# lmb-freiburg/flownet2

Hardware: AMD Instinct MI355X
Metric: image-pairs/sec FlowNetC forward at 448x320 (higher is better)
Workload: dtype f32

## Files before the change

flownet2_amd/_lib.py:

```python
from __future__ import annotations

import ctypes as C
import os
import re

_HERE = os.path.dirname(os.path.abspath(__file__))
SO_PATH = os.path.join(_HERE, "libflownet2_hip.so")
INCLUDE_DIR = os.path.join(_HERE, "..", "include")

_SCALARS = {"int": C.c_int, "float": C.c_float, "size_t": C.c_size_t, "long long": C.c_longlong, "unsigned long long": C.c_ulonglong,
            "char": C.c_char}
_POINTERS = {"float": C.c_void_p, "void": C.c_void_p, "unsigned char": C.c_void_p, "char": C.c_char_p, "int": C.POINTER(C.c_int),
             "unsigned": C.POINTER(C.c_uint), "size_t": C.POINTER(C.c_size_t)}
_STRUCT_NAMES = {"fn2_l1loss_params": "L1LossParams", "fn2_l1loss_scale": "L1LossScale"}
_DECLARATOR = re.compile(r"^([\w\s*]*?)(\w+)\s*(?:\[(\d+)\])?$")
_FUNCTION = re.compile(r"^([\w\s*]+?)\b(fn2_\w+)\s*\(([^()]*)\)$")


class Fn2Error(RuntimeError):

    def __init__(self, status: int, message: str):
        super().__init__(f"[fn2 status {status}] {message}")
        self.status = status


def _ctype(spec, structs, where):
    words = [w for w in spec.replace("*", " ").split() if w != "const"]
    base, stars = " ".join(words), spec.count("*")
    if stars == 0 and base in _SCALARS:
        return _SCALARS[base]
    if stars == 1 and base in structs:
        return C.POINTER(structs[base])
    if stars == 1 and base in _POINTERS:
        return _POINTERS[base]
    if stars == 2 and base in ("float", "void"):
        return C.POINTER(C.c_void_p)
    raise ValueError(f"C header: unknown type `{spec.strip()}` in `{where}`")


def _declarator(text, structs, where):
    m = _DECLARATOR.match(text.strip())
    if not m or not m.group(1).strip():
        raise ValueError(f"C header: cannot read `{text.strip()}` in `{where}`")
    t = _ctype(m.group(1), structs, where)
    return m.group(2), (t * int(m.group(3)) if m.group(3) else t), m.group(1)


def parse_header(text, structs=None):
    structs = dict(structs or {})
    functions, constants = {}, {}
    text = re.sub(r"/\*.*?\*/", " ", text, flags=re.S)
    for name, value in re.findall(r"^[ \t]*#[ \t]*define[ \t]+(FN2_\w+)[ \t]+(-?(?:0[xX][0-9a-fA-F]+|\d+))[ \t]*$", text, flags=re.M):
        constants[name] = int(value, 0)
    text = re.sub(r"^[ \t]*#.*$", " ", text, flags=re.M)

    def enum(m):
        value = -1
        for item in filter(None, (s.strip() for s in m.group(1).split(","))):
            name, _, v = (s.strip() for s in item.partition("="))
            value = int(v, 0) if v else value + 1
            constants[name] = value
        return " "
    text = re.sub(r"(?:typedef\s+)?enum\s*\w*\s*\{([^{}]*)\}\s*\w*\s*;", enum, text)

    def struct(m):
        cname, fields = m.group(1), []
        for decl in filter(None, (s.strip() for s in m.group(2).split(";"))):
            first, *more = decl.split(",")
            name, t, spec = _declarator(first, structs, "struct " + cname)
            fields.append((name, t))
            fields += [_declarator(spec + " " + other, structs, "struct " + cname)[:2] for other in more]
        pyname = _STRUCT_NAMES.get(cname) or "".join(w.capitalize() for w in cname.split("_")[1:])
        structs[cname] = type(pyname, (C.Structure,), {"_fields_": fields, "__doc__": cname, "__module__": __name__})
        return " "
    text = re.sub(r"typedef\s+struct\s+(fn2_\w+)\s*\{([^{}]*)\}\s*\w+\s*;", struct, text)

    text = re.sub(r'extern\s*"C"\s*\{|\}', " ", text)
    for stmt in filter(None, (" ".join(s.split()) for s in text.split(";"))):
        m = _FUNCTION.match(stmt)
        if not m:
            raise ValueError(f"C header: cannot read the declaration `{stmt}`")
        params = m.group(3).strip()
        args = [] if params == "void" else [_declarator(p, structs, stmt)[1] for p in params.split(",")]
        functions[m.group(2)] = (_ctype(m.group(1), structs, stmt), args)
    return functions, structs, constants


def _parse_headers():
    per_header, structs, constants = [], {}, {}
    for h in ("flownet2_hip.h", "flownet2_hip_solver.h", "flownet2_hip_corr_route.h", "flownet2_hip_conv_general.h"):
        with open(os.path.join(INCLUDE_DIR, h)) as f:
            functions, structs, c = parse_header(f.read(), structs)
        per_header.append(functions)
        constants.update(c)
    return per_header, structs, constants


_PER_HEADER, _STRUCTS, CONSTANTS = _parse_headers()
EXPORTS, SOLVER_EXPORTS, CORR_ROUTE_EXPORTS, CONV_GENERAL_EXPORTS = (list(f) for f in _PER_HEADER)
PROTOTYPES = {name: proto for f in _PER_HEADER for name, proto in f.items()}
globals().update({cls.__name__: cls for cls in _STRUCTS.values()})
_HOOKS = parse_header("""
    int fn2_debug_set_correlation_impl(int impl);
    int fn2_debug_correlation_units_plan(int N, int H, int W, int policy, unsigned* out_words, int max_words);
    int fn2_debug_set_resample_generic(int on);
    int fn2_debug_set_correlation_trace(void* device_buffer);""")[0]

_lib = None


def lib():
    global _lib
    if _lib is not None:
        return _lib
    if not os.path.exists(SO_PATH):
        raise RuntimeError(
            f"{SO_PATH} not found: the HIP extension is not built. Run `python -m flownet2_amd.build` "
            "(or __graft_entry__.build()). flownet2_amd has no CPU / PyTorch fallback.")
    L = C.CDLL(SO_PATH)
    for table, required in ((PROTOTYPES, True), (_HOOKS, False)):
        for name, (restype, argtypes) in table.items():
            if not hasattr(L, name):
                if required:
                    raise RuntimeError(f"{SO_PATH} does not export {name}")
                continue
            fn = getattr(L, name)
            fn.restype, fn.argtypes = restype, argtypes
    _lib = L
    return L


def check(status: int):
    if status != 0:
        raise Fn2Error(status, lib().fn2_last_error_string().decode())


def version() -> str:
    return lib().fn2_version().decode()
```

flownet2_amd/csrc/conv_mfma.hip:

```cpp
#include "mfma_tile.hpp"

namespace fn2 {
namespace cv {

using namespace mfma;

struct Args {
  const float* in; const float* wp; const float* bias; float* out;
  int N, Cin, Hin, Win, in_ctot, in_c0;
  int Cout, Hout, Wout, out_ctot, out_c0;
  int pad;
  int nchunks;
  int ksteps;
  int tx, ty;
  int ng;
  unsigned total;
  unsigned nbig;
  float slope; int relu;
};

template <int KS_, int S_, int MW_, int NP_, int WM_, int WNX_, int WNY_, int CQ_, int P16_ = 0, int PIN_ = 0>
struct Cfg : Window<((P16_ ? 1 : 4) * WNY_ - 1) * S_ + KS_,
                    ((P16_ ? 16 : 4) * NP_ * WNX_ - 1) * S_ + KS_ + 4,
                    CQ_, WM_ * WNX_ * WNY_> {
// ... 170 lines not shown
}

template <int KS> struct PackTile {
  static constexpr int T = KS * KS;
  static constexpr int QT = KS == 1 ? 8 : KS == 3 ? 3 : KS == 4 ? 2 : 1;
  static constexpr int CIL = 4 * QT, ROW = CIL * T + 1;
  static constexpr int LDS_FLOATS = 64 * ROW;
};

template <int KS, int ORDER>
__global__ void __launch_bounds__(256) pack_weights_view(const float* __restrict__ w, float* __restrict__ wp, int ksteps, int kalloc,
                                                         int src_co, int src_ci, long long s_co, long long s_ci, int flip) {
  using P = PackTile<KS>;
  constexpr int T = P::T, QT = P::QT, CIL = P::CIL, ROW = P::ROW;
  __shared__ float tile[P::LDS_FLOATS];
  const int grp = blockIdx.x, cq0 = blockIdx.y * QT;
  const int co0 = 64 * grp, ci0 = 4 * cq0;
  const int nquads = ksteps / T;
  constexpr int TOTAL = 64 * CIL * T;
  if constexpr (ORDER == 0) {
    const float* src = w + (size_t)co0 * s_co + (size_t)ci0 * T;
#pragma unroll
    for (int i = threadIdx.x; i < TOTAL; i += 256) {
      const int col = i / (CIL * T), e = i - col * (CIL * T), c = e / T;
      tile[col * ROW + e] = (co0 + col < src_co && ci0 + c < src_ci) ? src[(size_t)col * s_co + e] : 0.f;
    }
  } else if constexpr (ORDER == 1) {
    const float* src = w + (size_t)ci0 * s_ci + (size_t)co0 * T;
#pragma unroll
    for (int i = threadIdx.x; i < TOTAL; i += 256) {
      const int c = i / (64 * T), e = i - c * (64 * T), col = e / T, t = e - col * T;
      tile[col * ROW + c * T + t] = (co0 + col < src_co && ci0 + c < src_ci) ? src[(size_t)c * s_ci + e] : 0.f;
    }
  } else {
#pragma unroll
    for (int i = threadIdx.x; i < TOTAL; i += 256) {
      const int col = i / (CIL * T), e = i - col * (CIL * T), c = e / T, t = e - c * T;
      tile[col * ROW + e] = (co0 + col < src_co && ci0 + c < src_ci) ? w[(size_t)(co0 + col) * s_co + (size_t)(ci0 + c) * s_ci + t] : 0.f;
    }
  }
  __syncthreads();
  const int nq = min(QT, nquads - cq0);
  float* dst = wp + ((size_t)grp * kalloc + (size_t)cq0 * T) * 256;
  const int j = threadIdx.x & 3, lane = threadIdx.x >> 2;
  const float* trow = tile + (16 * j + (lane & 15)) * ROW + (lane >> 4) * T;
#pragma unroll
  for (int ks = 0; ks < QT * T; ++ks) {
    const int cq = ks / T, tap = ks - cq * T;
    if (cq < nq) dst[ks * 256 + threadIdx.x] = trow[4 * cq * T + (flip ? T - 1 - tap : tap)];
  }
  if (cq0 + QT >= nquads)
    for (int i = threadIdx.x; i < (kalloc - ksteps) * 256; i += 256) wp[((size_t)grp * kalloc + ksteps) * 256 + i] = 0.f;
}

template <int KS>
static void launch_pack_view(const float* w, float* wp, int Cout, int ksteps, int kalloc, int src_co, int src_ci, long long s_co, long long s_ci, int flip,
                             hipStream_t st) {
  using P = PackTile<KS>;
  const dim3 grid((unsigned)((Cout + 63) / 64), (unsigned)cdiv(ksteps / P::T, P::QT));
  if (s_ci == (long long)P::T) hipLaunchKernelGGL((pack_weights_view<KS, 0>), grid, dim3(256), 0, st, w, wp, ksteps, kalloc, src_co, src_ci, s_co, s_ci, flip);
  else if (s_co == (long long)P::T) hipLaunchKernelGGL((pack_weights_view<KS, 1>), grid, dim3(256), 0, st, w, wp, ksteps, kalloc, src_co, src_ci, s_co, s_ci, flip);
  else hipLaunchKernelGGL((pack_weights_view<KS, 2>), grid, dim3(256), 0, st, w, wp, ksteps, kalloc, src_co, src_ci, s_co, s_ci, flip);
}

constexpr int kSpare = 8;
constexpr int kChunkQuads = 2;

inline int chunk_quads(int KS) { return KS == 1 ? 8 : kChunkQuads; }
inline int ksteps_for(int Cin, int KS) { return cdiv(cdiv(Cin, 4), chunk_quads(KS)) * chunk_quads(KS) * KS * KS; }

template <class K>
static void set_geometry(Args& a) {
  if constexpr (K::P16) {
    a.Win *= a.Hin; a.Hin = 1; a.Wout *= a.Hout; a.Hout = 1;
  }
  a.tx = cdiv(a.Wout, K::TW); a.ty = cdiv(a.Hout, K::TH);
  a.ng = a.Cout / (16 * K::MW * K::WM);
  a.nchunks = cdiv(cdiv(a.Cin, 4), K::CQ);
}

inline long long tiles_of(const Args& a) { return (long long)a.N * a.tx * a.ty * a.ng; }

template <class K>
static int launch(const Args& base, hipStream_t st) {
  Args a = base;
  set_geometry<K>(a);
  a.nbig = (unsigned)tiles_of(a);
  return launch_tiles<&conv_mfma<K>>(a, tiles_of(a), K::THREADS, (int)(sizeof(float) * 2 * K::BUF), "conv_mfma", "conv_mfma_forward", st);
}

inline unsigned whole_rounds(long long tiles) { return (unsigned)(tiles / 256 * 256); }

template <class K>
static int launch_tail(const Args& base, hipStream_t st) {
  if constexpr (K::MW < 2) {
    return fail(FN2_ERR_UNSUPPORTED, "conv_mfma: variant has no split tail");
  } else {
    Args a = base;
    set_geometry<K>(a);
    if (tiles_of(a) > 0x1fffff00ll) return fail(FN2_ERR_UNSUPPORTED, "conv_mfma: grid too large");
    a.total = (unsigned)tiles_of(a); a.nbig = whole_rounds(a.total);
    const unsigned nsm = 2 * (a.total - a.nbig);
    const unsigned grid = a.nbig + 8 * ((nsm + 7) / 8);
    constexpr size_t lds = sizeof(float) * 2 * K::BUF;
    set_dynamic_lds_once<&conv_mfma_tail<K>>((int)lds);
    hipLaunchKernelGGL((conv_mfma_tail<K>), dim3(grid), dim3(K::THREADS), lds, st, a);
    return check_launch("conv_mfma_forward");
  }
}

struct Variant {
  int ks, s, mw, np, wm, wnx, wny, p16;
  int (*fn)(const Args&, hipStream_t);
  int (*fn_tail)(const Args&, hipStream_t);
};

#define FN2_CV_LIST(X) \
   \
  X(1, 1, 2, 7, 2, 2, 1, 8, 1) X(1, 1, 2, 7, 2, 1, 2, 8, 1) X(1, 1, 4, 7, 1, 2, 2, 8, 0) X(1, 1, 4, 7, 1, 1, 4, 8, 0) X(1, 1, 2, 6, 2, 2, 1, 8, 1) \
  X(1, 1, 2, 4, 2, 2, 1, 8, 1) X(1, 1, 2, 7, 1, 2, 2, 8, 0) X(1, 1, 2, 7, 1, 4, 1, 8, 0) X(1, 1, 2, 4, 1, 2, 2, 8, 0) X(1, 1, 4, 4, 1, 2, 2, 8, 0) \
   \
  X(3, 1, 2, 7, 2, 2, 1, 2, 1) X(3, 1, 2, 7, 2, 1, 2, 2, 1) X(3, 1, 4, 7, 1, 2, 2, 2, 0) X(3, 1, 4, 7, 1, 1, 4, 2, 0) \
  X(3, 1, 2, 6, 2, 2, 1, 2, 1) X(3, 1, 4, 6, 1, 2, 2, 2, 0) X(3, 1, 4, 4, 1, 2, 2, 2, 0) X(3, 1, 2, 4, 2, 2, 1, 2, 1) \
   \
  X(3, 2, 2, 7, 2, 1, 2, 2, 1) X(3, 2, 4, 7, 1, 1, 4, 2, 0) X(3, 2, 2, 6, 2, 2, 1, 2, 1) X(3, 2, 4, 6, 1, 2, 2, 2, 0) X(3, 2, 2, 4, 2, 2, 1, 2, 1) \
   \
  X(4, 2, 2, 7, 2, 2, 1, 2, 1) X(4, 2, 2, 7, 2, 1, 2, 2, 1) X(4, 2, 4, 7, 1, 2, 2, 2, 0) X(4, 2, 2, 6, 2, 2, 1, 2, 1) X(4, 2, 4, 4, 1, 2, 2, 2, 0) X(4, 2, 2, 4, 2, 2, 1, 2, 1) \
   \
  X(5, 2, 2, 7, 2, 2, 1, 1, 1) X(5, 2, 2, 7, 2, 1, 2, 1, 1) X(5, 2, 4, 7, 1, 2, 2, 1, 0) X(5, 2, 4, 7, 1, 1, 4, 1, 0) \
  X(5, 2, 2, 6, 2, 2, 1, 1, 1) X(5, 2, 4, 6, 1, 2, 2, 1, 0) X(5, 2, 4, 4, 1, 2, 2, 1, 0) \
   \
  X(7, 2, 2, 6, 2, 2, 1, 1, 1) X(7, 2, 2, 7, 2, 2, 1, 1, 1) X(7, 2, 4, 4, 1, 2, 2, 1, 0) X(7, 2, 4, 6, 1, 2, 2, 1, 0) X(7, 2, 2, 4, 2, 2, 1, 1, 1)

template <class K, int TAIL> struct TailFn { static constexpr int (*fn)(const Args&, hipStream_t) = nullptr; };
template <class K> struct TailFn<K, 1> { static constexpr int (*fn)(const Args&, hipStream_t) = &launch_tail<K>; };

#define FN2_CV_ROW(KS, S, MW, NP, WM, WNX, WNY, CQ, TAIL) \
  {KS, S, MW, NP, WM, WNX, WNY, 0, &launch<Cfg<KS, S, MW, NP, WM, WNX, WNY, CQ>>, TailFn<Cfg<KS, S, MW, NP, WM, WNX, WNY, CQ>, TAIL>::fn},
#define FN2_CV_ROW16(MW, NP, WM, WNX, WNY, TAIL) \
  {1, 1, MW, NP, WM, WNX, WNY, 1, &launch<Cfg<1, 1, MW, NP, WM, WNX, WNY, 8, 1>>, TailFn<Cfg<1, 1, MW, NP, WM, WNX, WNY, 8, 1>, TAIL>::fn},
#define FN2_CV_PIN(KS, S, MW, NP, WM, WNX, WNY, CQ, P16, TAIL) \
  {KS, S, MW, NP, WM, WNX, WNY, P16, &launch<Cfg<KS, S, MW, NP, WM, WNX, WNY, CQ, P16, 1>>, TailFn<Cfg<KS, S, MW, NP, WM, WNX, WNY, CQ, P16, 1>, TAIL>::fn},
static const Variant kVariants[] = {FN2_CV_LIST(FN2_CV_ROW)
  FN2_CV_ROW16(2, 7, 2, 2, 1, 1) FN2_CV_ROW16(2, 7, 4, 1, 1, 1) FN2_CV_ROW16(4, 7, 1, 4, 1, 0) FN2_CV_ROW16(4, 7, 2, 2, 1, 0) FN2_CV_ROW16(2, 5, 2, 2, 1, 1)
  FN2_CV_ROW16(2, 4, 2, 2, 1, 1) FN2_CV_ROW16(2, 7, 1, 4, 1, 0) FN2_CV_ROW16(2, 5, 1, 4, 1, 0) FN2_CV_ROW16(4, 5, 1, 4, 1, 0) FN2_CV_ROW16(2, 4, 1, 4, 1, 0)
  FN2_CV_ROW16(4, 5, 2, 2, 1, 0) FN2_CV_ROW16(4, 4, 2, 2, 1, 0)
  FN2_CV_ROW16(2, 9, 4, 1, 1, 1) FN2_CV_ROW16(2, 9, 2, 2, 1, 1) FN2_CV_ROW16(2, 3, 2, 2, 1, 1) FN2_CV_ROW16(4, 3, 1, 4, 1, 0)
  FN2_CV_ROW16(4, 9, 4, 1, 1, 0) FN2_CV_ROW16(4, 9, 2, 2, 1, 0) FN2_CV_ROW16(4, 7, 4, 1, 1, 0)
  FN2_CV_PIN(5, 2, 2, 7, 2, 2, 1, 1, 0, 1) FN2_CV_PIN(5, 2, 2, 7, 2, 1, 2, 1, 0, 1)
  FN2_CV_PIN(1, 1, 4, 9, 4, 1, 1, 8, 1, 0) FN2_CV_PIN(1, 1, 2, 9, 4, 1, 1, 8, 1, 1) FN2_CV_PIN(1, 1, 2, 5, 2, 2, 1, 8, 1, 1) FN2_CV_PIN(1, 1, 4, 7, 4, 1, 1, 8, 1, 0)
  FN2_CV_PIN(1, 1, 2, 7, 2, 2, 1, 8, 1, 1) FN2_CV_PIN(1, 1, 2, 3, 2, 2, 1, 8, 1, 1)
  FN2_CV_PIN(3, 1, 2, 7, 2, 2, 1, 2, 0, 1) FN2_CV_PIN(3, 1, 2, 6, 2, 2, 1, 2, 0, 1) FN2_CV_PIN(3, 2, 2, 7, 2, 1, 2, 2, 0, 1) FN2_CV_PIN(3, 2, 2, 6, 2, 2, 1, 2, 0, 1)
  FN2_CV_PIN(4, 2, 2, 7, 2, 2, 1, 2, 0, 1) FN2_CV_PIN(4, 2, 2, 6, 2, 2, 1, 2, 0, 1) FN2_CV_PIN(5, 2, 2, 6, 2, 2, 1, 1, 0, 1)
  FN2_CV_PIN(7, 2, 2, 6, 2, 2, 1, 1, 0, 1) FN2_CV_PIN(7, 2, 4, 6, 1, 2, 2, 1, 0, 0)};
constexpr int kNumVariants = sizeof(kVariants) / sizeof(kVariants[0]);

int g_forced_variant = -1;

static double variant_cost(const Variant& v, const Args& a, bool tail) {
  const int tw = (v.p16 ? 16 : 4) * v.np * v.wnx, th = (v.p16 ? 1 : 4) * v.wny;
  const long long wgs = v.p16 ? (long long)a.N * cdiv(a.Wout * a.Hout, tw) * (a.Cout / (16 * v.mw * v.wm))
                              : (long long)a.N * cdiv(a.Wout, tw) * cdiv(a.Hout, th) * (a.Cout / (16 * v.mw * v.wm));
  double rounds = (double)((wgs + 255) / 256);
  if (tail) {
    const long long r = wgs % 256;
    if (wgs < 256 || r == 0 || r > 128) return 1e30;
    rounds = (double)(wgs / 256) + 0.5 * 1.12;
  }
  const double eff = 1.0 / (1.0 + 0.08 * (4.0 / v.mw - 1.0) + 0.02 * (7.0 / v.np - 1.0));
  return rounds * v.mw * v.np / eff;
}

static bool variant_applies(const Variant& v, const Args& a, int KS, int S) {
  if (!v.p16 && a.Win % 4 != 0) return false;
  return v.ks == KS && v.s == S && a.Cout % (16 * v.mw * v.wm) == 0;
}

}
}

using namespace fn2;

FN2_API size_t fn2_conv_mfma_packed_floats(int Cout, int Cin, int kernel) {
  if (Cout <= 0 || Cout % 32 != 0 || Cin <= 0 || kernel <= 0) return 0;
  return (size_t)((Cout + 63) / 64) * (cv::ksteps_for(Cin, kernel) + cv::kSpare) * 256;
}

FN2_API int fn2_conv_mfma_pack_weights_view(const float* weight, float* packed, int Cout, int Cin, int kernel, int src_cout, int src_cin,
                                            long long stride_cout, long long stride_cin, int flip, void* stream);

FN2_API int fn2_conv_mfma_pack_weights(const float* weight, float* packed, int Cout, int Cin, int kernel, void* stream) {
  if (!weight || !packed) return fail(FN2_ERR_INVALID_ARG, "conv_mfma_pack_weights: null blob");
  if (Cout <= 0 || Cout % 32 != 0 || Cin <= 0 || (kernel != 1 && kernel != 3 && kernel != 4 && kernel != 5 && kernel != 7))
    return fail(FN2_ERR_UNSUPPORTED, "conv_mfma_pack_weights: needs Cout %% 32 == 0 and kernel_size 1, 3, 4, 5 or 7 (got Cout %d, kernel %d)", Cout, kernel);
  return fn2_conv_mfma_pack_weights_view(weight, packed, Cout, Cin, kernel, Cout, Cin, (long long)Cin * kernel * kernel, (long long)kernel * kernel, 0, stream);
}

FN2_API int fn2_conv_mfma_pack_weights_view(const float* weight, float* packed, int Cout, int Cin, int kernel, int src_cout, int src_cin,
                                            long long stride_cout, long long stride_cin, int flip, void* stream) {
  if (!weight || !packed) return fail(FN2_ERR_INVALID_ARG, "conv_mfma_pack_weights_view: null blob");
  if (Cout <= 0 || Cout % 32 != 0 || Cin <= 0 || (kernel != 1 && kernel != 3 && kernel != 4 && kernel != 5 && kernel != 7))
    return fail(FN2_ERR_UNSUPPORTED, "conv_mfma_pack_weights_view: needs Cout %% 32 == 0 and kernel_size 1, 3, 4, 5 or 7 (got Cout %d, kernel %d)", Cout, kernel);
  if (src_cout < 1 || src_cout > Cout || src_cin < 1 || src_cin > Cin || stride_cout < 1 || stride_cin < 1)
    return fail(FN2_ERR_INVALID_ARG, "conv_mfma_pack_weights_view: bad source view (%d of %d, %d of %d channels, strides %lld / %lld)", src_cout, Cout,
                src_cin, Cin, stride_cout, stride_cin);
  const int ksteps = cv::ksteps_for(Cin, kernel), kalloc = ksteps + cv::kSpare;
  hipStream_t st = as_stream(stream);
  switch (kernel) {
    case 1: cv::launch_pack_view<1>(weight, packed, Cout, ksteps, kalloc, src_cout, src_cin, stride_cout, stride_cin, flip ? 1 : 0, st); break;
    case 3: cv::launch_pack_view<3>(weight, packed, Cout, ksteps, kalloc, src_cout, src_cin, stride_cout, stride_cin, flip ? 1 : 0, st); break;
    case 4: cv::launch_pack_view<4>(weight, packed, Cout, ksteps, kalloc, src_cout, src_cin, stride_cout, stride_cin, flip ? 1 : 0, st); break;
    case 5: cv::launch_pack_view<5>(weight, packed, Cout, ksteps, kalloc, src_cout, src_cin, stride_cout, stride_cin, flip ? 1 : 0, st); break;
    default: cv::launch_pack_view<7>(weight, packed, Cout, ksteps, kalloc, src_cout, src_cin, stride_cout, stride_cin, flip ? 1 : 0, st); break;
  }
  return check_launch("conv_mfma_pack_weights_view");
}

FN2_API int fn2_conv_mfma_supported(int Cin, int Hin, int Win, int Cout, int kernel, int stride, int pad) {
  if (Cin <= 0 || Hin <= 0 || Win <= 0 || Cout <= 0 || Cout % 32 != 0) return 0;
  if (kernel == 1 ? ((long long)Hin * Win) % 4 != 0 : Win % 4 != 0) return 0;
  if (!((kernel == 1 && stride == 1) || (kernel == 3 && (stride == 1 || stride == 2)) || (kernel == 4 && stride == 2) || (kernel == 5 && stride == 2) || (kernel == 7 && stride == 2))) return 0;
  if (pad < 0 || pad > 4 || pad > kernel - 1) return 0;
  if ((long long)Cin * Hin * Win >= (1ll << 28)) return 0;
  const int Hout = (Hin + 2 * pad - kernel) / stride + 1, Wout = (Win + 2 * pad - kernel) / stride + 1;
  if (Hout < 1 || Wout < 1) return 0;
  cv::Args a{};
  a.Win = Win; a.Cout = Cout;
  for (int i = 0; i < cv::kNumVariants; ++i)
    if (cv::variant_applies(cv::kVariants[i], a, kernel, stride)) return 1;
  return 0;
}

FN2_API int fn2_debug_set_conv_variant(int v) { cv::g_forced_variant = v; return FN2_OK; }
FN2_API int fn2_conv_mfma_num_variants(void) { return cv::kNumVariants; }

FN2_API int fn2_conv_mfma_forward(const float* bottom, const float* packed_weight, const float* bias, float* top,
                                  int N, int Cin, int Hin, int Win, int bottom_channels, int bottom_c0,
                                  int Cout, int top_channels, int top_c0, int kernel, int stride, int pad,
                                  int relu, float negative_slope, void* stream) {
  if (N < 0) return fail(FN2_ERR_INVALID_ARG, "conv_mfma: bad batch");
  if (N == 0) return FN2_OK;
  if (const int rc = mfma::check_conv_args("conv_mfma", bottom, packed_weight, top, Cin, bottom_channels, bottom_c0, Cout, top_channels, top_c0, [&] {
        return fn2_conv_mfma_supported(Cin, Hin, Win, Cout, kernel, stride, pad) ? FN2_OK
            : fail(FN2_ERR_UNSUPPORTED, "conv_mfma: unsupported geometry (Cin %d, %dx%d, Cout %d, k %d s %d p %d)", Cin, Hin, Win, Cout, kernel, stride, pad);
      }))
    return rc;
  cv::Args a{};
  a.in = bottom; a.wp = packed_weight; a.bias = bias; a.out = top;
  a.N = N; a.Cin = Cin; a.Hin = Hin; a.Win = Win; a.in_ctot = bottom_channels; a.in_c0 = bottom_c0;
  a.Cout = Cout; a.Hout = (Hin + 2 * pad - kernel) / stride + 1; a.Wout = (Win + 2 * pad - kernel) / stride + 1;
  a.out_ctot = top_channels; a.out_c0 = top_c0; a.pad = pad;
  a.ksteps = cv::ksteps_for(Cin, kernel) + cv::kSpare;
  a.slope = negative_slope; a.relu = relu;
  hipStream_t st = as_stream(stream);
  static TuneCache cache("conv_mfma", cv::kNumVariants);
  const TuneKey key{N, Cin, Hin, Win, Cout, kernel, stride, pad, bottom_channels == Cin, top_channels == Cout};
  mfma::Pick p;
  if (const int rc = mfma::pick_variant(p, "conv_mfma", cv::g_forced_variant, cv::kNumVariants, true, cache, key, st,
                                        [&](int i) { return cv::variant_applies(cv::kVariants[i], a, kernel, stride); },
                                        [&](int i, bool tail) { return cv::variant_cost(cv::kVariants[i], a, tail); },
                                        [&](int i, bool tail) { return tail ? cv::kVariants[i].fn_tail(a, st) : cv::kVariants[i].fn(a, st); },
                                        [&](int i) { return cv::kVariants[i].fn_tail != nullptr; }))
    return rc;
  return p.tail ? cv::kVariants[p.variant].fn_tail(a, st) : cv::kVariants[p.variant].fn(a, st);
}
```

flownet2_amd/csrc/conv_plane.hip:

```cpp
#include "mfma_tile.hpp"

namespace fn2 {
namespace cp {

using namespace mfma;

constexpr int kNPR = 12;
constexpr int kLdsBytes = 160 * 1024;
constexpr int kSpare = 8;

struct Args {
  const float* in; const float* wp; const float* bias; float* out; float* part;
  int N, Cin, Hin, Win, in_ctot, in_c0;
  int Cout, Hout, Wout, out_ctot, out_c0;
  int pad;
  int P;
  int Wp;
  int img;
  int npb;
  int nig;
  int ng;
  int ksplit;
  int units;
  int ksteps;
  size_t class_stride;
  int rs, cs, wr;
  int band;
  int cap;
  int slots_c, npr;
  int buf;
  unsigned mP, mW, mrs;
  unsigned total;
  float slope; int relu;
};

template <int MODE_, int S_, int MW_, int NP_, int WM_, int WN_, int CQ_, int VEC_, int KS_ = 3>
struct Cfg {
  static constexpr int MODE = MODE_, S = S_, MW = MW_, NP = NP_, WM = WM_, WN = WN_, CQ = CQ_, VEC = VEC_, KS = KS_;
  static constexpr int NCLS = MODE == 1 ? 4 : 1;
  static constexpr int NW = NCLS * WM * WN, THREADS = 64 * NW;
  static constexpr int TAP = MODE == 1 ? 2 : KS;
  static constexpr int PADL = VEC == 4 ? 4 : (KS_ == 5 ? 2 : 1);
  static constexpr int KSC = CQ * TAP * TAP;
  static constexpr int NBUFA = KS_ == 5 ? 5 : (KSC % 9 == 0 && KSC > 9) ? 9 : (KSC % 8 == 0) ? 8 : (KSC % 4 == 0) ? 4 : 3;
  static constexpr int CAP = 16 * NP * WN;
  static_assert(KSC % NBUFA == 0, "ring phase must repeat per chunk");
  static_assert(NBUFA - 1 <= kSpare, "prefetch distance");
  static_assert(MODE == 0 || S == 1, "the deconvolution reads its input at stride 1");
  static_assert(KS == 3 || ((KS == 4 || KS == 5) && MODE == 0 && S == 2), "tap classes: 3x3 / 1, 3x3 / 2, 4x4 / 2, 5x5 / 2");
};

__device__ __forceinline__ int fastdiv(int q, int d, unsigned m) { return d == 1 ? q : (int)__umulhi((unsigned)q, m); }
inline unsigned magic_for(int d) { return d <= 1 ? 0u : (unsigned)(((1ull << 32) + (unsigned)d - 1) / (unsigned)d); }

template <class K>
__device__ __forceinline__ void stage_chunk(__amdgpu_buffer_rsrc_t rs, const unsigned (&voff)[kNPR], const Args& a, unsigned dst, int wave,
                                            unsigned chunk_off, unsigned plane_bytes, unsigned img_bytes, int nimg) {
  const int planes = nimg * 4 * K::CQ;
  const int last = a.slots_c - 64;
  for (int pl = wave; pl < planes; pl += K::NW) {
    const int il = pl / (4 * K::CQ), ch = pl % (4 * K::CQ);
    const unsigned soff = __builtin_amdgcn_readfirstlane(chunk_off + (unsigned)il * img_bytes + (unsigned)ch * plane_bytes);
    const unsigned d0 = __builtin_amdgcn_readfirstlane(dst + 4u * (unsigned)(pl * a.cs));
#pragma unroll
    for (int j = 0; j < kNPR; ++j) {
      if (j < a.npr) {
        const int s0 = 64 * j < last ? 64 * j : last;
        __builtin_amdgcn_raw_ptr_buffer_load_lds(rs, (lds_ptr_t)(uintptr_t)(d0 + 4u * K::VEC * (unsigned)s0), 4 * K::VEC, voff[j], soff, 0, 0);
      }
    }
  }
}

template <class K>
__global__ void __launch_bounds__(K::THREADS)
conv_plane(Args a) {
  extern __shared__ __attribute__((aligned(16))) float smem[];
  constexpr int S = K::S, MW = K::MW, NP = K::NP, TAP = K::TAP;
  unsigned t;
  if (!xcd_task(blockIdx.x, a.total, t)) return;
  const int g = __builtin_amdgcn_readfirstlane((int)(t % a.ng)); t /= a.ng;
  const int pb = __builtin_amdgcn_readfirstlane((int)(t % a.npb)); t /= a.npb;
  const int ig = __builtin_amdgcn_readfirstlane((int)(t % a.nig));
  const int kp = __builtin_amdgcn_readfirstlane((int)(t / a.nig));

  const int tid = threadIdx.x, lane = tid & 63;
  const int wave = __builtin_amdgcn_readfirstlane(tid >> 6);
  const int cls = wave % K::NCLS, w2 = wave / K::NCLS;
  const int py = cls >> 1, px = cls & 1;
  const int wm = w2 % K::WM, wn = w2 / K::WM;
  const int n0 = ig * a.img;
  const int nimg = a.N - n0 < a.img ? a.N - n0 : a.img;

  const int u0 = __builtin_amdgcn_readfirstlane((int)((long long)kp * a.units / a.ksplit));
  const int u1 = __builtin_amdgcn_readfirstlane((int)((long long)(kp + 1) * a.units / a.ksplit));
  const int chunk0 = u0 * (2 / K::CQ), nchunks = (u1 - u0) * (2 / K::CQ);

  const int yblk = a.band ? fastdiv(pb * a.cap, a.Wp, a.mW) : 0;
  const int yorg = (K::MODE == 0 ? S * yblk : yblk) - a.pad;

  const size_t plane = (size_t)a.Hin * a.Win;
  const unsigned plane_bytes = 4u * (unsigned)plane, img_bytes = plane_bytes * (unsigned)a.in_ctot;
  const __amdgpu_buffer_rsrc_t rs = __builtin_amdgcn_make_buffer_rsrc(
      const_cast<float*>(a.in + ((size_t)n0 * a.in_ctot + a.in_c0) * plane), 0,
      (unsigned)(img_bytes * (unsigned)(nimg - 1) + plane_bytes * (unsigned)a.Cin), kRsrcWord3);
  unsigned voff[kNPR];
#pragma unroll
  for (int j = 0; j < kNPR; ++j) {
    voff[j] = kOOB;
    if (j < a.npr) {
      const int last = a.slots_c - 64;
      const int d = K::VEC * ((64 * j < last ? 64 * j : last) + lane);
      const int row = fastdiv(d, a.rs, a.mrs), col = d - row * a.rs;
      const int yi = yorg + row, xi = col - K::PADL;
      if (row < a.wr && yi >= 0 && yi < a.Hin && xi >= 0 && xi < a.Win) voff[j] = 4u * (unsigned)(yi * a.Win + xi);
    }
  }
  const unsigned lds_base = (unsigned)(uintptr_t)(lds_ptr_t)smem;
  const unsigned chunk_bytes = 4u * K::CQ * plane_bytes;

  const int kq = lane >> 4;
  const int tile0 = NP * (pb * K::WN + wn);
  const int lim = nimg * a.P;
  int base[NP];
#pragma unroll
  for (int p = 0; p < NP; ++p) {
    int q = 16 * (tile0 + p) + (lane & 15);
    if (q >= lim) q = 16 * tile0 < lim ? 16 * tile0 : 0;
    const int il = fastdiv(q, a.P, a.mP), rem = q - il * a.P;
    const int y = fastdiv(rem, a.Wp, a.mW), x = rem - y * a.Wp;
    if constexpr (K::MODE == 0) base[p] = (il * 4 * K::CQ + kq) * a.cs + (S * (y - yblk)) * a.rs + S * x + K::PADL - a.pad;
    else base[p] = (il * 4 * K::CQ + kq) * a.cs + (y - yblk + py) * a.rs + x + K::PADL - 1 + px;
  }
  using WV = typename WVec<MW>::T;
  const int cg0 = (g * K::WM + wm) * MW;
  const float* wl = weight_lane(a.wp + (size_t)cls * a.class_stride, cg0, a.ksteps, lane) + (size_t)chunk0 * K::KSC * 256;

  f32x4 acc[MW][NP];
#pragma unroll
  for (int j = 0; j < MW; ++j)
#pragma unroll
    for (int p = 0; p < NP; ++p) acc[j][p] = f32x4{0.f, 0.f, 0.f, 0.f};

  WV wreg[K::NBUFA];
  stage_chunk<K>(rs, voff, a, lds_base, wave, (unsigned)chunk0 * chunk_bytes, plane_bytes, img_bytes, nimg);
#pragma unroll
  for (int i = 0; i < K::NBUFA - 1; ++i) wreg[i] = weight_load<MW>(wl, i);

  for (int c = 0; c < nchunks; ++c) {
    const int buf = c & 1;
    wait_vmcnt<K::NBUFA - 1>();
    __builtin_amdgcn_s_barrier();
    if (c + 1 < nchunks)
      stage_chunk<K>(rs, voff, a, lds_base + 4u * (unsigned)((buf ^ 1) * a.buf), wave, (unsigned)(chunk0 + c + 1) * chunk_bytes, plane_bytes, img_bytes, nimg);
    const float* win = smem + buf * a.buf;
    const int ks0 = c * K::KSC;
    constexpr int NSTEP = K::CQ * TAP;
    float bb[2][TAP][NP];
    auto lds_step = [&](int st, float (&b)[TAP][NP]) {
      const float* wk = win + ((st / TAP) * 4 * a.cs + (st % TAP) * a.rs);
#pragma unroll
      for (int kx = 0; kx < TAP; ++kx)
#pragma unroll
        for (int p = 0; p < NP; ++p) b[kx][p] = wk[base[p] + kx];
    };
    lds_step(0, bb[0]);
    __builtin_amdgcn_sched_barrier(0);
#pragma unroll
    for (int st = 0; st < NSTEP; ++st) {
      const float* wkn = win + (((st + 1) / TAP) * 4 * a.cs + ((st + 1) % TAP) * a.rs);
#pragma unroll
      for (int kx = 0; kx < TAP; ++kx) {
        const int ks = st * TAP + kx;
        wreg[(ks + K::NBUFA - 1) % K::NBUFA] = weight_load<MW>(wl, ks0 + ks + K::NBUFA - 1);
        const WV w = wreg[ks % K::NBUFA];
#pragma unroll
        for (int p = 0; p < NP; ++p) {
#pragma unroll
          for (int j = 0; j < MW; ++j)
            acc[j][p] = __builtin_amdgcn_mfma_f32_16x16x4f32(bb[st & 1][kx][p], wget<MW>(w, j), acc[j][p], 0, 0, 0);
          if (st + 1 < NSTEP) bb[(st + 1) & 1][kx][p] = wkn[base[p] + kx];
          __builtin_amdgcn_sched_barrier(0);
        }
      }
    }
  }

  const bool final_pass = a.ksplit == 1;
  const int Po = a.Hout * a.Wout;
  float* dst = final_pass ? a.out : a.part + (size_t)kp * a.N * a.Cout * Po;
  const int ctot = final_pass ? a.out_ctot : a.Cout, c0 = final_pass ? a.out_c0 : 0;
#pragma unroll
  for (int p = 0; p < NP; ++p) {
    const int q0 = 16 * (tile0 + p) + 4 * (lane >> 4);
    if (q0 >= lim) continue;
    const int il = fastdiv(q0, a.P, a.mP), pix = q0 - il * a.P;
#pragma unroll
    for (int j = 0; j < MW; ++j) {
      const int co = 16 * (cg0 + j) + (lane & 15);
      const float bv = (final_pass && a.bias) ? a.bias[co] : 0.f;
      f32x4 v = acc[j][p];
      if (final_pass) v = bias_relu4(v, bv, a.relu, a.slope);
      if constexpr (K::MODE == 0) {
        float* o = dst + ((size_t)(n0 + il) * ctot + c0 + co) * a.P + pix;
        if (pix + 3 < a.P && (a.P & 3) == 0) *reinterpret_cast<f32x4*>(o) = v;
        else {
          int il2 = il, pix2 = pix;
#pragma unroll
          for (int r = 0; r < 4; ++r) {
            if (q0 + r < lim) dst[((size_t)(n0 + il2) * ctot + c0 + co) * a.P + pix2] = v[r];
            if (++pix2 == a.P) { pix2 = 0; ++il2; }
          }
        }
      } else {
        int il2 = il, m = fastdiv(pix, a.Wp, a.mW), l = pix - m * a.Wp;
#pragma unroll
        for (int r = 0; r < 4; ++r) {
          if (q0 + r < lim) dst[(((size_t)(n0 + il2) * ctot + c0 + co) * a.Hout + 2 * m + py) * a.Wout + 2 * l + px] = v[r];
          if (++l == a.Wp) { l = 0; if (++m == a.Hin) { m = 0; ++il2; } }
        }
      }
    }
  }
}

template <int KS>
__global__ void __launch_bounds__(256) plane_reduce(const float* __restrict__ part, const float* __restrict__ bias, float* __restrict__ out,
                                                    int N, int Cout, int P, int out_ctot, int out_c0, int ksplit, int relu, float slope) {
  const unsigned total = (unsigned)N * (unsigned)Cout * (unsigned)P;
  for (unsigned i = blockIdx.x * blockDim.x + threadIdx.x; i < total; i += gridDim.x * blockDim.x) {
    float s;
    if constexpr (KS > 0) {
      float v[KS];
#pragma unroll
      for (int k = 0; k < KS; ++k) v[k] = part[(size_t)k * total + i];
      s = v[0];
#pragma unroll
      for (int k = 1; k < KS; ++k) s += v[k];
    } else {
      s = part[i];
      int k = 1;
      for (; k + 3 < ksplit; k += 4) {
        float v[4];
#pragma unroll
        for (int j = 0; j < 4; ++j) v[j] = part[(size_t)(k + j) * total + i];
#pragma unroll
        for (int j = 0; j < 4; ++j) s += v[j];
      }
      for (; k < ksplit; ++k) s += part[(size_t)k * total + i];
    }
    const unsigned r = i / (unsigned)P, pix = i - r * (unsigned)P;
    const unsigned n = r / (unsigned)Cout, co = r - n * (unsigned)Cout;
    s += bias ? bias[co] : 0.f;
    if (relu) s = s > 0.f ? s : s * slope;
    out[((size_t)n * out_ctot + out_c0 + co) * P + pix] = s;
  }
}

template <int SK>
__global__ void __launch_bounds__(256) pack_deconv_weights(const float* __restrict__ w, float* __restrict__ wp, int Cin, int Cout, int ksteps, int kalloc) {
  constexpr int T = SK * SK, ROW = 8 * T + 1;
  __shared__ float tile[64 * ROW];
  const int grp = blockIdx.x, u = blockIdx.y;
  const int co0 = 64 * grp, ci0 = 8 * u, ngrp = Cout / 64;
#pragma unroll
  for (int i = threadIdx.x; i < 8 * 64 * T; i += 256) {
    const int c = i / (64 * T), e = i - c * (64 * T), col = e / T, t = e - col * T;
    tile[col * ROW + c * T + t] = (ci0 + c < Cin) ? w[((size_t)(ci0 + c) * Cout + co0) * T + e] : 0.f;
  }
  __syncthreads();
  const int j = threadIdx.x & 3, lane = threadIdx.x >> 2;
  const float* trow = tile + (16 * j + (lane & 15)) * ROW + (lane >> 4) * T;
#pragma unroll
  for (int cls = 0; cls < 4; ++cls) {
    const int py = cls >> 1, px = cls & 1;
    float* dst = wp + (((size_t)cls * ngrp + grp) * kalloc + (size_t)8 * u) * 256 + threadIdx.x;
#pragma unroll
    for (int k = 0; k < 8; ++k) {
      const int q = k >> 2, ta = (k >> 1) & 1, tb = k & 1;
      const int ky = py == 0 ? (ta == 0 ? 3 : 1) : (ta == 0 ? 2 : 0), kx = px == 0 ? (tb == 0 ? 3 : 1) : (tb == 0 ? 2 : 0);
      dst[k * 256] = (ky < SK && kx < SK) ? trow[4 * q * T + ky * SK + kx] : 0.f;
    }
    if (8 * (u + 1) >= ksteps)
      for (int i = threadIdx.x; i < (kalloc - ksteps) * 256; i += 256) wp[(((size_t)cls * ngrp + grp) * kalloc + ksteps) * 256 + i] = 0.f;
  }
}

struct Variant {
  int mode, s, mw, np, wm, wn, cq, vec, ks;
  int (*fn)(const Args&, hipStream_t);
};

static bool plan(const Variant& v, Args& a) {
  if (a.Cout % (16 * v.mw * v.wm) != 0) return false;
  if (v.vec == 4 && a.Win % 4 != 0) return false;
  const int padl = v.vec == 4 ? 4 : (v.ks == 5 ? 2 : 1);
  const int cap = 16 * v.np * v.wn;
  a.cap = cap;
  int prow = v.mode == 0 ? a.Hout : a.Hin;
  a.band = 0;
  if (a.P > cap) {
    const int span = (cap + a.Wp - 2) / a.Wp + 1;
    if (span < prow) { prow = span; a.band = 1; }
  }
  if (v.mode == 0) {
    const int wr_need = (prow - 1) * v.s + v.ks;
    a.wr = (!a.band && a.Hin + 2 * a.pad < wr_need) ? a.Hin + 2 * a.pad : wr_need;
  } else {
    a.wr = prow + 2;
  }
  const int wc = padl + a.Win + (v.ks == 5 ? 2 : 1);
  a.rs = v.vec == 4 ? cdiv(wc, 4) * 4 : wc;
  const int plane_dw = a.wr * a.rs < 64 * v.vec ? 64 * v.vec : a.wr * a.rs;
  a.cs = up_mod(plane_dw, 16, 32);
  a.slots_c = a.cs / v.vec;
  a.npr = cdiv(a.slots_c, 64);
  if (a.npr > kNPR) return false;
  int img = 1;
  if (a.P < cap && a.Cin % 8 == 0) {
    img = cap / a.P;
    if (img > a.N) img = a.N;
    while (img > 1 && 2ll * img * 4 * v.cq * a.cs * 4 > kLdsBytes) --img;
  }
  if (2ll * img * 4 * v.cq * a.cs * 4 > kLdsBytes) return false;
  a.img = img;
  a.nig = cdiv(a.N, img);
  a.npb = img == 1 ? cdiv(a.P, cap) : 1;
  a.ng = a.Cout / (16 * v.mw * v.wm);
  a.buf = img * 4 * v.cq * a.cs;
  if ((long long)a.N * a.P >= 65536 || a.cs >= 65536) return false;
  a.mP = magic_for(a.P); a.mW = magic_for(a.Wp); a.mrs = magic_for(a.rs);
  const long long total = (long long)a.ng * a.npb * a.nig * a.ksplit;
  if (total > 0x3fffff00ll) return false;
  a.total = (unsigned)total;
  return true;
}

template <class K>
static int launch(const Args& a, hipStream_t st) {
  const size_t lds = sizeof(float) * 2 * (size_t)a.buf;
  set_dynamic_lds_once<&conv_plane<K>>(kLdsBytes);
  hipLaunchKernelGGL((conv_plane<K>), dim3(8 * ((a.total + 7) / 8)), dim3(K::THREADS), lds, st, a);
  return check_launch("conv_plane_forward");
}

#define FN2_CP_TILES(X, S, VEC) \
  X(0, S, 2, 9, 2, 2, 2, VEC) X(0, S, 2, 5, 2, 2, 2, VEC) X(0, S, 2, 7, 2, 2, 2, VEC) X(0, S, 4, 5, 1, 4, 2, VEC) X(0, S, 2, 9, 1, 4, 1, VEC) \
  X(0, S, 4, 9, 1, 4, 1, VEC) X(0, S, 2, 9, 1, 4, 2, VEC) X(0, S, 4, 4, 2, 2, 2, VEC) \
   \
  X(0, S, 2, 9, 2, 4, 2, VEC) X(0, S, 2, 5, 2, 4, 2, VEC) X(0, S, 2, 5, 4, 2, 2, VEC)
#define FN2_DP_TILES(X, VEC) \
  X(1, 1, 2, 9, 1, 1, 2, VEC) X(1, 1, 2, 9, 1, 1, 1, VEC) X(1, 1, 4, 9, 1, 1, 1, VEC) X(1, 1, 4, 9, 1, 1, 2, VEC) X(1, 1, 2, 5, 1, 1, 2, VEC) \
  X(1, 1, 4, 5, 1, 1, 2, VEC) X(1, 1, 2, 7, 1, 1, 2, VEC) X(1, 1, 4, 7, 1, 1, 1, VEC)
#define FN2_CP_LIST(X) FN2_CP_TILES(X, 1, 1) FN2_CP_TILES(X, 1, 4) FN2_CP_TILES(X, 2, 1) FN2_CP_TILES(X, 2, 4) FN2_DP_TILES(X, 1) FN2_DP_TILES(X, 4)
#define FN2_CP_ROW(MODE, S, MW, NP, WM, WN, CQ, VEC) {MODE, S, MW, NP, WM, WN, CQ, VEC, MODE == 1 ? 4 : 3, &launch<Cfg<MODE, S, MW, NP, WM, WN, CQ, VEC>>},
#define FN2_CP4_TILES(X, VEC) X(2, 9, 2, 2, 2, VEC) X(2, 5, 2, 2, 2, VEC) X(4, 5, 1, 4, 2, VEC) X(2, 5, 2, 4, 2, VEC)
#define FN2_CP4_ROW(MW, NP, WM, WN, CQ, VEC) {0, 2, MW, NP, WM, WN, CQ, VEC, 4, &launch<Cfg<0, 2, MW, NP, WM, WN, CQ, VEC, 4>>},
#define FN2_CP5_TILES(X, VEC) X(2, 9, 2, 2, 1, VEC) X(2, 5, 2, 2, 1, VEC) X(4, 5, 1, 4, 1, VEC) X(2, 9, 1, 4, 1, VEC) X(2, 7, 2, 2, 1, VEC) X(4, 4, 2, 2, 1, VEC)
#define FN2_CP5_ROW(MW, NP, WM, WN, CQ, VEC) {0, 2, MW, NP, WM, WN, CQ, VEC, 5, &launch<Cfg<0, 2, MW, NP, WM, WN, CQ, VEC, 5>>},
static const Variant kVariants[] = {FN2_CP_LIST(FN2_CP_ROW) FN2_CP4_TILES(FN2_CP4_ROW, 1) FN2_CP4_TILES(FN2_CP4_ROW, 4)
                                    FN2_CP5_TILES(FN2_CP5_ROW, 1) FN2_CP5_TILES(FN2_CP5_ROW, 4)};
constexpr int kNumVariants = sizeof(kVariants) / sizeof(kVariants[0]);

int g_forced_variant = -1;
int g_forced_ksplit = 0;

static int ksplit_for(long long mfma_tiles, int units) {
  int k = 1;
  if (g_forced_ksplit > 0) k = g_forced_ksplit;
  else {
    const double want = 14336.0 / (double)mfma_tiles;
    while (k < 16 && (double)k < want) k *= 2;
    if ((double)k > 1.5 * want && k > 1) k /= 2;
  }
  while (k > 1 && k > units) k /= 2;
  return k;
}

static double variant_cost(const Variant& v, const Args& a) {
  const double rounds = (double)((a.total + 255) / 256);
  const double eff = 1.0 / (1.0 + 0.08 * (4.0 / v.mw - 1.0) + 0.02 * (9.0 / v.np - 1.0));
  return rounds * v.mw * v.np / eff;
}

static int forward(Args a, int mode, int stride, int ks, void* workspace, size_t workspace_bytes, const char* what, hipStream_t st) {
  const int Po = a.Hout * a.Wout;
  if (a.ksplit > 1) {
    const size_t need = sizeof(float) * (size_t)a.ksplit * a.N * a.Cout * Po;
    if (!workspace || workspace_bytes < need) return fail(FN2_ERR_WORKSPACE, "%s: workspace of %zu bytes needed", what, need);
    if ((reinterpret_cast<uintptr_t>(workspace) & 15) != 0) return fail(FN2_ERR_UNSUPPORTED, "%s: workspace must be 16-byte aligned", what);
    a.part = static_cast<float*>(workspace);
  }
  auto run = [&](int i) -> int {
    const Variant& v = kVariants[i];
    Args t = a;
    if (v.mode != mode || v.s != stride || v.ks != ks || !plan(v, t)) return FN2_ERR_UNSUPPORTED;
    return v.fn(t, st);
  };
  auto applies = [&](int i) -> bool {
    Args t = a;
    return kVariants[i].mode == mode && kVariants[i].s == stride && kVariants[i].ks == ks && plan(kVariants[i], t);
  };
  auto cost = [&](int i, bool) -> double {
    Args t = a;
    plan(kVariants[i], t);
    return variant_cost(kVariants[i], t);
  };
  static TuneCache cache_conv("conv_plane", kNumVariants), cache_deconv("deconv_plane", kNumVariants);
  const TuneKey key{a.N, a.Cin, a.Hin, a.Win, a.Cout, stride + 16 * ks, a.pad, a.ksplit, a.in_ctot == a.Cin, a.out_ctot == a.Cout};
  Pick p;
  if (const int rc = pick_variant(p, what, g_forced_variant, kNumVariants, false, mode == 0 ? cache_conv : cache_deconv, key, st, applies, cost,
                                  [&](int i, bool) { return run(i); }, [](int) { return false; }))
    return rc;
  if (const int rc = run(p.variant)) return rc;
  if (a.ksplit > 1) {
    const long long total = (long long)a.N * a.Cout * Po;
    if (total >= (1ll << 31)) return fail(FN2_ERR_UNSUPPORTED, "%s: blob too large for the part reduction", what);
    const dim3 rg(blocks_for(total, 256, 4096));
#define FN2_PR(KS_) hipLaunchKernelGGL(plane_reduce<KS_>, rg, dim3(256), 0, st, a.part, a.bias, a.out, a.N, a.Cout, Po, a.out_ctot, a.out_c0, a.ksplit, a.relu, a.slope)
    switch (a.ksplit) {
      case 2: FN2_PR(2); break;
      case 3: FN2_PR(3); break;
      case 4: FN2_PR(4); break;
      case 6: FN2_PR(6); break;
      case 8: FN2_PR(8); break;
      case 12: FN2_PR(12); break;
      case 16: FN2_PR(16); break;
      default: FN2_PR(0); break;
    }
#undef FN2_PR
    return check_launch(what);
  }
  return FN2_OK;
}

static bool supported(const Args& a, int mode, int stride, int ks) {
  for (int i = 0; i < kNumVariants; ++i) {
    Args t = a;
    if (kVariants[i].mode == mode && kVariants[i].s == stride && kVariants[i].ks == ks && plan(kVariants[i], t)) return true;
  }
  return false;
}

}
}

using namespace fn2;

static bool plane_geometry_ok(int N, int Cin, int Hin, int Win, int Cout, int kernel, int stride, int pad) {
  if (N <= 0 || Cin <= 0 || Cin % 8 != 0 || Hin <= 0 || Win <= 0 || Cout <= 0 || Cout % 64 != 0) return false;
  if ((stride != 1 && stride != 2) || pad < 0 || pad > 2) return false;
  if (!((kernel == 3 && pad <= 1) || (kernel == 4 && stride == 2 && pad == 1) || (kernel == 5 && stride == 2 && pad == 2))) return false;
  if (Hin + 2 * pad < kernel || Win + 2 * pad < kernel) return false;
  if ((long long)N * Cin * Hin * Win >= (1ll << 28)) return false;
  return true;
}

static void fill_args(cp::Args& a, int N, int Cin, int Hin, int Win, int Cout, int kernel, int stride, int pad) {
  a.N = N; a.Cin = Cin; a.Hin = Hin; a.Win = Win; a.Cout = Cout; a.pad = pad;
  a.Hout = (Hin + 2 * pad - kernel) / stride + 1; a.Wout = (Win + 2 * pad - kernel) / stride + 1;
  a.P = a.Hout * a.Wout; a.Wp = a.Wout;
  a.units = ((Cin + 3) / 4 + 1) / 2;
  a.ksplit = cp::ksplit_for((long long)cp::cdiv(order_batch(N) * a.P, 16) * (Cout / 16), a.units);
  a.ksteps = a.units * 2 * kernel * kernel + cp::kSpare;
  a.class_stride = 0;
}

FN2_API int fn2_conv_plane_k_supported(int N, int Cin, int Hin, int Win, int Cout, int kernel, int stride, int pad) {
  if (!plane_geometry_ok(N, Cin, Hin, Win, Cout, kernel, stride, pad)) return 0;
  cp::Args a{};
  fill_args(a, N, Cin, Hin, Win, Cout, kernel, stride, pad);
  return cp::supported(a, 0, stride, kernel) ? 1 : 0;
}

FN2_API int fn2_conv_plane_k_ksplit(int N, int Cin, int Hin, int Win, int Cout, int kernel, int stride, int pad) {
  if (!plane_geometry_ok(N, Cin, Hin, Win, Cout, kernel, stride, pad)) return 0;
  cp::Args a{};
  fill_args(a, N, Cin, Hin, Win, Cout, kernel, stride, pad);
  return a.ksplit;
}

FN2_API size_t fn2_conv_plane_k_workspace_bytes(int N, int Cin, int Hin, int Win, int Cout, int kernel, int stride, int pad) {
  if (!plane_geometry_ok(N, Cin, Hin, Win, Cout, kernel, stride, pad)) return 0;
  cp::Args a{};
  fill_args(a, N, Cin, Hin, Win, Cout, kernel, stride, pad);
  return a.ksplit > 1 ? sizeof(float) * (size_t)a.ksplit * N * Cout * a.P : 0;
}

FN2_API int fn2_conv_plane_supported(int N, int Cin, int Hin, int Win, int Cout, int stride, int pad) {
  return fn2_conv_plane_k_supported(N, Cin, Hin, Win, Cout, 3, stride, pad);
}
FN2_API int fn2_conv_plane_ksplit(int N, int Cin, int Hin, int Win, int Cout, int stride, int pad) {
  return fn2_conv_plane_k_ksplit(N, Cin, Hin, Win, Cout, 3, stride, pad);
}
FN2_API size_t fn2_conv_plane_workspace_bytes(int N, int Cin, int Hin, int Win, int Cout, int stride, int pad) {
  return fn2_conv_plane_k_workspace_bytes(N, Cin, Hin, Win, Cout, 3, stride, pad);
}

FN2_API int fn2_debug_set_plane_variant(int v) { cp::g_forced_variant = v; return FN2_OK; }
FN2_API int fn2_debug_set_plane_ksplit(int k) { cp::g_forced_ksplit = k; return FN2_OK; }
FN2_API int fn2_conv_plane_num_variants(void) { return cp::kNumVariants; }

FN2_API int fn2_conv_plane_k_forward(const float* bottom, const float* packed_weight, const float* bias, float* top,
                                     int N, int Cin, int Hin, int Win, int bottom_channels, int bottom_c0,
                                     int Cout, int top_channels, int top_c0, int kernel, int stride, int pad,
                                     int relu, float negative_slope, void* workspace, size_t workspace_bytes, void* stream) {
  if (N < 0) return fail(FN2_ERR_INVALID_ARG, "conv_plane: bad batch");
  if (N == 0) return FN2_OK;
  if (!bottom || !packed_weight || !top) return fail(FN2_ERR_INVALID_ARG, "conv_plane: null blob");
  if (!plane_geometry_ok(N, Cin, Hin, Win, Cout, kernel, stride, pad))
    return fail(FN2_ERR_UNSUPPORTED, "conv_plane: unsupported geometry (N %d, Cin %d, %dx%d, Cout %d, k %d s %d p %d)", N, Cin, Hin, Win, Cout, kernel, stride, pad);
  if (bottom_c0 < 0 || bottom_c0 + Cin > bottom_channels || top_c0 < 0 || top_c0 + Cout > top_channels)
    return fail(FN2_ERR_INVALID_ARG, "conv_plane: channel slice outside the blob");
  if (((reinterpret_cast<uintptr_t>(bottom) | reinterpret_cast<uintptr_t>(top) | reinterpret_cast<uintptr_t>(packed_weight)) & 15) != 0)
    return fail(FN2_ERR_UNSUPPORTED, "conv_plane: blobs must be 16-byte aligned");
  if ((long long)bottom_channels * Hin * Win * 4 * N >= 0x7ffffff0ll) return fail(FN2_ERR_UNSUPPORTED, "conv_plane: bottom blob too large");
  cp::Args a{};
  fill_args(a, N, Cin, Hin, Win, Cout, kernel, stride, pad);
  a.in = bottom; a.wp = packed_weight; a.bias = bias; a.out = top;
  a.in_ctot = bottom_channels; a.in_c0 = bottom_c0; a.out_ctot = top_channels; a.out_c0 = top_c0;
  a.slope = negative_slope; a.relu = relu;
  return cp::forward(a, 0, stride, kernel, workspace, workspace_bytes, "conv_plane", as_stream(stream));
}

FN2_API int fn2_conv_plane_forward(const float* bottom, const float* packed_weight, const float* bias, float* top,
                                   int N, int Cin, int Hin, int Win, int bottom_channels, int bottom_c0,
                                   int Cout, int top_channels, int top_c0, int stride, int pad,
                                   int relu, float negative_slope, void* workspace, size_t workspace_bytes, void* stream) {
  return fn2_conv_plane_k_forward(bottom, packed_weight, bias, top, N, Cin, Hin, Win, bottom_channels, bottom_c0, Cout, top_channels, top_c0,
                                  3, stride, pad, relu, negative_slope, workspace, workspace_bytes, stream);
}

static bool deconv_geometry_ok(int N, int Cin, int Hin, int Win, int Cout) {
  if (N <= 0 || Cin <= 0 || Hin <= 0 || Win <= 0 || Cout <= 0 || Cout % 64 != 0) return false;
  if ((long long)N * Cin * Hin * Win >= (1ll << 28) || (long long)N * Cout * Hin * Win >= (1ll << 27)) return false;
  return true;
}

static void fill_deconv_args(cp::Args& a, int N, int Cin, int Hin, int Win, int Cout) {
  a.N = N; a.Cin = Cin; a.Hin = Hin; a.Win = Win; a.Cout = Cout; a.pad = 1;
  a.Hout = 2 * Hin; a.Wout = 2 * Win;
  a.P = Hin * Win; a.Wp = Win;
  a.units = ((Cin + 3) / 4 + 1) / 2;
  a.ksplit = cp::ksplit_for(4ll * cp::cdiv(order_batch(N) * a.P, 16) * (Cout / 16), a.units);
  a.ksteps = a.units * 2 * 4 + cp::kSpare;
  a.class_stride = (size_t)(Cout / 64) * a.ksteps * 256;
}

FN2_API int fn2_deconv_plane_supported(int N, int Cin, int Hin, int Win, int Cout) {
  if (!deconv_geometry_ok(N, Cin, Hin, Win, Cout)) return 0;
  cp::Args a{};
  fill_deconv_args(a, N, Cin, Hin, Win, Cout);
  return cp::supported(a, 1, 1, 4) ? 1 : 0;
}

FN2_API int fn2_deconv_plane_ksplit(int N, int Cin, int Hin, int Win, int Cout) {
  if (!deconv_geometry_ok(N, Cin, Hin, Win, Cout)) return 0;
  cp::Args a{};
  fill_deconv_args(a, N, Cin, Hin, Win, Cout);
  return a.ksplit;
}

FN2_API size_t fn2_deconv_plane_workspace_bytes(int N, int Cin, int Hin, int Win, int Cout) {
  if (!deconv_geometry_ok(N, Cin, Hin, Win, Cout)) return 0;
  cp::Args a{};
  fill_deconv_args(a, N, Cin, Hin, Win, Cout);
  return a.ksplit > 1 ? sizeof(float) * (size_t)a.ksplit * N * Cout * a.Hout * a.Wout : 0;
}

FN2_API size_t fn2_deconv_plane_packed_floats(int Cin, int Cout) {
  if (Cin <= 0 || Cout <= 0 || Cout % 64 != 0) return 0;
  return 4 * (size_t)(Cout / 64) * ((((Cin + 3) / 4 + 1) / 2) * 2 * 4 + cp::kSpare) * 256;
}

FN2_API int fn2_deconv_plane_pack_weights_k(const float* weight, float* packed, int Cin, int Cout, int src_kernel, void* stream) {
  if (!weight || !packed) return fail(FN2_ERR_INVALID_ARG, "deconv_plane_pack_weights: null blob");
  if (Cin <= 0 || Cout <= 0 || Cout % 64 != 0) return fail(FN2_ERR_UNSUPPORTED, "deconv_plane_pack_weights: needs Cout %% 64 == 0 (got %d)", Cout);
  if (src_kernel != 3 && src_kernel != 4) return fail(FN2_ERR_UNSUPPORTED, "deconv_plane_pack_weights: the blob has 4x4 taps, or 3x3 (zero-padded to 4x4)");
  const int units = ((Cin + 3) / 4 + 1) / 2, ksteps = units * 2 * 4, kalloc = ksteps + cp::kSpare;
  const dim3 grid((unsigned)(Cout / 64), (unsigned)units);
  if (src_kernel == 4) hipLaunchKernelGGL((cp::pack_deconv_weights<4>), grid, dim3(256), 0, as_stream(stream), weight, packed, Cin, Cout, ksteps, kalloc);
  else hipLaunchKernelGGL((cp::pack_deconv_weights<3>), grid, dim3(256), 0, as_stream(stream), weight, packed, Cin, Cout, ksteps, kalloc);
  return check_launch("deconv_plane_pack_weights");
}

FN2_API int fn2_deconv_plane_pack_weights(const float* weight, float* packed, int Cin, int Cout, void* stream) {
  return fn2_deconv_plane_pack_weights_k(weight, packed, Cin, Cout, 4, stream);
}

FN2_API int fn2_deconv_plane_forward(const float* bottom, const float* packed_weight, const float* bias, float* top,
                                     int N, int Cin, int Hin, int Win, int bottom_channels, int bottom_c0,
                                     int Cout, int top_channels, int top_c0, int relu, float negative_slope,
                                     void* workspace, size_t workspace_bytes, void* stream) {
  if (N < 0) return fail(FN2_ERR_INVALID_ARG, "deconv_plane: bad batch");
  if (N == 0) return FN2_OK;
  if (!bottom || !packed_weight || !top) return fail(FN2_ERR_INVALID_ARG, "deconv_plane: null blob");
  if (!deconv_geometry_ok(N, Cin, Hin, Win, Cout))
    return fail(FN2_ERR_UNSUPPORTED, "deconv_plane: unsupported geometry (N %d, Cin %d, %dx%d, Cout %d)", N, Cin, Hin, Win, Cout);
  if (bottom_c0 < 0 || bottom_c0 + Cin > bottom_channels || top_c0 < 0 || top_c0 + Cout > top_channels)
    return fail(FN2_ERR_INVALID_ARG, "deconv_plane: channel slice outside the blob");
  if (((reinterpret_cast<uintptr_t>(bottom) | reinterpret_cast<uintptr_t>(top) | reinterpret_cast<uintptr_t>(packed_weight)) & 15) != 0)
    return fail(FN2_ERR_UNSUPPORTED, "deconv_plane: blobs must be 16-byte aligned");
  if ((long long)bottom_channels * Hin * Win * 4 * N >= 0x7ffffff0ll) return fail(FN2_ERR_UNSUPPORTED, "deconv_plane: bottom blob too large");
  cp::Args a{};
  fill_deconv_args(a, N, Cin, Hin, Win, Cout);
  a.in = bottom; a.wp = packed_weight; a.bias = bias; a.out = top;
  a.in_ctot = bottom_channels; a.in_c0 = bottom_c0; a.out_ctot = top_channels; a.out_c0 = top_c0;
  a.slope = negative_slope; a.relu = relu;
  return cp::forward(a, 1, 1, 4, workspace, workspace_bytes, "deconv_plane", as_stream(stream));
}
```

flownet2_amd/csrc/conv_route.cpp:

```cpp
#include "conv_internal.hpp"
#include "fn2_common.hpp"

namespace {

struct Out { int H, W; };
inline Out conv_out(const fn2_conv_desc* d) {
  return {(d->Hin + 2 * d->pad - d->kernel) / d->stride + 1, (d->Win + 2 * d->pad - d->kernel) / d->stride + 1};
}

bool valid(const fn2_conv_desc* d) {
  return d && d->N >= 1 && d->Cin >= 1 && d->Cout >= 1 && d->Hin >= 1 && d->Win >= 1 && d->kernel >= 1 && d->stride >= 1 && d->pad >= 0 &&
         d->Hin + 2 * d->pad >= d->kernel && d->Win + 2 * d->pad >= d->kernel;
}

bool conv_route_applies(const fn2_conv_desc* d, int route) {
  const int k = d->kernel, s = d->stride, p = d->pad;
  switch (route) {
    case FN2_CONV_ROUTE_WINOGRAD: return k == 3 && s == 1 && fn2_conv_wino_supported(d->Cin, d->Hin, d->Win, d->Cout, p) != 0;
    case FN2_CONV_ROUTE_PLANE:
      return k == 3 ? fn2_conv_plane_supported(d->N, d->Cin, d->Hin, d->Win, d->Cout, s, p) != 0
                    : (k == 5 && s == 2 && p == 2 && fn2_conv_plane_k_supported(d->N, d->Cin, d->Hin, d->Win, d->Cout, 5, 2, 2) != 0);
    case FN2_CONV_ROUTE_DIRECT: return fn2_conv_mfma_supported(d->Cin, d->Hin, d->Win, d->Cout, k, s, p) != 0;
    case FN2_CONV_ROUTE_STEM: return k == 7 && s == 2 && p == 3 && fn2_conv_k7s2_relu_supported(d->Cin, d->Hin, d->Win, d->Cout) != 0;
    case FN2_CONV_ROUTE_HEAD: return k == 3 && s == 1 && p == 1 && d->Cout == 2;
    default: return false;
  }
}

bool split_route(const fn2_conv_desc* d, int route) {
  return route == (FN2_CONV_ROUTE_DIRECT | FN2_CONV_ARITH_BF16X3) && fn2_conv_bf16x3_supported(d) != 0;
}

bool wino_split_route(const fn2_conv_desc* d, int route) {
  return route == (FN2_CONV_ROUTE_WINOGRAD | FN2_CONV_ARITH_BF16X3) && fn2_conv_wino_bf16x3_supported(d) != 0;
}

bool deconv_gemm_ok(const fn2_conv_desc* d) {
  return (d->Cout * 16) % 32 == 0 && (d->Hin * d->Win) % 4 == 0 && fn2_conv_mfma_supported(d->Cin, d->Hin, d->Win, d->Cout * 16, 1, 1, 0) != 0;
}

bool deconv_split_route(const fn2_conv_desc* d, int route) {
  return route == (FN2_DECONV_ROUTE_GEMM | FN2_CONV_ARITH_BF16X3) && d->kernel == 4 && d->stride == 2 && d->pad == 1 && deconv_gemm_ok(d) &&
         fn2_deconv_bf16x3_supported(d) != 0;
}

bool deconv_route_applies(const fn2_conv_desc* d, int route) {
  if (d->kernel != 4 || d->stride != 2 || d->pad != 1) return false;
  if (deconv_split_route(d, route)) return true;
  switch (route) {
    case FN2_DECONV_ROUTE_GEMM: return deconv_gemm_ok(d);
    case FN2_DECONV_ROUTE_PLANE: return fn2_deconv_plane_supported(d->N, d->Cin, d->Hin, d->Win, d->Cout) != 0;
    case FN2_DECONV_ROUTE_HEAD: return d->Cin == 2 && d->Cout == 2;
    default: return false;
  }
}

}

FN2_API int fn2_conv_route(const fn2_conv_desc* d, int flags) {
  if (!valid(d)) return FN2_CONV_ROUTE_NONE;
  const bool force = (flags & FN2_ROUTE_FORCE) != 0;
  const int k = d->kernel, s = d->stride, p = d->pad, Cin = d->Cin, Cout = d->Cout, H = d->Hin, W = d->Win;
  const bool inv = fn2_get_batch_invariant() != 0;
  const int N = inv ? 1 : d->N;
  const bool wino_first = force || inv;
  const Out o = conv_out(d);
  if (k == 7 && s == 2 && p == 3 && !(Cin % 4 == 0 && fn2_conv_mfma_supported(Cin, H, W, Cout, k, s, p)) && fn2_conv_k7s2_relu_supported(Cin, H, W, Cout))
    return FN2_CONV_ROUTE_STEM;
  if (k == 3 && s == 1 && p == 1 && Cout == 2) return FN2_CONV_ROUTE_HEAD;
  const bool wino_ok = k == 3 && s == 1 && fn2_conv_wino_supported(Cin, H, W, Cout, p) != 0;
  const int wino = ((flags & FN2_ROUTE_WINO_BF16X3) && fn2_conv_wino_bf16x3_supported(d)) ? (FN2_CONV_ROUTE_WINOGRAD | FN2_CONV_ARITH_BF16X3) : FN2_CONV_ROUTE_WINOGRAD;
  if (wino_ok && (wino_first || (long long)N * ((o.H + 7) / 8) * ((o.W + 7) / 8) * (Cout / 16) >= 1000)) return wino;
  const int maxpix = 8000;
  if (k == 3 && (force || o.H * o.W <= maxpix) && fn2_conv_plane_supported(N, Cin, H, W, Cout, s, p) &&
      (N == d->N || fn2_conv_plane_supported(d->N, Cin, H, W, Cout, s, p)))
    return FN2_CONV_ROUTE_PLANE;
  if (k == 5 && s == 2 && p == 2 && (long long)N * ((o.H + 3) / 4) * ((o.W + 3) / 4) * (Cout / 16) < 64 * 256 && o.H * o.W <= maxpix &&
      fn2_conv_plane_k_supported(d->N, Cin, H, W, Cout, 5, 2, 2) && (N == d->N || fn2_conv_plane_k_supported(N, Cin, H, W, Cout, 5, 2, 2)))
    return FN2_CONV_ROUTE_PLANE;
  if (wino_ok) return wino;
  if (fn2_conv_mfma_supported(Cin, H, W, Cout, k, s, p))
    return ((flags & FN2_ROUTE_BF16X3) && fn2_conv_bf16x3_supported(d)) ? (FN2_CONV_ROUTE_DIRECT | FN2_CONV_ARITH_BF16X3) : FN2_CONV_ROUTE_DIRECT;
  return FN2_CONV_ROUTE_NONE;
}

FN2_API size_t fn2_conv_packed_weight_floats(const fn2_conv_desc* d, int route) {
  if (!valid(d)) return 0;
  if (split_route(d, route)) return fn2::conv_bf16x3_packed_floats(d->Cout, d->Cin, d->kernel);
  if (wino_split_route(d, route)) return fn2::conv_wino_bf16x3_packed_floats(d->Cout, d->Cin);
  if (route == FN2_CONV_ROUTE_WINOGRAD) return fn2_conv_wino_packed_floats(d->Cout, d->Cin);
  if (route == FN2_CONV_ROUTE_DIRECT || route == FN2_CONV_ROUTE_PLANE) return fn2_conv_mfma_packed_floats(d->Cout, d->Cin, d->kernel);
  if (route == FN2_CONV_ROUTE_STEM || route == FN2_CONV_ROUTE_HEAD) return (size_t)d->Cout * d->Cin * d->kernel * d->kernel;
  return 0;
}

FN2_API int fn2_conv_pack_weights(const fn2_conv_desc* d, int route, const float* weight, float* packed, void* stream) {
  if (!valid(d) || !weight || !packed) return fn2::fail(FN2_ERR_INVALID_ARG, "conv_pack_weights: bad descriptor or NULL blob");
  if (split_route(d, route)) return fn2::conv_bf16x3_pack_weights(weight, packed, d->Cout, d->Cin, d->kernel, stream);
  if (wino_split_route(d, route)) return fn2::conv_wino_bf16x3_pack_weights(weight, packed, d->Cout, d->Cin, stream);
  if (route == FN2_CONV_ROUTE_WINOGRAD) return fn2_conv_wino_pack_weights(weight, packed, d->Cout, d->Cin, stream);
  if (route == FN2_CONV_ROUTE_DIRECT || route == FN2_CONV_ROUTE_PLANE) return fn2_conv_mfma_pack_weights(weight, packed, d->Cout, d->Cin, d->kernel, stream);
  if (route == FN2_CONV_ROUTE_STEM || route == FN2_CONV_ROUTE_HEAD) {
    if (weight != packed &&
        hipMemcpyAsync(packed, weight, sizeof(float) * (size_t)d->Cout * d->Cin * d->kernel * d->kernel, hipMemcpyDeviceToDevice, fn2::as_stream(stream)) != hipSuccess)
      return fn2::fail(FN2_ERR_LAUNCH, "conv_pack_weights: device copy of the weight blob failed");
    return FN2_OK;
  }
  return fn2::fail(FN2_ERR_UNSUPPORTED, "conv_pack_weights: no own kernel for this layer (route %d)", route);
}

FN2_API size_t fn2_conv_workspace_bytes(const fn2_conv_desc* d, int route) {
  if (valid(d) && route == FN2_CONV_ROUTE_HEAD) return fn2_predict_flow_conv_workspace_bytes(d->N, d->Cin, d->Hin, d->Win);
  if (!valid(d) || route != FN2_CONV_ROUTE_PLANE) return 0;
  return d->kernel == 3 ? fn2_conv_plane_workspace_bytes(d->N, d->Cin, d->Hin, d->Win, d->Cout, d->stride, d->pad)
                        : fn2_conv_plane_k_workspace_bytes(d->N, d->Cin, d->Hin, d->Win, d->Cout, d->kernel, d->stride, d->pad);
}

FN2_API int fn2_conv_forward(const fn2_conv_desc* d, int route, const float* bottom, int bottom_channels, int bottom_c0,
                             const float* packed_weight, const float* bias, float* top, int top_channels, int top_c0,
                             int relu, float negative_slope, void* workspace, size_t workspace_bytes, void* stream) {
  if (!valid(d)) return fn2::fail(FN2_ERR_INVALID_ARG, "conv_forward: bad descriptor");
  if (split_route(d, route))
    return fn2::conv_bf16x3_forward(bottom, packed_weight, bias, top, d->N, d->Cin, d->Hin, d->Win, bottom_channels, bottom_c0, d->Cout, top_channels,
                                    top_c0, d->kernel, d->stride, d->pad, relu, negative_slope, stream);
  if (wino_split_route(d, route))
    return fn2::conv_wino_bf16x3_forward(bottom, packed_weight, bias, top, d->N, d->Cin, d->Hin, d->Win, bottom_channels, bottom_c0, d->Cout, top_channels,
                                         top_c0, d->kernel, d->stride, d->pad, relu, negative_slope, stream);
  if (!conv_route_applies(d, route))
    return fn2::fail(FN2_ERR_UNSUPPORTED, "conv_forward: no own kernel for Convolution{kernel %d, stride %d, pad %d} %d -> %d on %d x %d (route %d)",
                     d->kernel, d->stride, d->pad, d->Cin, d->Cout, d->Hin, d->Win, route);
  if (!bottom || !packed_weight || !top) return fn2::fail(FN2_ERR_INVALID_ARG, "conv_forward: NULL blob");
  if (bottom_c0 < 0 || bottom_c0 + d->Cin > bottom_channels || top_c0 < 0 || top_c0 + d->Cout > top_channels)
    return fn2::fail(FN2_ERR_INVALID_ARG, "conv_forward: channel slice outside its blob");
  switch (route) {
    case FN2_CONV_ROUTE_WINOGRAD:
      return fn2_conv_wino_forward(bottom, packed_weight, bias, top, d->N, d->Cin, d->Hin, d->Win, bottom_channels, bottom_c0, d->Cout, top_channels,
                                   top_c0, d->pad, relu, negative_slope, stream);
    case FN2_CONV_ROUTE_PLANE:
      if (d->kernel == 3)
        return fn2_conv_plane_forward(bottom, packed_weight, bias, top, d->N, d->Cin, d->Hin, d->Win, bottom_channels, bottom_c0, d->Cout,
                                      top_channels, top_c0, d->stride, d->pad, relu, negative_slope, workspace, workspace_bytes, stream);
      return fn2_conv_plane_k_forward(bottom, packed_weight, bias, top, d->N, d->Cin, d->Hin, d->Win, bottom_channels, bottom_c0, d->Cout,
                                      top_channels, top_c0, d->kernel, d->stride, d->pad, relu, negative_slope, workspace, workspace_bytes, stream);
    case FN2_CONV_ROUTE_DIRECT:
      return fn2_conv_mfma_forward(bottom, packed_weight, bias, top, d->N, d->Cin, d->Hin, d->Win, bottom_channels, bottom_c0, d->Cout, top_channels,
                                   top_c0, d->kernel, d->stride, d->pad, relu, negative_slope, stream);
    case FN2_CONV_ROUTE_STEM:
      if (bottom_channels != d->Cin || bottom_c0 != 0 || top_channels != d->Cout || top_c0 != 0)
        return fn2::fail(FN2_ERR_UNSUPPORTED, "conv_forward: the stem kernel reads and writes whole blobs, not channel slices");
      return fn2_conv_k7s2_relu_forward(bottom, packed_weight, bias, top, d->N, d->Cin, d->Hin, d->Win, d->Cout, relu ? negative_slope : 1.0f, stream);
    case FN2_CONV_ROUTE_HEAD: {
      if (bottom_channels != d->Cin || bottom_c0 != 0 || top_channels != d->Cout || top_c0 != 0)
        return fn2::fail(FN2_ERR_UNSUPPORTED, "conv_forward: the flow-head kernel reads and writes whole blobs, not channel slices");
      const int rc = fn2_predict_flow_conv_forward(bottom, packed_weight, bias, top, d->N, d->Cin, d->Hin, d->Win, workspace, workspace_bytes, stream);
      if (rc != FN2_OK || !relu) return rc;
      return fn2_bias_leaky_relu_forward(top, nullptr, d->N, d->Cout, d->Hin, d->Win, negative_slope, stream);
    }
    default:
      return fn2::fail(FN2_ERR_UNSUPPORTED, "conv_forward: no own kernel for Convolution{kernel %d, stride %d, pad %d} %d -> %d on %d x %d",
                       d->kernel, d->stride, d->pad, d->Cin, d->Cout, d->Hin, d->Win);
  }
}

FN2_API int fn2_deconv_route(const fn2_conv_desc* d, int flags) {
  if (!valid(d) || d->kernel != 4 || d->stride != 2 || d->pad != 1) return FN2_DECONV_ROUTE_NONE;
  if (d->Cin == 2 && d->Cout == 2) return FN2_DECONV_ROUTE_HEAD;
  if (deconv_gemm_ok(d))
    return ((flags & FN2_ROUTE_BF16X3) && fn2_deconv_bf16x3_supported(d)) ? (FN2_DECONV_ROUTE_GEMM | FN2_CONV_ARITH_BF16X3) : FN2_DECONV_ROUTE_GEMM;
  if (fn2_deconv_plane_supported(d->N, d->Cin, d->Hin, d->Win, d->Cout)) return FN2_DECONV_ROUTE_PLANE;
  return FN2_DECONV_ROUTE_NONE;
}

FN2_API size_t fn2_deconv_packed_weight_floats(const fn2_conv_desc* d, int route) {
  if (!valid(d)) return 0;
  if (deconv_split_route(d, route)) return fn2::deconv_bf16x3_packed_floats(d->Cin, d->Cout);
  if (route == FN2_DECONV_ROUTE_GEMM) return fn2_conv_mfma_packed_floats(d->Cout * 16, d->Cin, 1);
  if (route == FN2_DECONV_ROUTE_PLANE) return fn2_deconv_plane_packed_floats(d->Cin, d->Cout);
  if (route == FN2_DECONV_ROUTE_HEAD) return (size_t)d->Cin * d->Cout * 16;
  return 0;
}

FN2_API int fn2_deconv_pack_weights(const fn2_conv_desc* d, int route, const float* weight, float* packed, void* stream) {
  if (!valid(d) || !weight || !packed) return fn2::fail(FN2_ERR_INVALID_ARG, "deconv_pack_weights: bad descriptor or NULL blob");
  if (deconv_split_route(d, route)) return fn2::deconv_bf16x3_pack_weights(weight, packed, d->Cin, d->Cout, stream);
  const int M = d->Cout * 16;
  if (route == FN2_DECONV_ROUTE_GEMM) return fn2_conv_mfma_pack_weights_view(weight, packed, M, d->Cin, 1, M, d->Cin, 1, M, 0, stream);
  if (route == FN2_DECONV_ROUTE_PLANE) return fn2_deconv_plane_pack_weights(weight, packed, d->Cin, d->Cout, stream);
  if (route == FN2_DECONV_ROUTE_HEAD) {
    if (weight != packed && hipMemcpyAsync(packed, weight, sizeof(float) * (size_t)d->Cin * d->Cout * 16, hipMemcpyDeviceToDevice, fn2::as_stream(stream)) != hipSuccess)
      return fn2::fail(FN2_ERR_LAUNCH, "deconv_pack_weights: device copy of the weight blob failed");
    return FN2_OK;
  }
  return fn2::fail(FN2_ERR_UNSUPPORTED, "deconv_pack_weights: no own kernel for this layer (route %d)", route);
}

FN2_API size_t fn2_deconv_workspace_bytes(const fn2_conv_desc* d, int route) {
  if (!valid(d)) return 0;
  if (route == FN2_DECONV_ROUTE_GEMM || deconv_split_route(d, route)) return sizeof(float) * (size_t)d->N * d->Cout * 16 * d->Hin * d->Win;
  if (route == FN2_DECONV_ROUTE_PLANE) return fn2_deconv_plane_workspace_bytes(d->N, d->Cin, d->Hin, d->Win, d->Cout);
  return 0;
}

FN2_API int fn2_deconv_forward(const fn2_conv_desc* d, int route, const float* bottom, int bottom_channels, int bottom_c0,
                               const float* packed_weight, const float* bias, float* top, int top_channels, int top_c0,
                               int relu, float negative_slope, void* workspace, size_t workspace_bytes, void* stream) {
  if (!valid(d)) return fn2::fail(FN2_ERR_INVALID_ARG, "deconv_forward: bad descriptor");
  if (!deconv_route_applies(d, route))
    return fn2::fail(FN2_ERR_UNSUPPORTED, "deconv_forward: no own kernel for Deconvolution{kernel %d, stride %d, pad %d} %d -> %d on %d x %d (route %d)",
                     d->kernel, d->stride, d->pad, d->Cin, d->Cout, d->Hin, d->Win, route);
  if (!bottom || !packed_weight || !top) return fn2::fail(FN2_ERR_INVALID_ARG, "deconv_forward: NULL blob");
  if (bottom_c0 < 0 || bottom_c0 + d->Cin > bottom_channels || top_c0 < 0 || top_c0 + d->Cout > top_channels)
    return fn2::fail(FN2_ERR_INVALID_ARG, "deconv_forward: channel slice outside its blob");
  if (route == FN2_DECONV_ROUTE_GEMM || route == (FN2_DECONV_ROUTE_GEMM | FN2_CONV_ARITH_BF16X3)) {
    if (!workspace || workspace_bytes < fn2_deconv_workspace_bytes(d, route))
      return fn2::fail(FN2_ERR_INVALID_ARG, "deconv_forward: workspace of %zu bytes needed for the column matrix", fn2_deconv_workspace_bytes(d, route));
    float* col = static_cast<float*>(workspace);
    int rc = route != FN2_DECONV_ROUTE_GEMM
                 ? fn2::deconv_bf16x3_gemm(bottom, packed_weight, col, d->N, d->Cin, d->Hin, d->Win, bottom_channels, bottom_c0, d->Cout, stream)
                 : fn2_conv_mfma_forward(bottom, packed_weight, nullptr, col, d->N, d->Cin, d->Hin, d->Win, bottom_channels, bottom_c0, d->Cout * 16,
                                         d->Cout * 16, 0, 1, 1, 0, 0, 0.f, stream);
    if (rc) return rc;
    return fn2_col2im_bias_relu_forward_into(col, bias, top, d->N, d->Cout, 2 * d->Hin, 2 * d->Win, 4, 1, 2, relu, negative_slope, top_channels, top_c0, stream);
  }
  if (route == FN2_DECONV_ROUTE_PLANE)
    return fn2_deconv_plane_forward(bottom, packed_weight, bias, top, d->N, d->Cin, d->Hin, d->Win, bottom_channels, bottom_c0, d->Cout, top_channels,
                                    top_c0, relu, negative_slope, workspace, workspace_bytes, stream);
  if (route == FN2_DECONV_ROUTE_HEAD) {
    if (bottom_channels != 2 || bottom_c0 != 0) return fn2::fail(FN2_ERR_UNSUPPORTED, "deconv_forward: the flow-head kernel reads a whole 2-channel blob");
    if (relu) return fn2::fail(FN2_ERR_UNSUPPORTED, "deconv_forward: the 2-channel flow-head kernel has no fused ReLU (the FlowNet graphs have none there)");
    return fn2_upsample_flow_deconv_forward_into(bottom, packed_weight, bias, top, d->N, d->Hin, d->Win, top_channels, top_c0, stream);
  }
  return fn2::fail(FN2_ERR_UNSUPPORTED, "deconv_forward: no own kernel for Deconvolution{kernel %d, stride %d, pad %d} %d -> %d on %d x %d",
                   d->kernel, d->stride, d->pad, d->Cin, d->Cout, d->Hin, d->Win);
}

namespace {

inline int round_up(int v, int m) { return (v + m - 1) / m * m; }
inline size_t align256(size_t v) { return (v + 255) & ~(size_t)255; }

struct Bwd { int route, Ct, Ht, Wt, Cb, Hb, Wb, Cp; };

Bwd bwd_geom(const fn2_conv_desc* d, int transposed) {
  Bwd g{FN2_BWD_ROUTE_NONE, 0, 0, 0, 0, 0, 0, 0};
  if (!valid(d)) return g;
  const int k = d->kernel, s = d->stride, p = d->pad, N = d->N;
  g.Cb = d->Cin; g.Hb = d->Hin; g.Wb = d->Win; g.Ct = d->Cout; g.Cp = d->Cin;
  if (transposed) {
    if (k != 4 || s != 2 || p != 1 || d->Cout % 4 != 0) return g;
    g.Ht = 2 * d->Hin; g.Wt = 2 * d->Win; g.Cp = round_up(d->Cin, 64);
    if (fn2_conv_mfma_supported(g.Ct, g.Ht, g.Wt, g.Cp, 4, 2, 1)) g.route = FN2_BWD_ROUTE_DIRECT;
    else if (d->Cout % 8 == 0 && fn2_conv_plane_k_supported(N, g.Ct, g.Ht, g.Wt, g.Cp, 4, 2, 1)) g.route = FN2_BWD_ROUTE_PLANE;
    return g;
  }
  const Out o = conv_out(d);
  g.Ht = o.H; g.Wt = o.W;
  if (s == 2 && ((k == 5 && p == 2) || (k == 3 && p == 1)) && d->Cin % 64 == 0) {
    if (fn2_tconv_supported(g.Ct, g.Ht, g.Wt, g.Cb, g.Hb, g.Wb, k, p)) { g.route = FN2_BWD_ROUTE_TCONV; return g; }
    if (k == 3 && g.Hb == 2 * g.Ht && g.Wb == 2 * g.Wt && fn2_deconv_plane_supported(N, g.Ct, g.Ht, g.Wt, g.Cb)) { g.route = FN2_BWD_ROUTE_DECONV_PLANE; return g; }
  }
  if (k == 1 && s == 1 && p == 0) {
    g.Cp = round_up(d->Cin, 32);
    if (fn2_conv_mfma_supported(g.Ct, g.Ht, g.Wt, g.Cp, 1, 1, 0)) g.route = FN2_BWD_ROUTE_DIRECT;
    return g;
  }
  if (k == 3 && s == 1 && p == 1) {
    g.Cp = round_up(d->Cin, 16);
    if (fn2_conv_wino_supported(g.Ct, g.Ht, g.Wt, g.Cp, 1)) { g.route = FN2_BWD_ROUTE_WINOGRAD; return g; }
    g.Cp = round_up(d->Cin, 64);
    if (d->Cout % 8 == 0 && fn2_conv_plane_supported(N, g.Ct, g.Ht, g.Wt, g.Cp, 1, 1)) g.route = FN2_BWD_ROUTE_PLANE;
  }
  return g;
}

size_t bwd_kernel_workspace(const fn2_conv_desc* d, int transposed, const Bwd& g) {
  if (g.route == FN2_BWD_ROUTE_PLANE)
    return transposed ? fn2_conv_plane_k_workspace_bytes(d->N, g.Ct, g.Ht, g.Wt, g.Cp, 4, 2, 1) : fn2_conv_plane_workspace_bytes(d->N, g.Ct, g.Ht, g.Wt, g.Cp, 1, 1);
  if (g.route == FN2_BWD_ROUTE_DECONV_PLANE) return fn2_deconv_plane_workspace_bytes(d->N, g.Ct, g.Ht, g.Wt, g.Cb);
  return 0;
}

__global__ void __launch_bounds__(256) rot180_swap(const float* __restrict__ w, float* __restrict__ out, int Cout, int Cin, int Cp) {
  const long long i = (long long)blockIdx.x * 256 + threadIdx.x, total = (long long)Cp * Cout * 9;
  if (i >= total) return;
  const int t = (int)(i % 9);
  const long long r = i / 9;
  const int co = (int)(r % Cout), ci = (int)(r / Cout);
  out[i] = ci < Cin ? w[((size_t)co * Cin + ci) * 9 + (8 - t)] : 0.f;
}

struct BwdRoute { int base; bool split; };
BwdRoute bwd_route_of(const fn2_conv_desc* d, int transposed, int route, const Bwd& g) {
  if (route == (FN2_BWD_ROUTE_TCONV | FN2_CONV_ARITH_BF16X3))
    return (g.route == FN2_BWD_ROUTE_TCONV && fn2_tconv_bf16x3_supported(d, transposed)) ? BwdRoute{FN2_BWD_ROUTE_TCONV, true} : BwdRoute{FN2_BWD_ROUTE_NONE, false};
  if (route & FN2_CONV_ARITH_BF16X3) return BwdRoute{FN2_BWD_ROUTE_NONE, false};
  return BwdRoute{route, false};
}

}

FN2_API int fn2_conv_backward_data_route(const fn2_conv_desc* d, int transposed) { return bwd_geom(d, transposed).route; }

FN2_API int fn2_conv_backward_data_route_flags(const fn2_conv_desc* d, int transposed, int flags) {
  const int route = bwd_geom(d, transposed).route;
  if ((flags & FN2_ROUTE_BF16X3) && route == FN2_BWD_ROUTE_TCONV && fn2_tconv_bf16x3_supported(d, transposed)) return route | FN2_CONV_ARITH_BF16X3;
  return route;
}

FN2_API size_t fn2_conv_backward_data_packed_weight_floats(const fn2_conv_desc* d, int transposed, int route_arith) {
  const Bwd g = bwd_geom(d, transposed);
  const BwdRoute br = bwd_route_of(d, transposed, route_arith, g);
  const int route = br.base;
  if (route == FN2_BWD_ROUTE_NONE || route != g.route) return 0;
  if (br.split) return fn2::tconv_bf16x3_packed_floats(g.Cb, g.Ct, d->kernel, d->pad);
  switch (route) {
    case FN2_BWD_ROUTE_WINOGRAD: return fn2_conv_wino_packed_floats(g.Cp, g.Ct);
    case FN2_BWD_ROUTE_TCONV: return fn2_conv_mfma_packed_floats(g.Cb, g.Ct, d->kernel);
    case FN2_BWD_ROUTE_DECONV_PLANE: return fn2_deconv_plane_packed_floats(g.Ct, g.Cb);
    default: return fn2_conv_mfma_packed_floats(g.Cp, g.Ct, d->kernel);
  }
}

FN2_API size_t fn2_conv_backward_data_pack_workspace_bytes(const fn2_conv_desc* d, int transposed, int route) {
  const Bwd g = bwd_geom(d, transposed);
  return (route == FN2_BWD_ROUTE_WINOGRAD && route == g.route) ? sizeof(float) * (size_t)g.Cp * g.Ct * 9 : 0;
}

FN2_API int fn2_conv_backward_data_pack_weights(const fn2_conv_desc* d, int transposed, int route, const float* weight, float* packed,
                                                void* workspace, size_t workspace_bytes, void* stream) {
  const Bwd g = bwd_geom(d, transposed);
  if (!weight || !packed) return fn2::fail(FN2_ERR_INVALID_ARG, "conv_backward_data_pack_weights: NULL blob");
  const BwdRoute br = bwd_route_of(d, transposed, route, g);
  if (br.base == FN2_BWD_ROUTE_NONE || br.base != g.route)
    return fn2::fail(FN2_ERR_UNSUPPORTED, "conv_backward_data_pack_weights: route %d is not this layer's (%d)", route, g.route);
  if (br.split) return fn2::tconv_bf16x3_pack_weights(weight, packed, g.Cb, g.Ct, d->kernel, d->pad, stream);
  const int k = d->kernel, Cin = d->Cin, Cout = d->Cout;
  switch (route) {
    case FN2_BWD_ROUTE_WINOGRAD: {
      const size_t need = fn2_conv_backward_data_pack_workspace_bytes(d, transposed, route);
      if (!workspace || workspace_bytes < need) return fn2::fail(FN2_ERR_WORKSPACE, "conv_backward_data_pack_weights: %zu bytes of scratch needed for the rotated blob", need);
      const long long total = (long long)g.Cp * Cout * 9;
      hipLaunchKernelGGL(rot180_swap, dim3((unsigned)((total + 255) / 256)), dim3(256), 0, reinterpret_cast<hipStream_t>(stream), weight,
                         static_cast<float*>(workspace), Cout, Cin, g.Cp);
      const int rc = fn2::check_launch("conv_backward_data_pack_weights (rotate)");
      if (rc) return rc;
      return fn2_conv_wino_pack_weights(static_cast<const float*>(workspace), packed, g.Cp, Cout, stream);
    }
    case FN2_BWD_ROUTE_TCONV:
      return fn2_conv_mfma_pack_weights_view(weight, packed, Cin, Cout, k, Cin, Cout, (long long)k * k, (long long)Cin * k * k, 0, stream);
    case FN2_BWD_ROUTE_DECONV_PLANE:
      return fn2_deconv_plane_pack_weights_k(weight, packed, Cout, Cin, 3, stream);
    case FN2_BWD_ROUTE_PLANE:
      if (transposed) return fn2_conv_mfma_pack_weights_view(weight, packed, g.Cp, Cout, 4, Cin, Cout, (long long)Cout * 16, 16, 0, stream);
      return fn2_conv_mfma_pack_weights_view(weight, packed, g.Cp, Cout, 3, Cin, Cout, 9, (long long)Cin * 9, 1, stream);
    default:
      if (transposed) return fn2_conv_mfma_pack_weights_view(weight, packed, g.Cp, Cout, 4, Cin, Cout, (long long)Cout * 16, 16, 0, stream);
      return fn2_conv_mfma_pack_weights_view(weight, packed, g.Cp, Cout, 1, Cin, Cout, 1, Cin, 0, stream);
  }
}

FN2_API size_t fn2_conv_backward_data_workspace_bytes(const fn2_conv_desc* d, int transposed, int route_arith) {
  const Bwd g = bwd_geom(d, transposed);
  const int route = bwd_route_of(d, transposed, route_arith, g).base;
  if (route == FN2_BWD_ROUTE_NONE || route != g.route) return 0;
  size_t b = align256(bwd_kernel_workspace(d, transposed, g));
  if (g.Cp != g.Cb) b += sizeof(float) * (size_t)d->N * g.Cp * g.Hb * g.Wb;
  return b;
}

FN2_API size_t fn2_conv_backward_data_workspace_bytes_with_room(const fn2_conv_desc* d, int transposed, int route_arith, int bottom_room) {
  const Bwd g = bwd_geom(d, transposed);
  const int route = bwd_route_of(d, transposed, route_arith, g).base;
  if (route == FN2_BWD_ROUTE_NONE || route != g.route) return 0;
  if (bottom_room >= g.Cp) return bwd_kernel_workspace(d, transposed, g);
  return fn2_conv_backward_data_workspace_bytes(d, transposed, route);
}

FN2_API int fn2_conv_backward_data_computed_channels(const fn2_conv_desc* d, int transposed, int route_arith) {
  const Bwd g = bwd_geom(d, transposed);
  const int route = bwd_route_of(d, transposed, route_arith, g).base;
  return (route == FN2_BWD_ROUTE_NONE || route != g.route) ? 0 : g.Cp;
}

FN2_API int fn2_conv_backward_data_masked_supported(const fn2_conv_desc* d, int transposed, int route_arith) {
  const Bwd g = bwd_geom(d, transposed);
  const int route = bwd_route_of(d, transposed, route_arith, g).base;
  return route == FN2_BWD_ROUTE_TCONV && route == g.route && g.Cp == g.Cb;
}
// ... 155 lines not shown
```

flownet2_amd/csrc/flow_head.hip:

```cpp
#include "fn2_common.hpp"

namespace fn2 {

constexpr int kHeadPix = 64;

template <int G>
__global__ void __launch_bounds__(kHeadPix* G) conv3x3_c2_taps(const float* __restrict__ in, const float* __restrict__ w,
                                                                float* __restrict__ P, int N, int C, int H, int W, int nsplit) {
  __shared__ float red[G][18][kHeadPix];
  const int lane_pix = threadIdx.x % kHeadPix;
  const int grp = __builtin_amdgcn_readfirstlane(threadIdx.x / kHeadPix);
  const size_t plane = (size_t)H * W;
  const long long total = (long long)N * H * W;
  const long long p = (long long)blockIdx.x * kHeadPix + lane_pix;
  const bool live = p < total;
  const int n = live ? (int)(p / (long long)plane) : 0;
  const unsigned pix = live ? (unsigned)(p - (long long)n * plane) : 0u;
  const float* src = in + (size_t)n * C * plane + pix;
  float a[18];
#pragma unroll
  for (int k = 0; k < 18; ++k) a[k] = 0.f;
  const int ngroups = G * nsplit;
  const int c_per = (C + ngroups - 1) / ngroups;
  const int c_lo = min(C, ((int)blockIdx.y * G + grp) * c_per), c_hi = min(C, c_lo + c_per);
  for (int c = c_lo; c < c_hi; c += 8) {
    float v[8];
#pragma unroll
    for (int cc = 0; cc < 8; ++cc) v[cc] = (c + cc < c_hi) ? src[(size_t)(c + cc) * plane] : 0.f;
    __builtin_amdgcn_sched_barrier(0);
#pragma unroll
    for (int cc = 0; cc < 8; ++cc) {
      if (c + cc < c_hi) {
        const float* w0 = w + (size_t)(c + cc) * 9;
        const float* w1 = w + ((size_t)C + c + cc) * 9;
#pragma unroll
        for (int t = 0; t < 9; ++t) {
          a[t] = fmaf(w0[t], v[cc], a[t]);
          a[9 + t] = fmaf(w1[t], v[cc], a[9 + t]);
        }
      }
    }
  }
#pragma unroll
  for (int k = 0; k < 18; ++k) red[grp][k][lane_pix] = a[k];
  __syncthreads();
  if (live) {
    float* dst = P + ((size_t)blockIdx.y * N + n) * 18 * plane + pix;
    for (int k = grp; k < 18; k += G) {
      float sacc = 0.f;
#pragma unroll
      for (int g = 0; g < G; ++g) sacc += red[g][k][lane_pix];
      dst[(size_t)k * plane] = sacc;
    }
  }
}

template <int NSPLIT>
__global__ void __launch_bounds__(256) conv3x3_c2_gather(const float* __restrict__ P, const float* __restrict__ bias,
                                                          float* __restrict__ out, int N, int H, int W) {
  const unsigned plane = (unsigned)H * W;
  const unsigned pix = blockIdx.x * 256u + threadIdx.x;
  if (pix >= plane) return;
  const int y = pix / W, x = pix - y * W;
  const unsigned no = blockIdx.y;
  const unsigned n = no >> 1, o = no & 1;
  float v[NSPLIT][9];
#pragma unroll
  for (int sp = 0; sp < NSPLIT; ++sp) {
    const float* Pn = P + (((size_t)sp * N + n) * 18 + o * 9) * plane;
#pragma unroll
    for (int dy = 0; dy < 3; ++dy)
#pragma unroll
      for (int dx = 0; dx < 3; ++dx) {
        const int yy = y + dy - 1, xx = x + dx - 1;
        const bool ok = yy >= 0 && yy < H && xx >= 0 && xx < W;
        v[sp][dy * 3 + dx] = ok ? Pn[(size_t)(dy * 3 + dx) * plane + (unsigned)yy * W + xx] : 0.f;
      }
  }
  float sacc = bias ? bias[o] : 0.f;
#pragma unroll
  for (int sp = 0; sp < NSPLIT; ++sp)
#pragma unroll
    for (int t = 0; t < 9; ++t) sacc += v[sp][t];
  out[(size_t)no * plane + pix] = sacc;
}

__global__ void __launch_bounds__(256) deconv4x4s2_c2(const float* __restrict__ in, const float* __restrict__ w,
                                                       const float* __restrict__ bias, float* __restrict__ out,
                                                       int N, int H, int W, int out_ctot, int out_c0) {
  const int Ho = 2 * H, Wo = 2 * W;
  const long long total = (long long)N * Ho * Wo;
  for (long long idx = blockIdx.x * (long long)blockDim.x + threadIdx.x; idx < total; idx += (long long)gridDim.x * blockDim.x) {
    const int X = (int)(idx % Wo), Y = (int)((idx / Wo) % Ho), n = (int)(idx / ((long long)Wo * Ho));
    float a0 = bias ? bias[0] : 0.f, a1 = bias ? bias[1] : 0.f;
#pragma unroll
    for (int ty = 0; ty < 2; ++ty) {
      const int ky = ((Y + 1) & 1) + 2 * ty;
      const int iy = (Y + 1 - ky) / 2;
      if (Y + 1 - ky < 0 || iy >= H) continue;
#pragma unroll
      for (int tx = 0; tx < 2; ++tx) {
        const int kx = ((X + 1) & 1) + 2 * tx;
        const int ix = (X + 1 - kx) / 2;
        if (X + 1 - kx < 0 || ix >= W) continue;
#pragma unroll
        for (int c = 0; c < 2; ++c) {
          const float v = in[(((size_t)n * 2 + c) * H + iy) * W + ix];
          a0 = fmaf(w[((c * 2 + 0) * 4 + ky) * 4 + kx], v, a0);
          a1 = fmaf(w[((c * 2 + 1) * 4 + ky) * 4 + kx], v, a1);
        }
      }
    }
    out[(((size_t)n * out_ctot + out_c0 + 0) * Ho + Y) * Wo + X] = a0;
    out[(((size_t)n * out_ctot + out_c0 + 1) * Ho + Y) * Wo + X] = a1;
  }
}

}

using namespace fn2;

constexpr int kHeadG = 16;

static int head_splits(int N, int C, int H, int W) {
  const long long blocks = ((long long)order_batch(N) * H * W + kHeadPix - 1) / kHeadPix;
  int nsplit = 1;
  while (nsplit < 8 && blocks * kHeadG * nsplit < 4096 && C >= 8 * kHeadG * nsplit * 2) nsplit *= 2;
  return nsplit;
}

FN2_API size_t fn2_predict_flow_conv_workspace_bytes(int N, int C, int H, int W) {
  if (N < 1 || C < 1 || H < 1 || W < 1) return 0;
  return sizeof(float) * (size_t)head_splits(N, C, H, W) * N * 18 * H * W;
}

FN2_API int fn2_predict_flow_conv_forward(const float* in, const float* weight, const float* bias, float* out,
                                          int N, int C, int H, int W, void* workspace, size_t workspace_bytes, void* stream) {
  if (N < 0 || C < 1 || H < 1 || W < 1) return fail(FN2_ERR_INVALID_ARG, "predict_flow_conv: bad shape [%d,%d,%d,%d]", N, C, H, W);
  if (N == 0) return FN2_OK;
  if (!in || !weight || !out) return fail(FN2_ERR_INVALID_ARG, "predict_flow_conv: NULL blob pointer");
  if ((long long)H * W >= (1ll << 31) || 2ll * N > 65535) return fail(FN2_ERR_UNSUPPORTED, "predict_flow_conv: blob too large");
  const size_t need = fn2_predict_flow_conv_workspace_bytes(N, C, H, W);
  if (!workspace || workspace_bytes < need) return fail(FN2_ERR_WORKSPACE, "predict_flow_conv: workspace too small (%zu < %zu)", workspace_bytes, need);
  const long long total = (long long)N * H * W;
  const unsigned blocks = (unsigned)((total + kHeadPix - 1) / kHeadPix);
  const int nsplit = head_splits(N, C, H, W);
  hipStream_t st = as_stream(stream);
  float* P = reinterpret_cast<float*>(workspace);
  hipLaunchKernelGGL(conv3x3_c2_taps<kHeadG>, dim3(blocks, nsplit), dim3(kHeadPix * kHeadG), 0, st, in, weight, P, N, C, H, W, nsplit);
  const dim3 g2(((unsigned)H * W + 255) / 256, 2 * N);
  switch (nsplit) {
    case 1: hipLaunchKernelGGL(conv3x3_c2_gather<1>, g2, dim3(256), 0, st, P, bias, out, N, H, W); break;
    case 2: hipLaunchKernelGGL(conv3x3_c2_gather<2>, g2, dim3(256), 0, st, P, bias, out, N, H, W); break;
    case 4: hipLaunchKernelGGL(conv3x3_c2_gather<4>, g2, dim3(256), 0, st, P, bias, out, N, H, W); break;
    default: hipLaunchKernelGGL(conv3x3_c2_gather<8>, g2, dim3(256), 0, st, P, bias, out, N, H, W); break;
  }
  return check_launch("predict_flow_conv_forward");
}

FN2_API int fn2_upsample_flow_deconv_forward(const float* in, const float* weight, const float* bias, float* out,
                                             int N, int H, int W, void* stream) {
  if (N < 0 || H < 1 || W < 1) return fail(FN2_ERR_INVALID_ARG, "upsample_flow_deconv: bad shape");
  if (N == 0) return FN2_OK;
  if (!in || !weight || !out) return fail(FN2_ERR_INVALID_ARG, "upsample_flow_deconv: NULL blob pointer");
  const long long total = (long long)N * 4 * H * W;
  hipLaunchKernelGGL(deconv4x4s2_c2, dim3(blocks_for(total, 256, 4096)), dim3(256), 0, as_stream(stream), in, weight, bias, out, N, H, W, 2, 0);
  return check_launch("upsample_flow_deconv_forward");
}

FN2_API int fn2_upsample_flow_deconv_forward_into(const float* in, const float* weight, const float* bias, float* top,
                                                  int N, int H, int W, int top_channels, int top_c0, void* stream) {
  if (N < 0 || H < 1 || W < 1) return fail(FN2_ERR_INVALID_ARG, "upsample_flow_deconv: bad shape");
  if (top_c0 < 0 || top_c0 + 2 > top_channels) return fail(FN2_ERR_INVALID_ARG, "upsample_flow_deconv: channel slice outside the blob");
  if (N == 0) return FN2_OK;
  if (!in || !weight || !top) return fail(FN2_ERR_INVALID_ARG, "upsample_flow_deconv: NULL blob pointer");
  const long long total = (long long)N * 4 * H * W;
  hipLaunchKernelGGL(deconv4x4s2_c2, dim3(blocks_for(total, 256, 4096)), dim3(256), 0, as_stream(stream), in, weight, bias, top, N, H, W, top_channels, top_c0);
  return check_launch("upsample_flow_deconv_forward_into");
}
```

flownet2_amd/csrc/im2col.hip:

```cpp
#include "fn2_common.hpp"

namespace fn2 {

struct ColArgs {
  int C, H, W;
  int Hc, Wc;
  int k, pad, stride;
  float slope;
  int relu;
  int im_ctot, im_c0;
};

template <int K>
__global__ void __launch_bounds__(256) im2col_kernel(const float* __restrict__ im, float* __restrict__ col, ColArgs a) {
  const int kk = K > 0 ? K : a.k;
  const unsigned hwc = (unsigned)a.Hc * a.Wc;
  const unsigned plane = blockIdx.y;
  const float* src = im + (size_t)plane * a.H * a.W;
  float* dst = col + (size_t)plane * kk * kk * hwc;
  for (unsigned p = blockIdx.x * blockDim.x + threadIdx.x; p < hwc; p += gridDim.x * blockDim.x) {
    const int yc = p / a.Wc, xc = p % a.Wc;
    const int y0 = yc * a.stride - a.pad, x0 = xc * a.stride - a.pad;
    for (int i = 0; i < kk; ++i) {
      const int y = y0 + i;
      for (int j = 0; j < kk; ++j) {
        const int x = x0 + j;
        const bool in = y >= 0 && y < a.H && x >= 0 && x < a.W;
        dst[(size_t)(i * kk + j) * hwc + p] = in ? src[(size_t)y * a.W + x] : 0.f;
      }
    }
  }
}

__global__ void __launch_bounds__(256) col2im_bias_relu_kernel(const float* __restrict__ col, const float* __restrict__ bias,
                                                               float* __restrict__ im, ColArgs a) {
  const unsigned hw = (unsigned)a.H * a.W, hwc = (unsigned)a.Hc * a.Wc;
  const unsigned plane = blockIdx.y;
  const float* src = col + (size_t)plane * a.k * a.k * hwc;
  const float b = bias ? bias[plane % (unsigned)a.C] : 0.f;
  for (unsigned p = blockIdx.x * blockDim.x + threadIdx.x; p < hw; p += gridDim.x * blockDim.x) {
    const int y = p / a.W + a.pad, x = p % a.W + a.pad;
    const int yc_lo = y < a.k ? 0 : (y - a.k) / a.stride + 1, yc_hi = min(y / a.stride + 1, a.Hc);
    const int xc_lo = x < a.k ? 0 : (x - a.k) / a.stride + 1, xc_hi = min(x / a.stride + 1, a.Wc);
    float v = 0.f;
    for (int yc = yc_lo; yc < yc_hi; ++yc) {
      const int i = y - yc * a.stride;
      for (int xc = xc_lo; xc < xc_hi; ++xc) {
        const int j = x - xc * a.stride;
        v += src[(size_t)(i * a.k + j) * hwc + (unsigned)yc * a.Wc + xc];
      }
    }
    v += b;
    im[((size_t)(plane / (unsigned)a.C) * a.im_ctot + a.im_c0 + plane % (unsigned)a.C) * hw + p] = (a.relu && v <= 0.f) ? v * a.slope : v;
  }
}

__global__ void __launch_bounds__(256) col2im_k4s2p1_bias_relu_kernel(const float* __restrict__ col, const float* __restrict__ bias,
                                                                      float* __restrict__ im, ColArgs a) {
  const unsigned hw = (unsigned)a.H * a.W, hwc = (unsigned)a.Hc * a.Wc;
  const unsigned plane = blockIdx.y;
  const float* src = col + (size_t)plane * 16 * hwc;
  const float b = bias ? bias[plane % (unsigned)a.C] : 0.f;
  float* dst = im + ((size_t)(plane / (unsigned)a.C) * a.im_ctot + a.im_c0 + plane % (unsigned)a.C) * hw;
  for (unsigned p = blockIdx.x * blockDim.x + threadIdx.x; p < hwc; p += gridDim.x * blockDim.x) {
    const int yc0 = p / a.Wc, xc0 = p - yc0 * a.Wc;
    float t[4][4];
#pragma unroll
    for (int i = 0; i < 4; ++i) {
      const int yc = yc0 + (i == 3 ? -1 : i == 0 ? 1 : 0);
#pragma unroll
      for (int j = 0; j < 4; ++j) {
        const int xc = xc0 + (j == 3 ? -1 : j == 0 ? 1 : 0);
        const bool ok = yc >= 0 && yc < a.Hc && xc >= 0 && xc < a.Wc;
        t[i][j] = ok ? src[(size_t)(i * 4 + j) * hwc + (unsigned)yc * a.Wc + xc] : 0.f;
      }
    }
#pragma unroll
    for (int py = 0; py < 2; ++py) {
      const int i0 = py ? 2 : 3, i1 = py ? 0 : 1;
      float o[2];
#pragma unroll
      for (int px = 0; px < 2; ++px) {
        const int j0 = px ? 2 : 3, j1 = px ? 0 : 1;
        float v = 0.f;
        v += t[i0][j0]; v += t[i0][j1]; v += t[i1][j0]; v += t[i1][j1];
        v += b;
        o[px] = (a.relu && v <= 0.f) ? v * a.slope : v;
      }
      *reinterpret_cast<float2*>(dst + (size_t)(2 * yc0 + py) * a.W + 2 * xc0) = make_float2(o[0], o[1]);
    }
  }
}

static int col_geometry(const char* who, int N, int C, int H, int W, int k, int pad, int stride, ColArgs* a) {
  if (N < 0 || C <= 0 || H <= 0 || W <= 0 || k <= 0 || pad < 0 || stride <= 0)
    return fail(FN2_ERR_INVALID_ARG, "%s: bad arguments (N %d C %d H %d W %d kernel %d pad %d stride %d)", who, N, C, H, W, k, pad, stride);
  if (H + 2 * pad < k || W + 2 * pad < k) return fail(FN2_ERR_INVALID_ARG, "%s: kernel %d larger than the padded image", who, k);
  a->C = C; a->H = H; a->W = W; a->k = k; a->pad = pad; a->stride = stride;
  a->Hc = (H + 2 * pad - k) / stride + 1;
  a->Wc = (W + 2 * pad - k) / stride + 1;
  a->slope = 0.f; a->relu = 0; a->im_ctot = C; a->im_c0 = 0;
  if ((long long)N * C > 0x7fffffffll / 256 || (long long)H * W >= (1ll << 31) || (long long)k * k * a->Hc * a->Wc >= (1ll << 31))
    return fail(FN2_ERR_UNSUPPORTED, "%s: blob too large", who);
  return FN2_OK;
}

}

using namespace fn2;

FN2_API int fn2_im2col_forward(const float* im, float* col, int N, int C, int H, int W, int kernel, int pad, int stride, void* stream) {
  ColArgs a;
  int rc = col_geometry("im2col", N, C, H, W, kernel, pad, stride, &a);
  if (rc) return rc;
  if (N == 0) return FN2_OK;
  if (!im || !col) return fail(FN2_ERR_INVALID_ARG, "im2col: null blob");
  hipStream_t st = reinterpret_cast<hipStream_t>(stream);
  const unsigned hwc = (unsigned)a.Hc * a.Wc;
  unsigned bx = (hwc + 255) / 256; if (bx > 64) bx = 64;
  const long long planes = (long long)N * C;
  for (long long p0 = 0; p0 < planes; p0 += 65535) {
    const unsigned py = (unsigned)((planes - p0) < 65535 ? (planes - p0) : 65535);
    const float* s = im + (size_t)p0 * H * W;
    float* d = col + (size_t)p0 * kernel * kernel * hwc;
    if (kernel == 3) hipLaunchKernelGGL(im2col_kernel<3>, dim3(bx, py), dim3(256), 0, st, s, d, a);
    else             hipLaunchKernelGGL(im2col_kernel<0>, dim3(bx, py), dim3(256), 0, st, s, d, a);
  }
  return check_launch("im2col_forward");
}

static int col2im_launch(const float* col, const float* bias, float* im, int N, int C, int H, int W, int kernel, int pad, int stride,
                         int apply_relu, float negative_slope, int im_ctot, int im_c0, void* stream) {
  ColArgs a;
  int rc = col_geometry("col2im_bias_relu", N, C, H, W, kernel, pad, stride, &a);
  if (rc) return rc;
  if (im_c0 < 0 || im_c0 + C > im_ctot) return fail(FN2_ERR_INVALID_ARG, "col2im_bias_relu: channel slice outside the blob");
  if (N == 0) return FN2_OK;
  if (!im || !col) return fail(FN2_ERR_INVALID_ARG, "col2im_bias_relu: null blob");
  a.relu = apply_relu ? 1 : 0; a.slope = negative_slope; a.im_ctot = im_ctot; a.im_c0 = im_c0;
  hipStream_t st = reinterpret_cast<hipStream_t>(stream);
  const unsigned hw = (unsigned)H * W, hwc = (unsigned)a.Hc * a.Wc;
  unsigned bx = (hw + 255) / 256; if (bx > 64) bx = 64;
  const long long planes = (long long)N * C;
  const long long step = planes > 65535 ? ((65535 / C) > 0 ? (long long)(65535 / C) * C : 0) : planes;
  if (step == 0) return fail(FN2_ERR_UNSUPPORTED, "col2im_bias_relu: more than 65535 channels");
  const bool quad = kernel == 4 && stride == 2 && pad == 1 && H % 2 == 0 && W % 2 == 0 && (reinterpret_cast<uintptr_t>(im) & 7) == 0;
  unsigned bq = (hwc + 255) / 256; if (bq > 64) bq = 64;
  for (long long p0 = 0; p0 < planes; p0 += step) {
    const unsigned py = (unsigned)((planes - p0) < step ? (planes - p0) : step);
    if (quad) hipLaunchKernelGGL(col2im_k4s2p1_bias_relu_kernel, dim3(bq, py), dim3(256), 0, st, col + (size_t)p0 * kernel * kernel * hwc, bias,
                                 im + (size_t)(p0 / C) * im_ctot * hw, a);
    else hipLaunchKernelGGL(col2im_bias_relu_kernel, dim3(bx, py), dim3(256), 0, st, col + (size_t)p0 * kernel * kernel * hwc, bias,
                            im + (size_t)(p0 / C) * im_ctot * hw, a);
  }
  return check_launch("col2im_bias_relu_forward");
}

FN2_API int fn2_col2im_bias_relu_forward(const float* col, const float* bias, float* im, int N, int C, int H, int W,
                                         int kernel, int pad, int stride, int apply_relu, float negative_slope, void* stream) {
  return col2im_launch(col, bias, im, N, C, H, W, kernel, pad, stride, apply_relu, negative_slope, C, 0, stream);
}

FN2_API int fn2_col2im_bias_relu_forward_into(const float* col, const float* bias, float* top, int N, int C, int H, int W,
                                              int kernel, int pad, int stride, int apply_relu, float negative_slope,
                                              int top_channels, int top_c0, void* stream) {
  return col2im_launch(col, bias, top, N, C, H, W, kernel, pad, stride, apply_relu, negative_slope, top_channels, top_c0, stream);
}
```

flownet2_amd/functional.py:

```python
from __future__ import annotations

import collections
import os

import torch

from . import ops


_BATCH_INVARIANT = [False]


def set_batch_invariant(on: bool = True):
    _BATCH_INVARIANT[0] = bool(on)
    ops.set_batch_invariant(bool(on))


def batch_invariant() -> bool:
    return _BATCH_INVARIANT[0]


LIBRARY_FALLBACKS = [0]


# ... 724 lines not shown
                                                                                      "data " if lib_x else "", "weight" if lib_w else ""), flush=True)
    if lib_x or lib_w:
        if x.is_cuda:
            _note_fallback("%s backward{stride %d, pad %d}%s%s" % ("Deconvolution" if transposed else "Convolution", stride, pad,
                                                                   " data" if lib_x else "", " weight" if lib_w else ""), x, w)
        cd, was = torch.backends.cudnn, torch.backends.cudnn.deterministic
        cd.deterministic = True
        try:
            gxl, gwl, _ = torch.ops.aten.convolution_backward(d, x, w, None, [stride, stride], [pad, pad], [1, 1], transposed, [0, 0], 1,
                                                              [lib_x, lib_w, False])
        finally:
            cd.deterministic = was
        gx, gw = (gxl if lib_x else gx), (gwl if lib_w else gw)
    return gx, gw, db


def _layer_desc(w, stride, pad, transposed, x_shape=None, d_shape=None):
    k = int(w.shape[2])
    if w.shape[3] != k:
        return None
    Cin, Cout = (int(w.shape[0]), int(w.shape[1])) if transposed else (int(w.shape[1]), int(w.shape[0]))
    if x_shape is not None:
        N, H, W = int(x_shape[0]), int(x_shape[2]), int(x_shape[3])
    elif transposed and d_shape[2] % 2 == 0 and d_shape[3] % 2 == 0:
        N, H, W = int(d_shape[0]), int(d_shape[2]) // 2, int(d_shape[3]) // 2
    elif not transposed and stride == 1:
        N, H, W = int(d_shape[0]), int(d_shape[2]) - 1 + k - 2 * pad, int(d_shape[3]) - 1 + k - 2 * pad
    else:
        return None
    if H < 1 or W < 1:
        return None
    return ops.conv_desc(N, Cin, H, W, Cout, k, stride, pad)


def _own_bwd_weight(d, x, w, stride, pad, transposed):
    if not d.is_cuda:
        return None
    desc = _layer_desc(w, stride, pad, transposed, x_shape=x.shape)
    if desc is None or not ops.conv_backward_weights_supported(desc, transposed):
        return None
    if (not transposed and desc.kernel == 7) and not (d.is_contiguous() and x.is_contiguous()):
        d, x = d.contiguous(), x.contiguous()
    xb, x0 = _channel_slice(x)
    db, d0 = _channel_slice(d)
    return ops.conv_backward_weights(xb, db, desc, transposed, out=_grad_slot(w), bottom_c0=x0, top_c0=d0,
                                     bf16x3=not transposed and _bf16x3("wgrad"))


_PACKED_T = {}


def _cached_pack(cache, w, tag, make):
    return _cached(cache, (id(w), tag), w, make)


def _own_bwd_data(d, w, stride, pad, transposed, x_shape=None):
    if not d.is_cuda:
        return None
    desc = _layer_desc(w, stride, pad, transposed, x_shape=x_shape, d_shape=d.shape)
    if desc is None:
        return None
    route = ops.conv_backward_data_route(desc, transposed, bf16x3=_bf16x3("dgrad"))
    if route == 0:
        return None
    key = (desc.N, desc.Hin, desc.Win)
    packed = _cached_pack(_PACKED_T, w, ("dgrad", route, bool(transposed), stride, pad) + key,
                          lambda: ops.conv_backward_data_pack_weights(w.detach().contiguous(), desc, transposed, route))
    db, d0 = _channel_slice(d)
    return ops.conv_backward_data(db, packed, desc, transposed, route, top_c0=d0)


def _own_bwd_data_masked(d, w, stride, pad, x, slope):
    desc = _layer_desc(w, stride, pad, False, x_shape=x.shape)
    if desc is None or not d.is_cuda:
        return None
    route = ops.conv_backward_data_route(desc, False, bf16x3=_bf16x3("dgrad"))
    if route == 0 or not ops.conv_backward_data_masked_supported(desc, False, route):
        return None
    key = (desc.N, desc.Hin, desc.Win)
    packed = _cached_pack(_PACKED_T, w, ("dgrad", route, False, stride, pad) + key,
                          lambda: ops.conv_backward_data_pack_weights(w.detach().contiguous(), desc, False, route))
    db, d0 = _channel_slice(d)
    xb, x0 = _channel_slice(x)
    return ops.conv_backward_data_masked(db, packed, desc, False, route, xb, slope, top_c0=d0, data_c0=x0)


def _needs_grad(*ts):
    return torch.is_grad_enabled() and any(t is not None and t.requires_grad for t in ts)


def conv_forward_route(desc, act=True, whole_blobs=True) -> int:
    route = ops.conv_forward_route(desc, force=_ROUTE_FORCE[0], bf16x3=_bf16x3("conv"), wino_bf16x3=_bf16x3("wino"))
    stem = route == ops.CONV_ROUTE_STEM
    if route == ops.CONV_ROUTE_HEAD:
        return ops.CONV_ROUTE_NONE
    if stem and not (act and whole_blobs):
        return ops.CONV_ROUTE_NONE
    if desc.kernel not in (1, 3, 5, 7) or (desc.kernel == 7 and not stem and desc.Cin % 4 != 0):
        return ops.CONV_ROUTE_NONE
    return route


def deconv_forward_route(desc, act=True) -> int:
    if not act or desc.Cin < 64:
        return ops.DECONV_ROUTE_NONE
    route = ops.deconv_forward_route(desc, bf16x3=_bf16x3("deconv"))
    return ops.DECONV_ROUTE_NONE if route == ops.DECONV_ROUTE_HEAD else route


def conv_route_name(x_shape, w, stride, pad, act=True, whole_blobs=True):
    desc = _layer_desc(w, stride, pad, False, x_shape=x_shape)
    if desc is None:
        return None
    route = conv_forward_route(desc, act, whole_blobs)
    name = ops.CONV_FWD_ROUTES[route & ~ops.CONV_ARITH_BF16X3]
    return name + "+bf16x3" if name and route & ops.CONV_ARITH_BF16X3 else name


def conv_mfma_relu(x, weight, bias, stride, pad, negative_slope=0.1, act=True, out=None, out_c0=0, relu_chain=None):
    desc = _layer_desc(weight, stride, pad, False, x_shape=x.shape) if x.is_cuda else None
    route = conv_forward_route(desc, act, out is None) if desc is not None else ops.CONV_ROUTE_NONE
    if route == ops.CONV_ROUTE_NONE:
        return None
    if relu_chain is not None and int(relu_chain[0]) & 1 and route != ops.CONV_ROUTE_STEM:
        raise RuntimeError("relu_chain: only the stem layer is a chain producer")

    def run(xx, ww, bb, o=None, o0=0):
        if route == ops.CONV_ROUTE_STEM:
            blob, c0, packed = xx.contiguous(), 0, ww.detach().contiguous()
        else:
            blob, c0 = _channel_slice(xx)
            packed = _cached_pack(_PACKED_T, ww, ("fwd", route, False), lambda: ops.conv_pack_weights(ww.detach(), desc, route))
        return ops.conv_forward(blob, packed, bb, desc, route, False, act, negative_slope, out=o, out_c0=o0, in_c0=c0)

    if _needs_grad(x, weight, bias):
        return _OwnForwardConv.apply(x, weight, bias, run, stride, pad, negative_slope, act, False, None if out is None else (out, out_c0), relu_chain)
    return run(x, weight, bias, out, out_c0)


def deconv_relu(x, weight, bias, negative_slope=0.1, act=True, out=None, out_c0=0):
    desc = _layer_desc(weight, 2, 1, True, x_shape=x.shape) if x.is_cuda else None
    route = deconv_forward_route(desc, act) if desc is not None else ops.DECONV_ROUTE_NONE
    if route == ops.DECONV_ROUTE_NONE:
        return None

    def run(xx, ww, bb, o=None, o0=0):
        blob, c0 = _channel_slice(xx)
        packed = _cached_pack(_PACKED_T, ww, ("fwd", route, True), lambda: ops.conv_pack_weights(ww.detach(), desc, route, True))
        return ops.conv_forward(blob, packed, bb, desc, route, True, True, negative_slope, out=o, out_c0=o0, in_c0=c0)

    if _needs_grad(x, weight, bias):
        return _OwnForwardConv.apply(x, weight, bias, run, 2, 1, negative_slope, True, True, None if out is None else (out, out_c0))
    return run(x, weight, bias, out, out_c0)
```

flownet2_amd/graph_backend.py:

```python
from __future__ import annotations

import contextlib
import types

import torch.nn.functional as F

NEG_SLOPE = 0.1

_LISTENERS = []


@contextlib.contextmanager
def listening(fn):
    _LISTENERS.append(fn)
    try:
        yield fn
    finally:
        _LISTENERS.remove(fn)


def _declines(*args, **kwargs):
    return None


class GraphBackend:
    FORWARDED = ("correlation", "resample", "flow_warp", "channel_norm", "downsample", "l1_loss", "scale_shift", "resample_slices",
                 "flow_warp_slices", "channel_norm_slices", "l1_loss_multi", "downsample_ahead", "wait_ahead")

    def __init__(self, obj):
        get = lambda name: getattr(obj, name, None)
        self.obj = obj
        for name in self.FORWARDED:
            if get(name) is not None:
                setattr(self, name, get(name))
        self.own_conv, self.own_deconv = get("conv_mfma_relu") or _declines, get("deconv_relu") or _declines
        self.own_correlation_relu_into = get("correlation_relu_into") or _declines
        self._predict, self._upsample = get("predict_flow_conv"), get("upsample_flow_deconv")
        self._bias_act = get("conv_bias_leaky_relu")
        self._conv2d = get("lib_conv2d") or (lambda x, w, b, s, p: F.conv2d(x, w, b, stride=s, padding=p))
        self._deconv2d = get("lib_conv_transpose2d") or (lambda x, w, b, s, p: F.conv_transpose2d(x, w, b, stride=s, padding=p))
        self._act = get("leaky_relu") or (lambda y, slope, name: F.leaky_relu(y, slope))
        self.conv_route_name, self.relu_chain_supported = get("conv_route_name"), get("relu_chain_supported")
        self.writes_slices = self.own_conv is not _declines
        self.fuses_correlation = self.own_correlation_relu_into is not _declines
        self.has_slices = get("resample_slices") is not None
        self.has_scale_shift = get("scale_shift") is not None
        self.trains_in_place = get("conv_backward") is not None
        self.has_stem_chain = self.trains_in_place and self.conv_route_name is not None and self.relu_chain_supported is not None
        self.has_multi_loss = get("l1_loss_multi") is not None
        self.targets_ahead = get("downsample_ahead") is not None

    def __getattr__(self, name):
        if name in self.FORWARDED:
            return getattr(self.obj, name)
        raise AttributeError(name)

    def _ran(self, name, y, **info):
        for fn in list(_LISTENERS):
            fn(name, y, dict(info, backend=self))

    def wrote(self, kind, name, y, out, out_c0, channels, x, w=None, stride=1, pad=0):
        if _LISTENERS:
            self._ran(name, y if y.requires_grad else out[:, out_c0:out_c0 + channels], kind=kind, act=True, x=x, w=w, stride=stride, pad=pad,
                      own=True, into=True)

    def conv_wb(self, x, w, b, stride, pad, act=True, slope=NEG_SLOPE, name=None, relu_chain=None):
        y = self.own_conv(x, w, b, stride, pad, slope, act, relu_chain=relu_chain)
        own = y is not None
        if not own:
            if relu_chain is not None:
                raise RuntimeError("relu_chain: no own kernel takes this layer (its consumer was told the stem kernel would)")
            if act and self._bias_act is not None:
                y = self._bias_act(self._conv2d(x, w, None, stride, pad), b, slope)
            else:
                y = self._conv2d(x, w, b, stride, pad)
                if act:
                    y = self._act(y, slope, name)
        if _LISTENERS:
            self._ran(name, y, kind="conv", act=act, x=x, w=w, stride=stride, pad=pad, own=own, into=False)
        return y

    def conv(self, x, P, name, stride, pad, act=True, relu_chain=None):
        return self.conv_wb(x, P[name + ".w"], P[name + ".b"], stride, pad, act, NEG_SLOPE, name, relu_chain)

    def deconv_wb(self, x, w, b, act=True, slope=NEG_SLOPE, name=None):
        y = self.own_deconv(x, w, b, slope, act)
        own = y is not None
        if not own:
            if act and self._bias_act is not None:
                y = self._bias_act(self._deconv2d(x, w, None, 2, 1), b, slope)
            else:
                y = self._deconv2d(x, w, b, 2, 1)
                if act:
                    y = self._act(y, slope, name)
        if _LISTENERS:
            self._ran(name, y, kind="deconv", act=act, x=x, w=w, stride=2, pad=1, own=own, into=False)
        return y

    def deconv(self, x, P, name, act=True):
        return self.deconv_wb(x, P[name + ".w"], P[name + ".b"], act, NEG_SLOPE, name)

    def predict_flow(self, x, P, name):
        if self._predict is not None:
            return self._predict(x, P[name + ".w"], P[name + ".b"])
        return self.conv(x, P, name, 1, 1, act=False)

    def upsample_flow(self, x, P, name, out=None, out_c0=0):
        if self._upsample is None:
            return None if out is not None else self.deconv(x, P, name, act=False)
        if out is not None:
            return self._upsample(x, P[name + ".w"], P[name + ".b"], out=out, out_c0=out_c0)
        return self._upsample(x, P[name + ".w"], P[name + ".b"])

    def leaky_relu(self, x, name, slope=NEG_SLOPE):
        y = self._act(x, slope, name)
        if _LISTENERS:
            self._ran(name, y, kind="relu", act=True, x=x, own=False, into=False)
        return y


_MODULE_ADAPTERS = {}


def backend_of(obj) -> GraphBackend:
    if isinstance(obj, GraphBackend):
        return obj
    if obj is None or isinstance(obj, types.ModuleType):
        be = _MODULE_ADAPTERS.get(obj)
        if be is None:
            be = _MODULE_ADAPTERS[obj] = GraphBackend(obj)
        return be
    return GraphBackend(obj)
```

flownet2_amd/nets.py:

```python
from __future__ import annotations

import math
import os
from typing import Dict, Optional

import torch

from .graph_backend import NEG_SLOPE, GraphBackend, backend_of, listening

FLOW_SCALE = 20.0
SD_FLOW_SCALE = 0.05
LOSS_WEIGHTS = {6: 0.32, 5: 0.08, 4: 0.02, 3: 0.01, 2: 0.005}

_ENC_TAIL = [("conv4", 256, 512, 3, 2, 1), ("conv4_1", 512, 512, 3, 1, 1), ("conv5", 512, 512, 3, 2, 1),
             ("conv5_1", 512, 512, 3, 1, 1), ("conv6", 512, 1024, 3, 2, 1), ("conv6_1", 1024, 1024, 3, 1, 1)]
_DEC = [("Convolution1", "conv", 1024, 2), ("deconv5", "deconv", 1024, 512), ("upsample_flow6to5", "deconv", 2, 2),
        ("Convolution2", "conv", 1026, 2), ("deconv4", "deconv", 1026, 256), ("upsample_flow5to4", "deconv", 2, 2),
        ("Convolution3", "conv", 770, 2), ("deconv3", "deconv", 770, 128), ("upsample_flow4to3", "deconv", 2, 2),
        ("Convolution4", "conv", 386, 2), ("deconv2", "deconv", 386, 64), ("upsample_flow3to2", "deconv", 2, 2),
        ("Convolution5", "conv", 194, 2)]


def layer_table(kind: str = "C", in_channels: int = 6):
    t = []
    if kind == "C":
        t += [("conv1", "conv", 3, 64, 7, 2, 3), ("conv2", "conv", 64, 128, 5, 2, 2), ("conv3", "conv", 128, 256, 5, 2, 2),
              ("conv_redir", "conv", 256, 32, 1, 1, 0), ("conv3_1", "conv", 473, 256, 3, 1, 1)]
    else:
        t += [("conv1", "conv", in_channels, 64, 7, 2, 3), ("conv2", "conv", 64, 128, 5, 2, 2), ("conv3", "conv", 128, 256, 5, 2, 2),
              ("conv3_1", "conv", 256, 256, 3, 1, 1)]
    t += [(n, "conv", ci, co, k, s, p) for (n, ci, co, k, s, p) in _ENC_TAIL]
    for (n, k, ci, co) in _DEC:
        t.append((n, k, ci, co, 3, 1, 1) if k == "conv" else (n, k, ci, co, 4, 2, 1))
    return t


def init_params(kind: str = "C", seed: int = 0, device="cpu", in_channels: int = 6) -> Dict[str, torch.Tensor]:
    g = torch.Generator().manual_seed(seed)
    params = {}
    for (name, k, ci, co, ks, s, p) in layer_table(kind, in_channels):
        shape = (co, ci, ks, ks) if k == "conv" else (ci, co, ks, ks)
        fan_in = ci * ks * ks if k == "conv" else ci * ks * ks / (s * s)
        std = math.sqrt(2.0 / ((1 + NEG_SLOPE ** 2) * fan_in))
        if name.startswith("Convolution"):
            std *= 0.5
        if name.startswith("upsample_flow"):
            std = 0.25
        params[name + ".w"] = (torch.randn(shape, generator=g) * std).to(device)
        params[name + ".b"] = torch.zeros(co).to(device)
    return params


def num_params(params) -> int:
    return sum(int(v.numel()) for v in params.values())


def conv_forward(x, w, b, stride, pad, act, backend, slope=None, relu_chain=None):
    return backend_of(backend).conv_wb(x, w, b, stride, pad, act, NEG_SLOPE if slope is None else slope, relu_chain=relu_chain)


_LAST_ROUTE = [""]


def _note_route(name, y, info):
    if info["kind"] != "conv":
        return
    be, x, w = info["backend"], info["x"], info["w"]
    if not info["own"]:
        _LAST_ROUTE[0] = "library conv2d"
    elif be.conv_route_name is None:
        _LAST_ROUTE[0] = "own kernel"
    else:
        _LAST_ROUTE[0] = "fn2 %s" % be.conv_route_name(x.shape, w, info["stride"], info["pad"], info["act"], not info["into"])


def _trace_route(name, y, info):
    if info["kind"] == "conv":
        _note_route(name, y, info)
        print("conv route %-16s in %-22s k%d s%d act=%d -> %s%s" % (name, tuple(info["x"].shape), info["w"].shape[2], info["stride"], info["act"],
                                                                  _LAST_ROUTE[0], " (into its Concat blob)" if info["into"] else ""))


if os.environ.get("FN2_TRACE_CONV") == "1":
    listening(_trace_route).__enter__()


_CONSTS: Dict[tuple, torch.Tensor] = {}


def _const(device, values):
    key = (str(device), tuple(float(v) for v in values))
    if key not in _CONSTS:
        _CONSTS[key] = torch.tensor(key[1], device=device, dtype=torch.float32)
    return _CONSTS[key]


def deconv_forward(x, w, b, act=True, backend=None, slope=None):
    return backend_of(backend).deconv_wb(x, w, b, act, NEG_SLOPE if slope is None else slope)


def _conv_into_concat(x, P, name, stride, pad, extra_channels, be, relu_chain=None):
    w = P[name + ".w"]
    training = torch.is_grad_enabled() and (x.requires_grad or _any_requires_grad(P))
    if be.writes_slices and w.shape[2] in (3, 5) and (be.trains_in_place or not training):
        k = w.shape[2]
        ho, wo = (x.shape[2] + 2 * pad - k) // stride + 1, (x.shape[3] + 2 * pad - k) // stride + 1
        blob = torch.empty((x.shape[0], w.shape[0] + extra_channels, ho, wo), device=x.device, dtype=x.dtype)
        y = be.own_conv(x, w, P[name + ".b"], stride, pad, NEG_SLOPE, True, out=blob, out_c0=0, relu_chain=relu_chain)
        if y is not None:
            be.wrote("conv", name, y, blob, 0, w.shape[0], x, w, stride, pad)
            return blob, (y if (training and y.requires_grad) else blob[:, :w.shape[0]])
    if relu_chain is not None:
        raise RuntimeError("relu_chain: conv '%s' left the own-kernel route after its producer was told it would fold the ReLU derivative" % name)
    return None, be.conv(x, P, name, stride, pad)


def _any_requires_grad(P) -> bool:
    vals = P.P.values() if isinstance(P, _Prefixed) else P.values()
    return any(v.requires_grad for v in vals)


def _refine_stage(P, skip, x, dname, flow, uname, be):
    blob, s = skip if isinstance(skip, tuple) else (None, skip)
    if blob is None:
        return torch.cat([s, be.deconv(x, P, dname), be.upsample_flow(flow, P, uname)], 1)
    wd, bd = P[dname + ".w"], P[dname + ".b"]
    cs, cd = s.shape[1], wd.shape[1]
    assert blob.shape[1] == cs + cd + 2
    d = be.own_deconv(x, wd, bd, NEG_SLOPE, True, out=blob, out_c0=cs)
    if d is not None:
        be.wrote("deconv", dname, d, blob, cs, cd, x, wd, 2, 1)
    stage_params = [wd, bd, P[uname + ".w"], P[uname + ".b"]]
    if torch.is_grad_enabled() and (s.requires_grad or x.requires_grad or flow.requires_grad or any(p.requires_grad for p in stage_params)):
        u = be.upsample_flow(flow, P, uname, out=blob, out_c0=cs + cd) if d is not None else None
        if d is None or u is None:
            return torch.cat([s, be.deconv(x, P, dname), be.upsample_flow(flow, P, uname)], 1)
        part = lambda t, c0, c: t if t.requires_grad else blob[:, c0:c0 + c]
        return _ConcatInPlace.apply(blob, s, part(d, cs, cd), part(u, cs + cd, 2))
    if d is None:
        blob[:, cs:cs + cd].copy_(be.deconv(x, P, dname))
    if be.upsample_flow(flow, P, uname, out=blob, out_c0=cs + cd) is None:
        blob[:, cs + cd:].copy_(be.upsample_flow(flow, P, uname))
    return blob


def _decoder(P, conv6_1, conv5_1, conv4_1, conv3_1, conv2, be):
    flow6 = be.predict_flow(conv6_1, P, "Convolution1")
    c5 = _refine_stage(P, conv5_1, conv6_1, "deconv5", flow6, "upsample_flow6to5", be)
    flow5 = be.predict_flow(c5, P, "Convolution2")
    c4 = _refine_stage(P, conv4_1, c5, "deconv4", flow5, "upsample_flow5to4", be)
    flow4 = be.predict_flow(c4, P, "Convolution3")
    c3 = _refine_stage(P, conv3_1, c4, "deconv3", flow4, "upsample_flow4to3", be)
    flow3 = be.predict_flow(c3, P, "Convolution4")
    c2 = _refine_stage(P, conv2, c3, "deconv2", flow3, "upsample_flow3to2", be)
    flow2 = be.predict_flow(c2, P, "Convolution5")
    return {2: flow2, 3: flow3, 4: flow4, 5: flow5, 6: flow6}


def _skip_conv(x, P, name, stride, pad, dname, be, relu_chain=None):
    return _conv_into_concat(x, P, name, stride, pad, P[dname + ".w"].shape[1] + 2, be, relu_chain=relu_chain)


RELU_CHAIN = [True]


def _stem_chain(P, x, be):
    if not (RELU_CHAIN[0] and be.has_stem_chain and torch.is_grad_enabled() and x.is_cuda):
        return None, None
    w1, w2 = P["conv1.w"], P["conv2.w"]
    if not (w1.requires_grad and w2.requires_grad and P["conv1.b"].requires_grad) or x.requires_grad:
        return None, None
    if be.conv_route_name(x.shape, w1, 2, 3) != "stem":
        return None, None
    c1_shape = (x.shape[0], w1.shape[0], (x.shape[2] - 1) // 2 + 1, (x.shape[3] - 1) // 2 + 1)
    if not be.relu_chain_supported(c1_shape, w2, 2, 2):
        return None, None
    cell = {"masked": False, "slope": NEG_SLOPE}
    return (1, cell), (2, cell)


class _ConcatInPlace(torch.autograd.Function):

    @staticmethod
    def forward(ctx, blob, *parts):
        ctx.cuts = [p.shape[1] for p in parts]
        assert sum(ctx.cuts) == blob.shape[1] and all(p.data_ptr() >= blob.data_ptr() for p in parts)
        return blob.view_as(blob)

    @staticmethod
    def backward(ctx, g):
        out, c0 = [None], 0
        for c in ctx.cuts:
            out.append(g[:, c0:c0 + c])
            c0 += c
        return tuple(out)


class _SplitTowers(torch.autograd.Function):

    @staticmethod
    def forward(ctx, x):
        n = x.shape[0] // 2
        return x[:n], x[n:]

    @staticmethod
    def backward(ctx, ga, gb):
        return torch.cat([ga, gb], 0)


class _StackedAndFirstTower(torch.autograd.Function):

    @staticmethod
    def forward(ctx, x):
        return x.view_as(x), x[:x.shape[0] // 2]

    @staticmethod
    def backward(ctx, g_all, g_first):
        if g_all._base is not None or not g_all.is_contiguous():
            g_all = g_all.clone(memory_format=torch.contiguous_format)
        g_all[:g_first.shape[0]].add_(g_first)
        return g_all


_CORR = dict(pad=20, kernel_size=1, max_displacement=20, stride_1=1, stride_2=2)


def flownet_c_core(P, img0, img1, backend, towers=None):
    be = backend_of(backend)
    x = towers if towers is not None else torch.cat([img0, img1], 0)
    n = x.shape[0] // 2
    chain1, chain2 = _stem_chain(P, x, be)
    c1 = be.conv(x, P, "conv1", 2, 3, relu_chain=chain1)
    blob2, c2 = _skip_conv(c1, P, "conv2", 2, 2, "deconv2", be, relu_chain=chain2)
    training = torch.is_grad_enabled() and c2.requires_grad
    c2_first = None
    if training:
        c2, c2_first = _StackedAndFirstTower.apply(c2)
    c3 = be.conv(c2, P, "conv3", 2, 2)
    c3a, c3b = _SplitTowers.apply(c3) if (training and c3.requires_grad) else (c3[:n], c3[n:])
    wr, br = P["conv_redir.w"], P["conv_redir.b"]
    cr = wr.shape[0]
    cat = None
    if be.fuses_correlation:
        cat = torch.empty((n, cr + 441, c3a.shape[2], c3a.shape[3]), device=c3a.device, dtype=c3a.dtype)
        if be.trains_in_place and torch.is_grad_enabled() and (c3a.requires_grad or c3b.requires_grad):
            redir = be.own_conv(c3a, wr, br, 1, 0, NEG_SLOPE, True, out=cat, out_c0=0)
            if redir is not None:
                be.wrote("conv", "conv_redir", redir, cat, 0, cr, c3a, wr, 1, 0)
            corr = be.own_correlation_relu_into(c3a, c3b, cat, cr, NEG_SLOPE, training=True, **_CORR)
            be.wrote("relu", "relu", corr, cat, cr, 441, c3a)
            if redir is not None and redir.requires_grad:
                cat = _ConcatInPlace.apply(cat, redir, corr)
            else:
                cat = torch.cat([be.conv(c3a, P, "conv_redir", 1, 0), corr], 1)
        else:
            corr = be.own_correlation_relu_into(c3a, c3b, cat, cr, NEG_SLOPE, **_CORR)
            if corr is None:
                cat = None
            else:
                be.wrote("relu", "relu", corr, cat, cr, 441, c3a)
                redir = None
                if not (torch.is_grad_enabled() and _any_requires_grad(P)):
                    redir = be.own_conv(c3a, wr, br, 1, 0, NEG_SLOPE, True, out=cat, out_c0=0)
                if redir is None:
                    cat[:, :cr].copy_(be.conv(c3a, P, "conv_redir", 1, 0))
                else:
                    be.wrote("conv", "conv_redir", redir, cat, 0, cr, c3a, wr, 1, 0)
    if cat is None:
        redir = be.conv(c3a, P, "conv_redir", 1, 0)
        corr = be.correlation(c3a, c3b, **_CORR)
        cat = torch.cat([redir, be.leaky_relu(corr, "relu")], 1)
    blob3, c31 = _skip_conv(cat, P, "conv3_1", 1, 1, "deconv3", be)
    c4 = be.conv(c31, P, "conv4", 2, 1)
    blob4, c41 = _skip_conv(c4, P, "conv4_1", 1, 1, "deconv4", be)
    c5 = be.conv(c41, P, "conv5", 2, 1)
    blob5, c51 = _skip_conv(c5, P, "conv5_1", 1, 1, "deconv5", be)
    c6 = be.conv(c51, P, "conv6", 2, 1)
    c61 = be.conv(c6, P, "conv6_1", 1, 1)
    c2s = c2_first if c2_first is not None else c2[:n]
    skip2 = (blob2[:n], c2s) if blob2 is not None else c2s
    return _decoder(P, c61, (blob5, c51), (blob4, c41), (blob3, c31), skip2, be)


def flownet_s_core(P, x, backend=None):
    be = backend_of(backend)
    c1 = be.conv(x, P, "conv1", 2, 3)
    blob2, c2 = _skip_conv(c1, P, "conv2", 2, 2, "deconv2", be)
    c3 = be.conv(c2, P, "conv3", 2, 2)
    blob3, c31 = _skip_conv(c3, P, "conv3_1", 1, 1, "deconv3", be)
    c4 = be.conv(c31, P, "conv4", 2, 1)
    blob4, c41 = _skip_conv(c4, P, "conv4_1", 1, 1, "deconv4", be)
    c5 = be.conv(c41, P, "conv5", 2, 1)
    blob5, c51 = _skip_conv(c5, P, "conv5_1", 1, 1, "deconv5", be)
    c6 = be.conv(c51, P, "conv6", 2, 1)
    c61 = be.conv(c6, P, "conv6_1", 1, 1)
    return _decoder(P, c61, (blob5, c51), (blob4, c41), (blob3, c31), (blob2, c2), be)


def adapted_size(h: int, w: int, divisor: int = 64):
    return int(math.ceil(h / divisor) * divisor), int(math.ceil(w / divisor) * divisor)


def deploy_forward(kind: str, P, img0, img1, backend, mean: Optional[torch.Tensor] = None):
    backend = backend_of(backend)
    N, _, H, W = img0.shape
    ah, aw = adapted_size(H, W)
    neg_default = mean is None
    if mean is None:
        mean = _const(img0.device, (0.411, 0.433, 0.45))
# ... 350 lines not shown
```

flownet2_amd/ops.py:

```python
from __future__ import annotations

import ctypes as C

import torch

from . import _lib
from ._lib import CorrParams, L1LossParams, check


def _consts(*names):
    return tuple(_lib.CONSTANTS["FN2_" + n] for n in names)


MULTIPLY, SUBTRACT = _consts("CORR_MULTIPLY", "CORR_SUBTRACT")
FILL_ZERO, FILL_NAN = _consts("FILL_ZERO", "FILL_NAN")
NEAREST, LINEAR, CUBIC, AREA = _consts("RESAMPLE_NEAREST", "RESAMPLE_LINEAR", "RESAMPLE_CUBIC", "RESAMPLE_AREA")


def _stream():
    return C.c_void_p(torch.cuda.current_stream().cuda_stream)


def _chk(t: torch.Tensor, name: str, ndim: int = 4):
    if not isinstance(t, torch.Tensor) or not t.is_cuda:
# ... 396 lines not shown
            raise ValueError("scale_shift: top blob does not match the bottom")
    s = _chk_opt(shift, "shift", 1)
    check(_lib.lib().fn2_scale_shift_forward(_ptr(x), _ptr(out), _ptr(s), N, Cc, H, W, out.shape[1], out_c0, C.c_float(float(scale)), _stream()))
    return out


def predict_flow_conv_backward_supported(N, C, H, W) -> bool:
    return bool(_lib.lib().fn2_predict_flow_conv_backward_supported(int(N), int(C), int(H), int(W)))


def predict_flow_conv_backward(x, weight, top_diff, need_x=True, need_w=True, need_b=True):
    xb, xctot, xc0, Cc = _as_slice(x, "bottom[0]")
    w, g = _chk(weight, "weight"), _chk(top_diff, "top.diff")
    N, _, H, W = xb.shape
    if tuple(w.shape) != (2, Cc, 3, 3) or tuple(g.shape) != (N, 2, H, W):
        raise ValueError("predict_flow_conv_backward: weight must be [2,C,3,3] and top_diff [N,2,H,W]")
    dx = torch.empty((N, Cc, H, W), device=g.device, dtype=torch.float32) if need_x else None
    dw = torch.empty_like(w) if need_w else None
    db = torch.empty(2, device=g.device, dtype=torch.float32) if need_b else None
    nbytes = _lib.lib().fn2_predict_flow_conv_backward_workspace_bytes(N, Cc, H, W) if (need_w or need_b) else 0
    ws = torch.empty(max(nbytes, 4), dtype=torch.uint8, device=g.device)
    check(_lib.lib().fn2_predict_flow_conv_backward(_ptr(xb), xctot, xc0, _ptr(w), _ptr(g), _ptr(dx), _ptr(dw), _ptr(db), N, Cc, H, W, 0,
                                                    _ptr(ws), nbytes, _stream()))
    return dx, dw, db


def upsample_flow_deconv_backward(x, weight, top_diff, need_x=True, need_w=True, need_b=True):
    x, w, g = _chk(x, "bottom[0]"), _chk(weight, "weight"), _chk(top_diff, "top.diff")
    N, Cc, H, W = x.shape
    if Cc != 2 or tuple(w.shape) != (2, 2, 4, 4) or tuple(g.shape) != (N, 2, 2 * H, 2 * W):
        raise ValueError("upsample_flow_deconv_backward: bottom [N,2,H,W], weight [2,2,4,4], top_diff [N,2,2H,2W]")
    dx = torch.empty_like(x) if need_x else None
    dw = torch.empty_like(w) if need_w else None
    db = torch.empty(2, device=g.device, dtype=torch.float32) if need_b else None
    nbytes = _lib.lib().fn2_upsample_flow_deconv_backward_workspace_bytes(N, H, W) if (need_w or need_b) else 0
    ws = torch.empty(max(nbytes, 4), dtype=torch.uint8, device=g.device)
    check(_lib.lib().fn2_upsample_flow_deconv_backward(_ptr(x), _ptr(w), _ptr(g), _ptr(dx), _ptr(dw), _ptr(db), N, H, W, 0, _ptr(ws), nbytes, _stream()))
    return dx, dw, db


def conv_k7s2_relu_supported(Cin, Hin, Win, Cout) -> bool:
    return bool(_lib.lib().fn2_conv_k7s2_relu_supported(int(Cin), int(Hin), int(Win), int(Cout)))


def conv_k7s2_wgrad_supported(N, Cin, Hin, Win, Cout) -> bool:
    return bool(_lib.lib().fn2_conv_k7s2_wgrad_supported(int(N), int(Cin), int(Hin), int(Win), int(Cout)))


def conv_k7s2_wgrad_ksplit(N, Cin, Hin, Win, Cout) -> int:
    return int(_lib.lib().fn2_conv_k7s2_wgrad_ksplit(int(N), int(Cin), int(Hin), int(Win), int(Cout)))


def conv_k7s2_wgrad(top_diff, bottom):
    d, x = _chk(top_diff, "top.diff"), _chk(bottom, "bottom[0]")
    N, Cin, H, W = x.shape
    Cout = d.shape[1]
    if tuple(d.shape) != (N, Cout, (H - 1) // 2 + 1, (W - 1) // 2 + 1):
        raise ValueError(f"conv_k7s2_wgrad: top_diff {tuple(d.shape)} does not belong to a bottom of {tuple(x.shape)}")
    dw = torch.empty((Cout, Cin, 7, 7), device=x.device, dtype=torch.float32)
    ws, need = _scratch(x.device, _lib.lib().fn2_conv_k7s2_wgrad_workspace_bytes(N, Cin, H, W, Cout))
    check(_lib.lib().fn2_conv_k7s2_wgrad(_ptr(d), _ptr(x), _ptr(dw), N, Cin, H, W, Cout, 0, _ptr(ws), need, _stream()))
    return dw


def conv_k7s2_relu_forward(x, weight, bias=None, negative_slope=0.1):
    x, w = _chk(x, "bottom[0]"), _chk(weight, "weight")
    N, Cin, H, W = x.shape
    Cout = w.shape[0]
    if tuple(w.shape) != (Cout, Cin, 7, 7):
        raise ValueError(f"stem weight must be [Cout,{Cin},7,7], got {tuple(w.shape)}")
    b = _chk_opt(bias, "bias", 1)
    out = torch.empty((N, Cout, (H - 1) // 2 + 1, (W - 1) // 2 + 1), device=x.device, dtype=torch.float32)
    check(_lib.lib().fn2_conv_k7s2_relu_forward(_ptr(x), _ptr(w), _ptr(b), _ptr(out), N, Cin, H, W, Cout,
                                                C.c_float(float(negative_slope)), _stream()))
    return out


CONV_ROUTE_NONE, CONV_ROUTE_DIRECT, CONV_ROUTE_WINOGRAD, CONV_ROUTE_PLANE, CONV_ROUTE_STEM, CONV_ROUTE_HEAD = _consts(
    "CONV_ROUTE_NONE", "CONV_ROUTE_DIRECT", "CONV_ROUTE_WINOGRAD", "CONV_ROUTE_PLANE", "CONV_ROUTE_STEM", "CONV_ROUTE_HEAD")
DECONV_ROUTE_NONE, DECONV_ROUTE_GEMM, DECONV_ROUTE_PLANE, DECONV_ROUTE_HEAD = _consts("DECONV_ROUTE_NONE", "DECONV_ROUTE_GEMM", "DECONV_ROUTE_PLANE",
                                                                                      "DECONV_ROUTE_HEAD")
ROUTE_FORCE, ROUTE_BF16X3, ROUTE_WINO_BF16X3 = _consts("ROUTE_FORCE", "ROUTE_BF16X3", "ROUTE_WINO_BF16X3")
CONV_ARITH_BF16X3, = _consts("CONV_ARITH_BF16X3")
CONV_FWD_ROUTES = {0: None, 1: "direct", 2: "wino", 3: "plane", 4: "stem", 5: "head"}
DECONV_FWD_ROUTES = {0: None, 1: "gemm", 2: "plane", 3: "head"}
CONV_ROUTES = {0: None, 1: "direct", 2: "wino", 3: "plane", 4: None, 5: None}
DECONV_ROUTES = {0: None, 1: "gemm", 2: "plane", 3: None}


def conv_route(N, Cin, Hin, Win, Cout, kernel, stride, pad, force=False):
    return CONV_ROUTES[conv_forward_route(conv_desc(N, Cin, Hin, Win, Cout, kernel, stride, pad), force)]


def deconv_route(N, Cin, Hin, Win, Cout, kernel=4, stride=2, pad=1):
    return DECONV_ROUTES[deconv_forward_route(conv_desc(N, Cin, Hin, Win, Cout, kernel, stride, pad))]


BWD_ROUTES = {0: None, 1: "wino", 2: "tconv", 3: "plane", 4: "direct", 5: "deconv_plane"}


def conv_desc(N, Cin, Hin, Win, Cout, kernel, stride, pad):
    return _lib.ConvDesc(int(N), int(Cin), int(Hin), int(Win), int(Cout), int(kernel), int(stride), int(pad))


def conv_forward_route(desc, force=False, bf16x3=False, wino_bf16x3=False) -> int:
    flags = (ROUTE_FORCE if force else 0) | (ROUTE_BF16X3 if bf16x3 else 0) | (ROUTE_WINO_BF16X3 if wino_bf16x3 else 0)
    return int(_lib.lib().fn2_conv_route(C.byref(desc), flags))


def deconv_forward_route(desc, bf16x3=False) -> int:
    return int(_lib.lib().fn2_deconv_route(C.byref(desc), ROUTE_BF16X3 if bf16x3 else 0))


def conv_pack_weights(weight, desc, route, transposed=False):
    w = _chk(weight, "weight")
    L = _lib.lib()
    floats, pack = (L.fn2_deconv_packed_weight_floats, L.fn2_deconv_pack_weights) if transposed else (L.fn2_conv_packed_weight_floats, L.fn2_conv_pack_weights)
    n = int(floats(C.byref(desc), int(route)))
    k = desc.kernel
    if n == 0 or tuple(w.shape) != ((desc.Cin, desc.Cout, k, k) if transposed else (desc.Cout, desc.Cin, k, k)):
        raise ValueError("conv_pack_weights: route %d has no operand for a weight of shape %s" % (route, tuple(w.shape)))
    packed = torch.empty(n, device=w.device, dtype=torch.float32)
    check(pack(C.byref(desc), int(route), _ptr(w), _ptr(packed), _stream()))
    return packed


def conv_forward(x, packed, bias, desc, route, transposed=False, relu=True, negative_slope=0.1, out=None, out_c0=0, in_c0=0):
    x = _chk(x, "bottom[0]")
    N, Ctot, H, W = x.shape
    k, s, p = desc.kernel, desc.stride, desc.pad
    if (N, H, W) != (desc.N, desc.Hin, desc.Win) or in_c0 < 0 or in_c0 + desc.Cin > Ctot:
        raise ValueError(f"conv_forward: bottom blob {tuple(x.shape)} does not hold the layer's [{desc.N},{desc.Cin},{desc.Hin},{desc.Win}] at channel {in_c0}")
    Ho, Wo = (2 * H, 2 * W) if transposed else ((H + 2 * p - k) // s + 1, (W + 2 * p - k) // s + 1)
    if out is None:
        out = torch.empty((N, desc.Cout, Ho, Wo), device=x.device, dtype=torch.float32)
    else:
        _chk(out, "top[0]")
        if not out.is_contiguous() or out.shape[0] != N or tuple(out.shape[2:]) != (Ho, Wo) or out_c0 < 0 or out_c0 + desc.Cout > out.shape[1]:
            raise ValueError(f"conv_forward: top blob {tuple(out.shape)} does not match [{N},>={out_c0 + desc.Cout},{Ho},{Wo}]")
    b = _chk(bias, "bias", ndim=1) if bias is not None else None
    pw = _chk(packed, "packed weight", ndim=None)
    L = _lib.lib()
    if pw.numel() != int((L.fn2_deconv_packed_weight_floats if transposed else L.fn2_conv_packed_weight_floats)(C.byref(desc), int(route))):
        raise ValueError("conv_forward: the operand has %d floats, not what route %d reads for this layer" % (pw.numel(), route))
    need = int((L.fn2_deconv_workspace_bytes if transposed else L.fn2_conv_workspace_bytes)(C.byref(desc), int(route)))
    if transposed and (route & ~CONV_ARITH_BF16X3) == DECONV_ROUTE_GEMM:
        ws = torch.empty((need + 3) // 4, device=x.device, dtype=torch.float32)
    else:
        ws = _plane_workspace(x.device, need) if need else None
    check((L.fn2_deconv_forward if transposed else L.fn2_conv_forward)(
        C.byref(desc), int(route), _ptr(x), Ctot, int(in_c0), _ptr(pw), _ptr(b), _ptr(out), out.shape[1], int(out_c0),
        int(bool(relu)), C.c_float(float(negative_slope)), _ptr(ws), need, _stream()))
    return out


def conv_backward_data_route(desc, transposed=False, bf16x3=False) -> int:
    if not bf16x3:
        return int(_lib.lib().fn2_conv_backward_data_route(C.byref(desc), int(bool(transposed))))
    return int(_lib.lib().fn2_conv_backward_data_route_flags(C.byref(desc), int(bool(transposed)), ROUTE_BF16X3))


def _check_dgrad_operand(what, packed, desc, tr, route):
    n = int(_lib.lib().fn2_conv_backward_data_packed_weight_floats(C.byref(desc), tr, int(route)))
    if n == 0:
        raise ValueError("%s: route %d is not this layer's" % (what, route))
    if packed.numel() != n:
        raise ValueError("%s: the operand has %d floats, route %d of this layer needs %d (packed for another route?)" % (what, packed.numel(), route, n))


def conv_backward_data_pack_weights(weight, desc, transposed, route):
    w = _chk(weight, "weight")
    L, tr = _lib.lib(), int(bool(transposed))
    n = int(L.fn2_conv_backward_data_packed_weight_floats(C.byref(desc), tr, int(route)))
    if n == 0:
        raise ValueError("conv_backward_data_pack_weights: route %d is not this layer's" % route)
    packed = torch.empty(n, device=w.device, dtype=torch.float32)
    need = int(L.fn2_conv_backward_data_pack_workspace_bytes(C.byref(desc), tr, int(route)))
    ws = torch.empty(need // 4, device=w.device, dtype=torch.float32) if need else None
    check(L.fn2_conv_backward_data_pack_weights(C.byref(desc), tr, int(route), _ptr(w), _ptr(packed), _ptr(ws), need, _stream()))
    return packed


def conv_backward_data(top_diff, packed_weight, desc, transposed, route, top_c0=0):
    d = _chk(top_diff, "top_diff")
    L, tr = _lib.lib(), int(bool(transposed))
    Cp = int(L.fn2_conv_backward_data_computed_channels(C.byref(desc), tr, int(route)))
    if Cp == 0:
        raise ValueError("conv_backward_data: route %d is not this layer's" % route)
    _check_dgrad_operand("conv_backward_data", packed_weight, desc, tr, route)
    out = torch.empty((desc.N, Cp, desc.Hin, desc.Win), device=d.device, dtype=torch.float32)
    need = int(L.fn2_conv_backward_data_workspace_bytes_with_room(C.byref(desc), tr, int(route), Cp))
    ws = _plane_workspace(d.device, need) if need else None
    check(L.fn2_conv_backward_data(C.byref(desc), tr, int(route), _ptr(d), d.shape[1], int(top_c0), _ptr(packed_weight), _ptr(out), Cp, 0, Cp,
                                   _ptr(ws), need, _stream()))
    return out[:, :desc.Cin] if Cp != desc.Cin else out


def conv_backward_weights_supported(desc, transposed=False) -> bool:
    return bool(_lib.lib().fn2_conv_backward_weights_supported(C.byref(desc), int(bool(transposed))))


def conv_backward_weights_arith(desc, transposed=False, bf16x3=False) -> int:
    return int(_lib.lib().fn2_conv_backward_weights_arith(C.byref(desc), int(bool(transposed)), ROUTE_BF16X3 if bf16x3 else 0))


def conv_backward_weights(bottom, top_diff, desc, transposed=False, out=None, accumulate=False, bottom_c0=0, top_c0=0, bf16x3=False):
    x, d = _chk(bottom, "bottom"), _chk(top_diff, "top_diff")
    L, tr = _lib.lib(), int(bool(transposed))
    k = desc.kernel
    shape = (desc.Cin, desc.Cout, k, k) if transposed else (desc.Cout, desc.Cin, k, k)
    if out is None:
        out = torch.empty(shape, device=x.device, dtype=torch.float32)
        accumulate = False
    else:
        out = _chk(out, "weight diff")
        if tuple(out.shape) != shape:
            raise ValueError("conv_backward_weights: weight diff has the wrong shape")
    arith = conv_backward_weights_arith(desc, transposed, True) if bf16x3 else 0
    if arith:
        need = int(L.fn2_conv_backward_weights_workspace_bytes_arith(C.byref(desc), tr, arith))
        ws = _plane_workspace(x.device, need) if need else None
        check(L.fn2_conv_backward_weights_arith_run(C.byref(desc), tr, arith, _ptr(x), x.shape[1], int(bottom_c0), _ptr(d), d.shape[1], int(top_c0),
                                                    _ptr(out), int(bool(accumulate)), _ptr(ws), need, _stream()))
        return out
    need = int(L.fn2_conv_backward_weights_workspace_bytes(C.byref(desc), tr))
    ws = _plane_workspace(x.device, need) if need else None
    check(L.fn2_conv_backward_weights(C.byref(desc), tr, _ptr(x), x.shape[1], int(bottom_c0), _ptr(d), d.shape[1], int(top_c0), _ptr(out),
                                      int(bool(accumulate)), _ptr(ws), need, _stream()))
    return out


def conv_backward_data_masked_supported(desc, transposed, route) -> bool:
    return bool(_lib.lib().fn2_conv_backward_data_masked_supported(C.byref(desc), int(bool(transposed)), int(route)))


def conv_backward_data_masked(top_diff, packed, desc, transposed, route, bottom_data, negative_slope, top_c0=0, data_c0=0):
    d, y = _chk(top_diff, "top_diff"), _chk(bottom_data, "bottom data")
    _check_dgrad_operand("conv_backward_data_masked", packed, desc, int(bool(transposed)), route)
    out = torch.empty((desc.N, desc.Cin, desc.Hin, desc.Win), device=d.device, dtype=torch.float32)
    check(_lib.lib().fn2_conv_backward_data_masked(C.byref(desc), int(bool(transposed)), int(route), _ptr(d), d.shape[1], int(top_c0), _ptr(packed),
                                                   _ptr(out), desc.Cin, 0, _ptr(y), y.shape[1], int(data_c0), C.c_float(float(negative_slope)), _stream()))
    return out


def conv_backward_weights_bias_fused(desc, transposed=False) -> bool:
    return bool(_lib.lib().fn2_conv_backward_weights_bias_fused(C.byref(desc), int(bool(transposed))))


def conv_backward_weights_bias(bottom, top_diff, desc, transposed=False, out=None):
    x, d = _chk(bottom, "bottom"), _chk(top_diff, "top_diff")
    L, tr = _lib.lib(), int(bool(transposed))
    k = desc.kernel
    dw = out if out is not None else torch.empty((desc.Cout, desc.Cin, k, k), device=x.device, dtype=torch.float32)
    db = torch.empty(desc.Cout, device=x.device, dtype=torch.float32)
    need = int(L.fn2_conv_backward_weights_workspace_bytes(C.byref(desc), tr))
    ws = _plane_workspace(x.device, need) if need else None
    check(L.fn2_conv_backward_weights_bias(C.byref(desc), tr, _ptr(x), _ptr(d), _ptr(dw), _ptr(db), 0, _ptr(ws), need, _stream()))
    return dw, db


def conv_backward_bias(top_diff, C_, top_c0=0, out=None, accumulate=False):
    d = _chk(top_diff, "top_diff")
    N, Ctot, H, W = d.shape
    if out is None:
        out = torch.empty(C_, device=d.device, dtype=torch.float32)
        accumulate = False
    need = int(_lib.lib().fn2_bias_leaky_relu_backward_workspace_bytes(N, C_, H, W))
    ws = _plane_workspace(d.device, need)
    check(_lib.lib().fn2_conv_backward_bias(_ptr(d), Ctot, int(top_c0), _ptr(out), N, int(C_), H, W, int(bool(accumulate)), _ptr(ws), need, _stream()))
    return out


def conv_general_supported(desc, transposed=False) -> bool:
    return bool(_lib.lib().fn2_conv_general_supported(C.byref(desc), int(bool(transposed))))


def set_conv_general_groups(groups: int = 0):
    check(_lib.lib().fn2_debug_set_conv_general_groups(int(groups)))


def conv_general_sizes(desc, transposed=False):
    n = [C.c_size_t() for _ in range(4)]
    check(_lib.lib().fn2_conv_general_sizes(C.byref(desc), int(bool(transposed)), *(C.byref(v) for v in n)))
    return tuple(int(v.value) for v in n)


def conv_general_out_shape(desc, transposed=False):
    k, s, p = desc.kernel, desc.stride, desc.pad
    if transposed:
        return s * (desc.Hin - 1) + k - 2 * p, s * (desc.Win - 1) + k - 2 * p
    return (desc.Hin + 2 * p - k) // s + 1, (desc.Win + 2 * p - k) // s + 1


def _general_weight_shape(desc, transposed):
    k = desc.kernel
    return (desc.Cin, desc.Cout, k, k) if transposed else (desc.Cout, desc.Cin, k, k)


def conv_general_pack_weights(weight, desc, transposed=False, backward=False):
    w = _chk(weight, "weight")
    if tuple(w.shape) != _general_weight_shape(desc, transposed):
        raise ValueError("conv_general_pack_weights: weight of shape %s is not this layer's" % (tuple(w.shape),))
    packed = torch.empty(conv_general_sizes(desc, transposed)[1 if backward else 0], device=w.device, dtype=torch.float32)
    check(_lib.lib().fn2_conv_general_pack_weights(C.byref(desc), int(bool(transposed)), 1 if backward else 0, _ptr(w), _ptr(packed), _stream()))
    return packed

# ... 484 lines not shown
```

Baseline: 3597.

## Fuse flow-head gather and upsample into deconv second pass in decoder stages

Adds a decoder stage-finish path. The predict_flow tap gather plus the 4x4 flow upsample into the concat blob now run as extra workgroups inside the deconvolution's second pass: the plane K-split reduction or the col2im finish. This removes separate small kernel launches for predict_flow and upsample per refinement level. It also adds two 1x1 MFMA conv variants. The path is on by default through an environment flag, falls back when unsupported, and adds code complexity plus a risk of load imbalance inside the fused kernels.

```diff
diff --git a/flownet2_amd/_lib.py b/flownet2_amd/_lib.py
--- a/flownet2_amd/_lib.py
+++ b/flownet2_amd/_lib.py
@@ -88,7 +88,7 @@
 
 def _parse_headers():
     per_header, structs, constants = [], {}, {}
-    for h in ("flownet2_hip.h", "flownet2_hip_solver.h", "flownet2_hip_corr_route.h", "flownet2_hip_conv_general.h"):
+    for h in ("flownet2_hip.h", "flownet2_hip_solver.h", "flownet2_hip_corr_route.h", "flownet2_hip_conv_general.h", "flownet2_hip_decoder.h"):
         with open(os.path.join(INCLUDE_DIR, h)) as f:
             functions, structs, c = parse_header(f.read(), structs)
         per_header.append(functions)
@@ -97,7 +97,7 @@
 
 
 _PER_HEADER, _STRUCTS, CONSTANTS = _parse_headers()
-EXPORTS, SOLVER_EXPORTS, CORR_ROUTE_EXPORTS, CONV_GENERAL_EXPORTS = (list(f) for f in _PER_HEADER)
+EXPORTS, SOLVER_EXPORTS, CORR_ROUTE_EXPORTS, CONV_GENERAL_EXPORTS, DECODER_EXPORTS = (list(f) for f in _PER_HEADER)
 PROTOTYPES = {name: proto for f in _PER_HEADER for name, proto in f.items()}
 globals().update({cls.__name__: cls for cls in _STRUCTS.values()})
 _HOOKS = parse_header("""
diff --git a/flownet2_amd/csrc/conv_mfma.hip b/flownet2_amd/csrc/conv_mfma.hip
--- a/flownet2_amd/csrc/conv_mfma.hip
+++ b/flownet2_amd/csrc/conv_mfma.hip
@@ -346,7 +346,8 @@
   FN2_CV_PIN(1, 1, 2, 7, 2, 2, 1, 8, 1, 1) FN2_CV_PIN(1, 1, 2, 3, 2, 2, 1, 8, 1, 1)
   FN2_CV_PIN(3, 1, 2, 7, 2, 2, 1, 2, 0, 1) FN2_CV_PIN(3, 1, 2, 6, 2, 2, 1, 2, 0, 1) FN2_CV_PIN(3, 2, 2, 7, 2, 1, 2, 2, 0, 1) FN2_CV_PIN(3, 2, 2, 6, 2, 2, 1, 2, 0, 1)
   FN2_CV_PIN(4, 2, 2, 7, 2, 2, 1, 2, 0, 1) FN2_CV_PIN(4, 2, 2, 6, 2, 2, 1, 2, 0, 1) FN2_CV_PIN(5, 2, 2, 6, 2, 2, 1, 1, 0, 1)
-  FN2_CV_PIN(7, 2, 2, 6, 2, 2, 1, 1, 0, 1) FN2_CV_PIN(7, 2, 4, 6, 1, 2, 2, 1, 0, 0)};
+  FN2_CV_PIN(7, 2, 2, 6, 2, 2, 1, 1, 0, 1) FN2_CV_PIN(7, 2, 4, 6, 1, 2, 2, 1, 0, 0)
+  FN2_CV_ROW16(2, 2, 1, 4, 1, 0) FN2_CV_ROW16(2, 1, 1, 4, 1, 0)};
 constexpr int kNumVariants = sizeof(kVariants) / sizeof(kVariants[0]);
 
 int g_forced_variant = -1;
diff --git a/flownet2_amd/csrc/conv_plane.hip b/flownet2_amd/csrc/conv_plane.hip
--- a/flownet2_amd/csrc/conv_plane.hip
+++ b/flownet2_amd/csrc/conv_plane.hip
@@ -1,4 +1,5 @@
 #include "mfma_tile.hpp"
+#include "stage_finish.hpp"
 
 namespace fn2 {
 namespace cp {
@@ -225,10 +226,11 @@
 }
 
 template <int KS>
-__global__ void __launch_bounds__(256) plane_reduce(const float* __restrict__ part, const float* __restrict__ bias, float* __restrict__ out,
-                                                    int N, int Cout, int P, int out_ctot, int out_c0, int ksplit, int relu, float slope) {
+__device__ __forceinline__ void plane_reduce_body(const float* __restrict__ part, const float* __restrict__ bias, float* __restrict__ out,
+                                                  int N, int Cout, int P, int out_ctot, int out_c0, int ksplit, int relu, float slope,
+                                                  unsigned bx, unsigned nbx) {
   const unsigned total = (unsigned)N * (unsigned)Cout * (unsigned)P;
-  for (unsigned i = blockIdx.x * blockDim.x + threadIdx.x; i < total; i += gridDim.x * blockDim.x) {
+  for (unsigned i = bx * blockDim.x + threadIdx.x; i < total; i += nbx * blockDim.x) {
     float s;
     if constexpr (KS > 0) {
       float v[KS];
@@ -255,6 +257,24 @@
     if (relu) s = s > 0.f ? s : s * slope;
     out[((size_t)n * out_ctot + out_c0 + co) * P + pix] = s;
   }
+}
+
+template <int KS>
+__global__ void __launch_bounds__(256) plane_reduce(const float* __restrict__ part, const float* __restrict__ bias, float* __restrict__ out,
+                                                    int N, int Cout, int P, int out_ctot, int out_c0, int ksplit, int relu, float slope) {
+  plane_reduce_body<KS>(part, bias, out, N, Cout, P, out_ctot, out_c0, ksplit, relu, slope, blockIdx.x, gridDim.x);
+}
+
+template <int KS>
+__global__ void __launch_bounds__(256) plane_reduce_finish(const float* __restrict__ part, const float* __restrict__ bias, float* __restrict__ out,
+                                                           int N, int Cout, int P, int out_ctot, int out_c0, int ksplit, int relu, float slope,
+                                                           StageHead h) {
+  __shared__ float tile[2][kStageHalo][kStageHalo];
+  if (blockIdx.x < h.nwg) {
+    stage_head_workgroup<0>(h, blockIdx.x, tile);
+    return;
+  }
+  plane_reduce_body<KS>(part, bias, out, N, Cout, P, out_ctot, out_c0, ksplit, relu, slope, blockIdx.x - h.nwg, gridDim.x - h.nwg);
 }
 
 template <int SK>
@@ -383,8 +403,11 @@
   return rounds * v.mw * v.np / eff;
 }
 
-static int forward(Args a, int mode, int stride, int ks, void* workspace, size_t workspace_bytes, const char* what, hipStream_t st) {
+static int forward(Args a, int mode, int stride, int ks, void* workspace, size_t workspace_bytes, const char* what, hipStream_t st,
+                   const StageHead* head = nullptr) {
   const int Po = a.Hout * a.Wout;
+  if (head && (a.ksplit <= 1 || (long long)a.N * a.Cout * Po >= (1ll << 31) || head->nwg >= (1u << 30)))
+    return fail(FN2_ERR_UNSUPPORTED, "%s: no part reduction to carry the flow head (K parts: %d)", what, a.ksplit);
   if (a.ksplit > 1) {
     const size_t need = sizeof(float) * (size_t)a.ksplit * a.N * a.Cout * Po;
     if (!workspace || workspace_bytes < need) return fail(FN2_ERR_WORKSPACE, "%s: workspace of %zu bytes needed", what, need);
@@ -416,8 +439,11 @@
   if (a.ksplit > 1) {
     const long long total = (long long)a.N * a.Cout * Po;
     if (total >= (1ll << 31)) return fail(FN2_ERR_UNSUPPORTED, "%s: blob too large for the part reduction", what);
-    const dim3 rg(blocks_for(total, 256, 4096));
-#define FN2_PR(KS_) hipLaunchKernelGGL(plane_reduce<KS_>, rg, dim3(256), 0, st, a.part, a.bias, a.out, a.N, a.Cout, Po, a.out_ctot, a.out_c0, a.ksplit, a.relu, a.slope)
+    const dim3 rg(blocks_for(total, 256, 4096)), fg(rg.x + (head ? head->nwg : 0u));
+#define FN2_PR(KS_)                                                                                                                                \
+  if (head) hipLaunchKernelGGL(plane_reduce_finish<KS_>, fg, dim3(256), 0, st, a.part, a.bias, a.out, a.N, a.Cout, Po, a.out_ctot, a.out_c0, a.ksplit, \
+                               a.relu, a.slope, *head);                                                                                            \
+  else hipLaunchKernelGGL(plane_reduce<KS_>, rg, dim3(256), 0, st, a.part, a.bias, a.out, a.N, a.Cout, Po, a.out_ctot, a.out_c0, a.ksplit, a.relu, a.slope)
     switch (a.ksplit) {
       case 2: FN2_PR(2); break;
       case 3: FN2_PR(3); break;
@@ -588,10 +614,10 @@
   return fn2_deconv_plane_pack_weights_k(weight, packed, Cin, Cout, 4, stream);
 }
 
-FN2_API int fn2_deconv_plane_forward(const float* bottom, const float* packed_weight, const float* bias, float* top,
-                                     int N, int Cin, int Hin, int Win, int bottom_channels, int bottom_c0,
-                                     int Cout, int top_channels, int top_c0, int relu, float negative_slope,
-                                     void* workspace, size_t workspace_bytes, void* stream) {
+static int deconv_plane_run(const float* bottom, const float* packed_weight, const float* bias, float* top,
+                            int N, int Cin, int Hin, int Win, int bottom_channels, int bottom_c0,
+                            int Cout, int top_channels, int top_c0, int relu, float negative_slope,
+                            void* workspace, size_t workspace_bytes, void* stream, const StageHead* head) {
   if (N < 0) return fail(FN2_ERR_INVALID_ARG, "deconv_plane: bad batch");
   if (N == 0) return FN2_OK;
   if (!bottom || !packed_weight || !top) return fail(FN2_ERR_INVALID_ARG, "deconv_plane: null blob");
@@ -607,5 +633,20 @@
   a.in = bottom; a.wp = packed_weight; a.bias = bias; a.out = top;
   a.in_ctot = bottom_channels; a.in_c0 = bottom_c0; a.out_ctot = top_channels; a.out_c0 = top_c0;
   a.slope = negative_slope; a.relu = relu;
-  return cp::forward(a, 1, 1, 4, workspace, workspace_bytes, "deconv_plane", as_stream(stream));
-}
+  return cp::forward(a, 1, 1, 4, workspace, workspace_bytes, "deconv_plane", as_stream(stream), head);
+}
+
+FN2_API int fn2_deconv_plane_forward(const float* bottom, const float* packed_weight, const float* bias, float* top,
+                                     int N, int Cin, int Hin, int Win, int bottom_channels, int bottom_c0,
+                                     int Cout, int top_channels, int top_c0, int relu, float negative_slope,
+                                     void* workspace, size_t workspace_bytes, void* stream) {
+  return deconv_plane_run(bottom, packed_weight, bias, top, N, Cin, Hin, Win, bottom_channels, bottom_c0, Cout, top_channels, top_c0, relu,
+                          negative_slope, workspace, workspace_bytes, stream, nullptr);
+}
+
+int fn2::deconv_plane_stage_forward(const float* bottom, const float* packed_weight, const float* bias, float* top, int N, int Cin, int Hin, int Win,
+                                    int bottom_channels, int bottom_c0, int Cout, int top_channels, int top_c0, int relu, float negative_slope,
+                                    void* workspace, size_t workspace_bytes, const StageHead& head, void* stream) {
+  return deconv_plane_run(bottom, packed_weight, bias, top, N, Cin, Hin, Win, bottom_channels, bottom_c0, Cout, top_channels, top_c0, relu,
+                          negative_slope, workspace, workspace_bytes, stream, &head);
+}
diff --git a/flownet2_amd/csrc/conv_route.cpp b/flownet2_amd/csrc/conv_route.cpp
--- a/flownet2_amd/csrc/conv_route.cpp
+++ b/flownet2_amd/csrc/conv_route.cpp
@@ -1,5 +1,7 @@
+#include "../../include/flownet2_hip_decoder.h"
 #include "conv_internal.hpp"
 #include "fn2_common.hpp"
+#include "stage_finish.hpp"
 
 namespace {
 
@@ -234,6 +236,46 @@
                    d->kernel, d->stride, d->pad, d->Cin, d->Cout, d->Hin, d->Win);
 }
 
+FN2_API int fn2_deconv_flow_stage_forward(const fn2_conv_desc* d, int route, const float* bottom, int bottom_channels, int bottom_c0,
+                                          const float* packed_weight, const float* bias, float* top, int top_channels, int top_c0,
+                                          int relu, float negative_slope, void* workspace, size_t workspace_bytes,
+                                          const float* head_taps, size_t head_taps_bytes, int head_N, int head_C, int head_H, int head_W,
+                                          const float* head_bias, float* flow, const float* upsample_weight, const float* upsample_bias, void* stream) {
+  if (!valid(d)) return fn2::fail(FN2_ERR_INVALID_ARG, "deconv_flow_stage: bad descriptor");
+  const bool gemm = route == FN2_DECONV_ROUTE_GEMM || route == (FN2_DECONV_ROUTE_GEMM | FN2_CONV_ARITH_BF16X3);
+  if (!deconv_route_applies(d, route) || !(gemm || route == FN2_DECONV_ROUTE_PLANE))
+    return fn2::fail(FN2_ERR_UNSUPPORTED, "deconv_flow_stage: no stage finish for Deconvolution{kernel %d, stride %d, pad %d} %d -> %d on %d x %d (route %d)",
+                     d->kernel, d->stride, d->pad, d->Cin, d->Cout, d->Hin, d->Win, route);
+  if (!bottom || !packed_weight || !top || !head_taps || !flow || !upsample_weight) return fn2::fail(FN2_ERR_INVALID_ARG, "deconv_flow_stage: NULL blob");
+  if (bottom_c0 < 0 || bottom_c0 + d->Cin > bottom_channels || top_c0 < 0 || top_c0 + d->Cout + 2 > top_channels)
+    return fn2::fail(FN2_ERR_INVALID_ARG, "deconv_flow_stage: channel slice outside its blob");
+  if (head_N != d->N || head_C < 1 || head_H != d->Hin || head_W != d->Win)
+    return fn2::fail(FN2_ERR_INVALID_ARG, "deconv_flow_stage: a head on [%d,%d,%d,%d] is not the level above [%d,*,%d,%d]", head_N, head_C, head_H, head_W,
+                     d->N, d->Hin, d->Win);
+  if (head_taps_bytes < fn2_predict_flow_conv_workspace_bytes(head_N, head_C, head_H, head_W))
+    return fn2::fail(FN2_ERR_WORKSPACE, "deconv_flow_stage: the head's per-tap image has %zu bytes, not %zu", head_taps_bytes,
+                     fn2_predict_flow_conv_workspace_bytes(head_N, head_C, head_H, head_W));
+  const fn2::StageHead head = fn2::stage_head(head_taps, head_bias, flow, upsample_weight, upsample_bias, top, d->N, d->Hin, d->Win,
+                                              fn2::predict_flow_head_splits(head_N, head_C, head_H, head_W), top_channels, top_c0 + d->Cout);
+  if (route == FN2_DECONV_ROUTE_PLANE) {
+    if (fn2_deconv_plane_ksplit(d->N, d->Cin, d->Hin, d->Win, d->Cout) <= 1)
+      return fn2::fail(FN2_ERR_UNSUPPORTED, "deconv_flow_stage: the small-map kernel does not split K here: no second pass to carry the head");
+    return fn2::deconv_plane_stage_forward(bottom, packed_weight, bias, top, d->N, d->Cin, d->Hin, d->Win, bottom_channels, bottom_c0, d->Cout,
+                                           top_channels, top_c0, relu, negative_slope, workspace, workspace_bytes, head, stream);
+  }
+  if ((reinterpret_cast<uintptr_t>(top) & 7) != 0)
+    return fn2::fail(FN2_ERR_UNSUPPORTED, "deconv_flow_stage: the 2 x 2 second pass needs an 8-byte aligned top");
+  if (!workspace || workspace_bytes < fn2_deconv_workspace_bytes(d, route))
+    return fn2::fail(FN2_ERR_INVALID_ARG, "deconv_flow_stage: workspace of %zu bytes needed for the column matrix", fn2_deconv_workspace_bytes(d, route));
+  float* col = static_cast<float*>(workspace);
+  int rc = route != FN2_DECONV_ROUTE_GEMM
+               ? fn2::deconv_bf16x3_gemm(bottom, packed_weight, col, d->N, d->Cin, d->Hin, d->Win, bottom_channels, bottom_c0, d->Cout, stream)
+               : fn2_conv_mfma_forward(bottom, packed_weight, nullptr, col, d->N, d->Cin, d->Hin, d->Win, bottom_channels, bottom_c0, d->Cout * 16,
+                                       d->Cout * 16, 0, 1, 1, 0, 0, 0.f, stream);
+  if (rc) return rc;
+  return fn2::col2im_stage_finish(col, bias, top, d->N, d->Cout, 2 * d->Hin, 2 * d->Win, relu, negative_slope, top_channels, top_c0, head, stream);
+}
+
 namespace {
 
 inline int round_up(int v, int m) { return (v + m - 1) / m * m; }
diff --git a/flownet2_amd/csrc/flow_head.hip b/flownet2_amd/csrc/flow_head.hip
--- a/flownet2_amd/csrc/flow_head.hip
+++ b/flownet2_amd/csrc/flow_head.hip
@@ -1,4 +1,7 @@
+#include "../../include/flownet2_hip_decoder.h"
+#include "flow_head_device.hpp"
 #include "fn2_common.hpp"
+#include "stage_finish.hpp"
 
 namespace fn2 {
 
@@ -64,25 +67,7 @@
   const int y = pix / W, x = pix - y * W;
   const unsigned no = blockIdx.y;
   const unsigned n = no >> 1, o = no & 1;
-  float v[NSPLIT][9];
-#pragma unroll
-  for (int sp = 0; sp < NSPLIT; ++sp) {
-    const float* Pn = P + (((size_t)sp * N + n) * 18 + o * 9) * plane;
-#pragma unroll
-    for (int dy = 0; dy < 3; ++dy)
-#pragma unroll
-      for (int dx = 0; dx < 3; ++dx) {
-        const int yy = y + dy - 1, xx = x + dx - 1;
-        const bool ok = yy >= 0 && yy < H && xx >= 0 && xx < W;
-        v[sp][dy * 3 + dx] = ok ? Pn[(size_t)(dy * 3 + dx) * plane + (unsigned)yy * W + xx] : 0.f;
-      }
-  }
-  float sacc = bias ? bias[o] : 0.f;
-#pragma unroll
-  for (int sp = 0; sp < NSPLIT; ++sp)
-#pragma unroll
-    for (int t = 0; t < 9; ++t) sacc += v[sp][t];
-  out[(size_t)no * plane + pix] = sacc;
+  out[(size_t)no * plane + pix] = head_gather_value<NSPLIT>(P, bias, N, H, W, n, o, y, x);
 }
 
 __global__ void __launch_bounds__(256) deconv4x4s2_c2(const float* __restrict__ in, const float* __restrict__ w,
@@ -92,25 +77,8 @@
   const long long total = (long long)N * Ho * Wo;
   for (long long idx = blockIdx.x * (long long)blockDim.x + threadIdx.x; idx < total; idx += (long long)gridDim.x * blockDim.x) {
     const int X = (int)(idx % Wo), Y = (int)((idx / Wo) % Ho), n = (int)(idx / ((long long)Wo * Ho));
-    float a0 = bias ? bias[0] : 0.f, a1 = bias ? bias[1] : 0.f;
-#pragma unroll
-    for (int ty = 0; ty < 2; ++ty) {
-      const int ky = ((Y + 1) & 1) + 2 * ty;
-      const int iy = (Y + 1 - ky) / 2;
-      if (Y + 1 - ky < 0 || iy >= H) continue;
-#pragma unroll
-      for (int tx = 0; tx < 2; ++tx) {
-        const int kx = ((X + 1) & 1) + 2 * tx;
-        const int ix = (X + 1 - kx) / 2;
-        if (X + 1 - kx < 0 || ix >= W) continue;
-#pragma unroll
-        for (int c = 0; c < 2; ++c) {
-          const float v = in[(((size_t)n * 2 + c) * H + iy) * W + ix];
-          a0 = fmaf(w[((c * 2 + 0) * 4 + ky) * 4 + kx], v, a0);
-          a1 = fmaf(w[((c * 2 + 1) * 4 + ky) * 4 + kx], v, a1);
-        }
-      }
-    }
+    float a0, a1;
+    head_upsample_value([&](int c, int iy, int ix) { return in[(((size_t)n * 2 + c) * H + iy) * W + ix]; }, w, bias, H, W, Y, X, a0, a1);
     out[(((size_t)n * out_ctot + out_c0 + 0) * Ho + Y) * Wo + X] = a0;
     out[(((size_t)n * out_ctot + out_c0 + 1) * Ho + Y) * Wo + X] = a1;
   }
@@ -134,20 +102,41 @@
   return sizeof(float) * (size_t)head_splits(N, C, H, W) * N * 18 * H * W;
 }
 
-FN2_API int fn2_predict_flow_conv_forward(const float* in, const float* weight, const float* bias, float* out,
-                                          int N, int C, int H, int W, void* workspace, size_t workspace_bytes, void* stream) {
+int fn2::predict_flow_head_splits(int N, int C, int H, int W) { return head_splits(N, C, H, W); }
+
+static int taps_checks(const float* in, const float* weight, int N, int C, int H, int W, void* workspace, size_t workspace_bytes) {
   if (N < 0 || C < 1 || H < 1 || W < 1) return fail(FN2_ERR_INVALID_ARG, "predict_flow_conv: bad shape [%d,%d,%d,%d]", N, C, H, W);
   if (N == 0) return FN2_OK;
-  if (!in || !weight || !out) return fail(FN2_ERR_INVALID_ARG, "predict_flow_conv: NULL blob pointer");
+  if (!in || !weight) return fail(FN2_ERR_INVALID_ARG, "predict_flow_conv: NULL blob pointer");
   if ((long long)H * W >= (1ll << 31) || 2ll * N > 65535) return fail(FN2_ERR_UNSUPPORTED, "predict_flow_conv: blob too large");
   const size_t need = fn2_predict_flow_conv_workspace_bytes(N, C, H, W);
   if (!workspace || workspace_bytes < need) return fail(FN2_ERR_WORKSPACE, "predict_flow_conv: workspace too small (%zu < %zu)", workspace_bytes, need);
+  return FN2_OK;
+}
+
+static void launch_taps(const float* in, const float* weight, float* P, int N, int C, int H, int W, int nsplit, hipStream_t st) {
   const long long total = (long long)N * H * W;
   const unsigned blocks = (unsigned)((total + kHeadPix - 1) / kHeadPix);
+  hipLaunchKernelGGL(conv3x3_c2_taps<kHeadG>, dim3(blocks, nsplit), dim3(kHeadPix * kHeadG), 0, st, in, weight, P, N, C, H, W, nsplit);
+}
+
+FN2_API int fn2_predict_flow_conv_taps(const float* in, const float* weight, int N, int C, int H, int W, void* workspace, size_t workspace_bytes,
+                                       void* stream) {
+  if (const int rc = taps_checks(in, weight, N, C, H, W, workspace, workspace_bytes)) return rc;
+  if (N == 0) return FN2_OK;
+  launch_taps(in, weight, reinterpret_cast<float*>(workspace), N, C, H, W, head_splits(N, C, H, W), as_stream(stream));
+  return check_launch("predict_flow_conv_taps");
+}
+
+FN2_API int fn2_predict_flow_conv_forward(const float* in, const float* weight, const float* bias, float* out,
+                                          int N, int C, int H, int W, void* workspace, size_t workspace_bytes, void* stream) {
+  if (N > 0 && C >= 1 && H >= 1 && W >= 1 && !out) return fail(FN2_ERR_INVALID_ARG, "predict_flow_conv: NULL blob pointer");
+  if (const int rc = taps_checks(in, weight, N, C, H, W, workspace, workspace_bytes)) return rc;
+  if (N == 0) return FN2_OK;
   const int nsplit = head_splits(N, C, H, W);
   hipStream_t st = as_stream(stream);
   float* P = reinterpret_cast<float*>(workspace);
-  hipLaunchKernelGGL(conv3x3_c2_taps<kHeadG>, dim3(blocks, nsplit), dim3(kHeadPix * kHeadG), 0, st, in, weight, P, N, C, H, W, nsplit);
+  launch_taps(in, weight, P, N, C, H, W, nsplit, st);
   const dim3 g2(((unsigned)H * W + 255) / 256, 2 * N);
   switch (nsplit) {
     case 1: hipLaunchKernelGGL(conv3x3_c2_gather<1>, g2, dim3(256), 0, st, P, bias, out, N, H, W); break;
diff --git a/flownet2_amd/csrc/flow_head_device.hpp b/flownet2_amd/csrc/flow_head_device.hpp
--- /dev/null
+++ b/flownet2_amd/csrc/flow_head_device.hpp
@@ -0,0 +1,119 @@
+#pragma once
+
+#include <hip/hip_runtime.h>
+
+namespace fn2 {
+
+template <int NSPLIT>
+__device__ __forceinline__ float head_gather_value(const float* __restrict__ P, const float* __restrict__ bias, int N, int H, int W,
+                                                   unsigned n, unsigned o, int y, int x) {
+  const unsigned plane = (unsigned)H * W;
+  float v[NSPLIT][9];
+#pragma unroll
+  for (int sp = 0; sp < NSPLIT; ++sp) {
+    const float* Pn = P + (((size_t)sp * N + n) * 18 + o * 9) * plane;
+#pragma unroll
+    for (int dy = 0; dy < 3; ++dy)
+#pragma unroll
+      for (int dx = 0; dx < 3; ++dx) {
+        const int yy = y + dy - 1, xx = x + dx - 1;
+        const bool ok = yy >= 0 && yy < H && xx >= 0 && xx < W;
+        v[sp][dy * 3 + dx] = ok ? Pn[(size_t)(dy * 3 + dx) * plane + (unsigned)yy * W + xx] : 0.f;
+      }
+  }
+  float sacc = bias ? bias[o] : 0.f;
+#pragma unroll
+  for (int sp = 0; sp < NSPLIT; ++sp)
+#pragma unroll
+    for (int t = 0; t < 9; ++t) sacc += v[sp][t];
+  return sacc;
+}
+
+template <class In>
+__device__ __forceinline__ void head_upsample_value(In in, const float* __restrict__ w, const float* __restrict__ bias, int H, int W, int Y, int X,
+                                                    float& a0, float& a1) {
+  a0 = bias ? bias[0] : 0.f;
+  a1 = bias ? bias[1] : 0.f;
+#pragma unroll
+  for (int ty = 0; ty < 2; ++ty) {
+    const int ky = ((Y + 1) & 1) + 2 * ty;
+    const int iy = (Y + 1 - ky) / 2;
+    if (Y + 1 - ky < 0 || iy >= H) continue;
+#pragma unroll
+    for (int tx = 0; tx < 2; ++tx) {
+      const int kx = ((X + 1) & 1) + 2 * tx;
+      const int ix = (X + 1 - kx) / 2;
+      if (X + 1 - kx < 0 || ix >= W) continue;
+#pragma unroll
+      for (int c = 0; c < 2; ++c) {
+        const float v = in(c, iy, ix);
+        a0 = fmaf(w[((c * 2 + 0) * 4 + ky) * 4 + kx], v, a0);
+        a1 = fmaf(w[((c * 2 + 1) * 4 + ky) * 4 + kx], v, a1);
+      }
+    }
+  }
+}
+
+constexpr int kStageTile = 16;
+constexpr int kStageHalo = kStageTile + 2;
+
+struct StageHead {
+  const float* P;
+  const float* bias;
+  float* flow;
+  const float* up_w;
+  const float* up_b;
+  float* top;
+  int N, H, W, nsplit, top_ctot, top_c0;
+  int tiles_x, tiles_y;
+  unsigned nwg;
+};
+
+inline StageHead stage_head(const float* P, const float* bias, float* flow, const float* up_w, const float* up_b, float* top, int N, int H, int W,
+                            int nsplit, int top_ctot, int top_c0) {
+  StageHead h{P, bias, flow, up_w, up_b, top, N, H, W, nsplit, top_ctot, top_c0, 0, 0, 0u};
+  h.tiles_x = (W + kStageTile - 1) / kStageTile;
+  h.tiles_y = (H + kStageTile - 1) / kStageTile;
+  h.nwg = (unsigned)N * h.tiles_y * h.tiles_x;
+  return h;
+}
+
+template <int NSPLIT>
+__device__ __forceinline__ void stage_head_workgroup(const StageHead& h, unsigned wg, float (*tile)[kStageHalo][kStageHalo]) {
+  const unsigned per = (unsigned)h.tiles_x * h.tiles_y;
+  const unsigned n = wg / per, r = wg - n * per;
+  const int y0 = (int)(r / h.tiles_x) * kStageTile, x0 = (int)(r % h.tiles_x) * kStageTile;
+  const int H = h.H, W = h.W;
+  for (int i = threadIdx.x; i < 2 * kStageHalo * kStageHalo; i += 256) {
+    const int o = i / (kStageHalo * kStageHalo), q = i - o * (kStageHalo * kStageHalo);
+    const int ly = q / kStageHalo, lx = q - ly * kStageHalo;
+    const int y = y0 + ly - 1, x = x0 + lx - 1;
+    float v = 0.f;
+    if (y >= 0 && y < H && x >= 0 && x < W) {
+      if constexpr (NSPLIT > 0) {
+        v = head_gather_value<NSPLIT>(h.P, h.bias, h.N, H, W, n, o, y, x);
+      } else {
+        switch (h.nsplit) {
+          case 1: v = head_gather_value<1>(h.P, h.bias, h.N, H, W, n, o, y, x); break;
+          case 2: v = head_gather_value<2>(h.P, h.bias, h.N, H, W, n, o, y, x); break;
+          case 4: v = head_gather_value<4>(h.P, h.bias, h.N, H, W, n, o, y, x); break;
+          default: v = head_gather_value<8>(h.P, h.bias, h.N, H, W, n, o, y, x); break;
+        }
+      }
+      if (ly >= 1 && ly <= kStageTile && lx >= 1 && lx <= kStageTile) h.flow[(((size_t)n * 2 + o) * H + y) * W + x] = v;
+    }
+    tile[o][ly][lx] = v;
+  }
+  __syncthreads();
+  const int Ho = 2 * H, Wo = 2 * W;
+  for (int i = threadIdx.x; i < 4 * kStageTile * kStageTile; i += 256) {
+    const int Y = 2 * y0 + i / (2 * kStageTile), X = 2 * x0 + i % (2 * kStageTile);
+    if (Y >= Ho || X >= Wo) continue;
+    float a0, a1;
+    head_upsample_value([&](int c, int iy, int ix) { return tile[c][iy - y0 + 1][ix - x0 + 1]; }, h.up_w, h.up_b, H, W, Y, X, a0, a1);
+    h.top[(((size_t)n * h.top_ctot + h.top_c0 + 0) * Ho + Y) * Wo + X] = a0;
+    h.top[(((size_t)n * h.top_ctot + h.top_c0 + 1) * Ho + Y) * Wo + X] = a1;
+  }
+}
+
+}
diff --git a/flownet2_amd/csrc/im2col.hip b/flownet2_amd/csrc/im2col.hip
--- a/flownet2_amd/csrc/im2col.hip
+++ b/flownet2_amd/csrc/im2col.hip
@@ -1,4 +1,6 @@
+#include "flow_head_device.hpp"
 #include "fn2_common.hpp"
+#include "stage_finish.hpp"
 
 namespace fn2 {
 
@@ -55,14 +57,13 @@
   }
 }
 
-__global__ void __launch_bounds__(256) col2im_k4s2p1_bias_relu_kernel(const float* __restrict__ col, const float* __restrict__ bias,
-                                                                      float* __restrict__ im, ColArgs a) {
+__device__ __forceinline__ void col2im_k4s2p1_body(const float* __restrict__ col, const float* __restrict__ bias, float* __restrict__ im,
+                                                   const ColArgs& a, unsigned plane, unsigned bx, unsigned nbx) {
   const unsigned hw = (unsigned)a.H * a.W, hwc = (unsigned)a.Hc * a.Wc;
-  const unsigned plane = blockIdx.y;
   const float* src = col + (size_t)plane * 16 * hwc;
   const float b = bias ? bias[plane % (unsigned)a.C] : 0.f;
   float* dst = im + ((size_t)(plane / (unsigned)a.C) * a.im_ctot + a.im_c0 + plane % (unsigned)a.C) * hw;
-  for (unsigned p = blockIdx.x * blockDim.x + threadIdx.x; p < hwc; p += gridDim.x * blockDim.x) {
+  for (unsigned p = bx * blockDim.x + threadIdx.x; p < hwc; p += nbx * blockDim.x) {
     const int yc0 = p / a.Wc, xc0 = p - yc0 * a.Wc;
     float t[4][4];
 #pragma unroll
@@ -90,6 +91,23 @@
       *reinterpret_cast<float2*>(dst + (size_t)(2 * yc0 + py) * a.W + 2 * xc0) = make_float2(o[0], o[1]);
     }
   }
+}
+
+__global__ void __launch_bounds__(256) col2im_k4s2p1_bias_relu_kernel(const float* __restrict__ col, const float* __restrict__ bias,
+                                                                      float* __restrict__ im, ColArgs a) {
+  col2im_k4s2p1_body(col, bias, im, a, blockIdx.y, blockIdx.x, gridDim.x);
+}
+
+template <int NSPLIT>
+__global__ void __launch_bounds__(256) col2im_k4s2p1_finish_kernel(const float* __restrict__ col, const float* __restrict__ bias,
+                                                                   float* __restrict__ im, ColArgs a, StageHead h, unsigned head_rows) {
+  __shared__ float tile[2][kStageHalo][kStageHalo];
+  if (blockIdx.y < head_rows) {
+    const unsigned wg = blockIdx.y * gridDim.x + blockIdx.x;
+    if (wg < h.nwg) stage_head_workgroup<NSPLIT>(h, wg, tile);
+    return;
+  }
+  col2im_k4s2p1_body(col, bias, im, a, blockIdx.y - head_rows, blockIdx.x, gridDim.x);
 }
 
 static int col_geometry(const char* who, int N, int C, int H, int W, int k, int pad, int stride, ColArgs* a) {
@@ -130,7 +148,7 @@
 }
 
 static int col2im_launch(const float* col, const float* bias, float* im, int N, int C, int H, int W, int kernel, int pad, int stride,
-                         int apply_relu, float negative_slope, int im_ctot, int im_c0, void* stream) {
+                         int apply_relu, float negative_slope, int im_ctot, int im_c0, void* stream, const StageHead* head = nullptr) {
   ColArgs a;
   int rc = col_geometry("col2im_bias_relu", N, C, H, W, kernel, pad, stride, &a);
   if (rc) return rc;
@@ -142,13 +160,25 @@
   const unsigned hw = (unsigned)H * W, hwc = (unsigned)a.Hc * a.Wc;
   unsigned bx = (hw + 255) / 256; if (bx > 64) bx = 64;
   const long long planes = (long long)N * C;
-  const long long step = planes > 65535 ? ((65535 / C) > 0 ? (long long)(65535 / C) * C : 0) : planes;
-  if (step == 0) return fail(FN2_ERR_UNSUPPORTED, "col2im_bias_relu: more than 65535 channels");
   const bool quad = kernel == 4 && stride == 2 && pad == 1 && H % 2 == 0 && W % 2 == 0 && (reinterpret_cast<uintptr_t>(im) & 7) == 0;
   unsigned bq = (hwc + 255) / 256; if (bq > 64) bq = 64;
+  if (head && !quad) return fail(FN2_ERR_UNSUPPORTED, "col2im stage finish: only the 4x4 / 2 / 1 pass on even maps and an 8-byte aligned top carries the flow head");
+  const unsigned head_rows = head ? (head->nwg + bq - 1) / bq : 0u;
+  if (head_rows >= 32768) return fail(FN2_ERR_UNSUPPORTED, "col2im stage finish: flow map too large");
+  const long long ymax = 65535 - (long long)head_rows;
+  const long long step = planes > ymax ? ((ymax / C) > 0 ? (ymax / C) * C : 0) : planes;
+  if (step == 0) return fail(FN2_ERR_UNSUPPORTED, "col2im_bias_relu: more than 65535 channels");
   for (long long p0 = 0; p0 < planes; p0 += step) {
     const unsigned py = (unsigned)((planes - p0) < step ? (planes - p0) : step);
-    if (quad) hipLaunchKernelGGL(col2im_k4s2p1_bias_relu_kernel, dim3(bq, py), dim3(256), 0, st, col + (size_t)p0 * kernel * kernel * hwc, bias,
+    if (head && p0 == 0) {
+      const dim3 fg(bq, head_rows + py);
+      switch (head->nsplit) {
+        case 1: hipLaunchKernelGGL(col2im_k4s2p1_finish_kernel<1>, fg, dim3(256), 0, st, col, bias, im, a, *head, head_rows); break;
+        case 2: hipLaunchKernelGGL(col2im_k4s2p1_finish_kernel<2>, fg, dim3(256), 0, st, col, bias, im, a, *head, head_rows); break;
+        case 4: hipLaunchKernelGGL(col2im_k4s2p1_finish_kernel<4>, fg, dim3(256), 0, st, col, bias, im, a, *head, head_rows); break;
+        default: hipLaunchKernelGGL(col2im_k4s2p1_finish_kernel<8>, fg, dim3(256), 0, st, col, bias, im, a, *head, head_rows); break;
+      }
+    } else if (quad) hipLaunchKernelGGL(col2im_k4s2p1_bias_relu_kernel, dim3(bq, py), dim3(256), 0, st, col + (size_t)p0 * kernel * kernel * hwc, bias,
                                  im + (size_t)(p0 / C) * im_ctot * hw, a);
     else hipLaunchKernelGGL(col2im_bias_relu_kernel, dim3(bx, py), dim3(256), 0, st, col + (size_t)p0 * kernel * kernel * hwc, bias,
                             im + (size_t)(p0 / C) * im_ctot * hw, a);
@@ -159,6 +189,11 @@
 FN2_API int fn2_col2im_bias_relu_forward(const float* col, const float* bias, float* im, int N, int C, int H, int W,
                                          int kernel, int pad, int stride, int apply_relu, float negative_slope, void* stream) {
   return col2im_launch(col, bias, im, N, C, H, W, kernel, pad, stride, apply_relu, negative_slope, C, 0, stream);
+}
+
+int fn2::col2im_stage_finish(const float* col, const float* bias, float* top, int N, int C, int H, int W, int apply_relu, float negative_slope,
+                             int top_channels, int top_c0, const StageHead& head, void* stream) {
+  return col2im_launch(col, bias, top, N, C, H, W, 4, 1, 2, apply_relu, negative_slope, top_channels, top_c0, stream, &head);
 }
 
 FN2_API int fn2_col2im_bias_relu_forward_into(const float* col, const float* bias, float* top, int N, int C, int H, int W,
diff --git a/flownet2_amd/csrc/stage_finish.hpp b/flownet2_amd/csrc/stage_finish.hpp
--- /dev/null
+++ b/flownet2_amd/csrc/stage_finish.hpp
@@ -0,0 +1,18 @@
+#pragma once
+
+#include <cstddef>
+
+#include "flow_head_device.hpp"
+
+namespace fn2 {
+
+int predict_flow_head_splits(int N, int C, int H, int W);
+
+int col2im_stage_finish(const float* col, const float* bias, float* top, int N, int C, int H, int W, int apply_relu, float negative_slope,
+                        int top_channels, int top_c0, const StageHead& head, void* stream);
+
+int deconv_plane_stage_forward(const float* bottom, const float* packed_weight, const float* bias, float* top, int N, int Cin, int Hin, int Win,
+                               int bottom_channels, int bottom_c0, int Cout, int top_channels, int top_c0, int relu, float negative_slope,
+                               void* workspace, size_t workspace_bytes, const StageHead& head, void* stream);
+
+}
diff --git a/flownet2_amd/functional.py b/flownet2_amd/functional.py
--- a/flownet2_amd/functional.py
+++ b/flownet2_amd/functional.py
@@ -900,3 +900,25 @@
     if _needs_grad(x, weight, bias):
         return _OwnForwardConv.apply(x, weight, bias, run, 2, 1, negative_slope, True, True, None if out is None else (out, out_c0))
     return run(x, weight, bias, out, out_c0)
+
+
+_STAGE_DECLINED = set()
+
+
+def deconv_flow_stage(x, weight, bias, head_x, head_weight, head_bias, up_weight, up_bias, out, out_c0, negative_slope=0.1):
+    if not x.is_cuda or _needs_grad(x, weight, bias, head_x, head_weight, head_bias, up_weight, up_bias):
+        return None
+    desc = _layer_desc(weight, 2, 1, True, x_shape=x.shape)
+    route = deconv_forward_route(desc, True) if desc is not None else ops.DECONV_ROUTE_NONE
+    key = (tuple(x.shape), tuple(weight.shape), tuple(head_x.shape), route)
+    if route == ops.DECONV_ROUTE_NONE or route & ops.CONV_ARITH_BF16X3 or key in _STAGE_DECLINED or not head_x.is_contiguous() or head_x.shape[0] != x.shape[0] \
+            or head_x.shape[2:] != x.shape[2:]:
+        return None
+    blob, c0 = _channel_slice(x)
+    packed = _cached_pack(_PACKED_T, weight, ("fwd", route, True), lambda: ops.conv_pack_weights(weight.detach(), desc, route, True))
+    taps = ops.predict_flow_conv_taps(head_x, head_weight)
+    flow = ops.deconv_flow_stage_forward(blob, packed, bias, desc, route, negative_slope, out, out_c0, taps, head_x.shape[1], head_bias,
+                                         up_weight, up_bias, in_c0=c0)
+    if flow is None:
+        _STAGE_DECLINED.add(key)
+    return flow
diff --git a/flownet2_amd/graph_backend.py b/flownet2_amd/graph_backend.py
--- a/flownet2_amd/graph_backend.py
+++ b/flownet2_amd/graph_backend.py
@@ -36,6 +36,7 @@
         self.own_conv, self.own_deconv = get("conv_mfma_relu") or _declines, get("deconv_relu") or _declines
         self.own_correlation_relu_into = get("correlation_relu_into") or _declines
         self._predict, self._upsample = get("predict_flow_conv"), get("upsample_flow_deconv")
+        self._flow_stage = get("deconv_flow_stage")
         self._bias_act = get("conv_bias_leaky_relu")
         self._conv2d = get("lib_conv2d") or (lambda x, w, b, s, p: F.conv2d(x, w, b, stride=s, padding=p))
         self._deconv2d = get("lib_conv_transpose2d") or (lambda x, w, b, s, p: F.conv_transpose2d(x, w, b, stride=s, padding=p))
@@ -112,6 +113,16 @@
             return self._upsample(x, P[name + ".w"], P[name + ".b"], out=out, out_c0=out_c0)
         return self._upsample(x, P[name + ".w"], P[name + ".b"])
 
+    def flow_stage(self, x, P, dname, head_x, hname, uname, out, out_c0):
+        if self._flow_stage is None:
+            return None
+        wd = P[dname + ".w"]
+        flow = self._flow_stage(x, wd, P[dname + ".b"], head_x, P[hname + ".w"], P[hname + ".b"], P[uname + ".w"], P[uname + ".b"], out, out_c0,
+                                NEG_SLOPE)
+        if flow is not None:
+            self.wrote("deconv", dname, out, out, out_c0, wd.shape[1], x, wd, 2, 1)
+        return flow
+
     def leaky_relu(self, x, name, slope=NEG_SLOPE):
         y = self._act(x, slope, name)
         if _LISTENERS:
diff --git a/flownet2_amd/nets.py b/flownet2_amd/nets.py
--- a/flownet2_amd/nets.py
+++ b/flownet2_amd/nets.py
@@ -145,16 +145,25 @@
 
 
 def _decoder(P, conv6_1, conv5_1, conv4_1, conv3_1, conv2, be):
-    flow6 = be.predict_flow(conv6_1, P, "Convolution1")
-    c5 = _refine_stage(P, conv5_1, conv6_1, "deconv5", flow6, "upsample_flow6to5", be)
-    flow5 = be.predict_flow(c5, P, "Convolution2")
-    c4 = _refine_stage(P, conv4_1, c5, "deconv4", flow5, "upsample_flow5to4", be)
-    flow4 = be.predict_flow(c4, P, "Convolution3")
-    c3 = _refine_stage(P, conv3_1, c4, "deconv3", flow4, "upsample_flow4to3", be)
-    flow3 = be.predict_flow(c3, P, "Convolution4")
-    c2 = _refine_stage(P, conv2, c3, "deconv2", flow3, "upsample_flow3to2", be)
+    flow6, c5 = _flow_and_stage(P, conv5_1, conv6_1, "Convolution1", "deconv5", "upsample_flow6to5", be)
+    flow5, c4 = _flow_and_stage(P, conv4_1, c5, "Convolution2", "deconv4", "upsample_flow5to4", be)
+    flow4, c3 = _flow_and_stage(P, conv3_1, c4, "Convolution3", "deconv3", "upsample_flow4to3", be)
+    flow3, c2 = _flow_and_stage(P, conv2, c3, "Convolution4", "deconv2", "upsample_flow3to2", be)
     flow2 = be.predict_flow(c2, P, "Convolution5")
     return {2: flow2, 3: flow3, 4: flow4, 5: flow5, 6: flow6}
+
+
+STAGE_FINISH = [os.environ.get("FN2_STAGE_FINISH", "1") != "0"]
+
+
+def _flow_and_stage(P, skip, x, hname, dname, uname, be):
+    blob, s = skip if isinstance(skip, tuple) else (None, skip)
+    if STAGE_FINISH[0] and blob is not None and not (torch.is_grad_enabled() and s.requires_grad):
+        flow = be.flow_stage(x, P, dname, x, hname, uname, blob, s.shape[1])
+        if flow is not None:
+            return flow, blob
+    flow = be.predict_flow(x, P, hname)
+    return flow, _refine_stage(P, skip, x, dname, flow, uname, be)
 
 
 def _skip_conv(x, P, name, stride, pad, dname, be, relu_chain=None):
diff --git a/flownet2_amd/ops.py b/flownet2_amd/ops.py
--- a/flownet2_amd/ops.py
+++ b/flownet2_amd/ops.py
@@ -572,6 +572,49 @@
         C.byref(desc), int(route), _ptr(x), Ctot, int(in_c0), _ptr(pw), _ptr(b), _ptr(out), out.shape[1], int(out_c0),
         int(bool(relu)), C.c_float(float(negative_slope)), _ptr(ws), need, _stream()))
     return out
+
+
+def predict_flow_conv_taps(x, weight):
+    x, w = _chk(x, "bottom[0]"), _chk(weight, "weight")
+    N, Cc, H, W = x.shape
+    if tuple(w.shape) != (2, Cc, 3, 3):
+        raise ValueError(f"predict_flow weight must be [2,{Cc},3,3], got {tuple(w.shape)}")
+    L = _lib.lib()
+    nbytes = L.fn2_predict_flow_conv_workspace_bytes(N, Cc, H, W)
+    taps = torch.empty(nbytes, dtype=torch.uint8, device=x.device)
+    check(L.fn2_predict_flow_conv_taps(_ptr(x), _ptr(w), N, Cc, H, W, _ptr(taps), nbytes, _stream()))
+    return taps
+
+
+def deconv_flow_stage_forward(x, packed, bias, desc, route, negative_slope, out, out_c0, taps, head_channels, head_bias, up_weight, up_bias, in_c0=0):
+    x = _chk(x, "bottom[0]")
+    N, Ctot, H, W = x.shape
+    _chk(out, "top[0]")
+    if (N, H, W) != (desc.N, desc.Hin, desc.Win) or in_c0 < 0 or in_c0 + desc.Cin > Ctot:
+        raise ValueError(f"deconv_flow_stage_forward: bottom blob {tuple(x.shape)} does not hold the layer's [{desc.N},{desc.Cin},{desc.Hin},{desc.Win}] at channel {in_c0}")
+    if not out.is_contiguous() or out.shape[0] != N or tuple(out.shape[2:]) != (2 * H, 2 * W) or out_c0 < 0 or out_c0 + desc.Cout + 2 > out.shape[1]:
+        raise ValueError(f"deconv_flow_stage_forward: top blob {tuple(out.shape)} does not match [{N},>={out_c0 + desc.Cout + 2},{2 * H},{2 * W}]")
+    b, hb, ub = _chk_opt(bias, "bias", 1), _chk_opt(head_bias, "head bias", 1), _chk_opt(up_bias, "upsample bias", 1)
+    pw, uw = _chk(packed, "packed weight", ndim=None), _chk(up_weight, "upsample weight")
+    if tuple(uw.shape) != (2, 2, 4, 4) or (hb is not None and hb.numel() != 2) or (ub is not None and ub.numel() != 2):
+        raise ValueError("deconv_flow_stage_forward: the flow head has a [2,2,4,4] up-sampling weight and 2-entry biases")
+    L = _lib.lib()
+    if pw.numel() != int(L.fn2_deconv_packed_weight_floats(C.byref(desc), int(route))):
+        raise ValueError("deconv_flow_stage_forward: the operand has %d floats, not what route %d reads for this layer" % (pw.numel(), route))
+    need = int(L.fn2_deconv_workspace_bytes(C.byref(desc), int(route)))
+    if (route & ~CONV_ARITH_BF16X3) == DECONV_ROUTE_GEMM:
+        ws = torch.empty((need + 3) // 4, device=x.device, dtype=torch.float32)
+    else:
+        ws = _plane_workspace(x.device, need) if need else None
+    flow = torch.empty((N, 2, H, W), device=x.device, dtype=torch.float32)
+    status = L.fn2_deconv_flow_stage_forward(
+        C.byref(desc), int(route), _ptr(x), Ctot, int(in_c0), _ptr(pw), _ptr(b), _ptr(out), out.shape[1], int(out_c0), 1,
+        C.c_float(float(negative_slope)), _ptr(ws), need, _ptr(taps), taps.numel() * taps.element_size(), N, int(head_channels), H, W,
+        _ptr(hb), _ptr(flow), _ptr(uw), _ptr(ub), _stream())
+    if status == _lib.CONSTANTS["FN2_ERR_UNSUPPORTED"]:
+        return None
+    check(status)
+    return flow
 
 
 def conv_backward_data_route(desc, transposed=False, bf16x3=False) -> int:
diff --git a/include/flownet2_hip_decoder.h b/include/flownet2_hip_decoder.h
--- /dev/null
+++ b/include/flownet2_hip_decoder.h
@@ -0,0 +1,15 @@
+#pragma once
+#include "flownet2_hip.h"
+#ifdef __cplusplus
+extern "C" {
+#endif
+int fn2_predict_flow_conv_taps(const float* in, const float* weight, int N, int C, int H, int W, void* workspace, size_t workspace_bytes,
+                               void* stream);
+int fn2_deconv_flow_stage_forward(const fn2_conv_desc* desc, int route, const float* bottom, int bottom_channels, int bottom_c0,
+                                  const float* packed_weight, const float* bias, float* top, int top_channels, int top_c0,
+                                  int relu, float negative_slope, void* workspace, size_t workspace_bytes,
+                                  const float* head_taps, size_t head_taps_bytes, int head_N, int head_C, int head_H, int head_W,
+                                  const float* head_bias, float* flow, const float* upsample_weight, const float* upsample_bias, void* stream);
+#ifdef __cplusplus
+}
+#endif
```

Result: no change. 3631, median of 6 (+0.9%).
